# nolmoonen/jpeggpu

Measured on AMD Instinct MI355X. Metric: images/s, 12 MP 4:2:0 baseline JPEG decode, inputs resident in HBM (value_full_path: from pinned host memory, parse + transfer + decode; latency_ms: p50 of the reference's protocol), higher is better.
Workload: dtype int16/int32 fixed point, u8 out; 1 GPU; cfg2: 4032x3024 4:2:0 interleaved baseline JPEG, DRI=252 (one MCU row), 16 seeded images per rank; batch_per_gpu=256, mode=batch, streams=4, subsequence_bytes=256, device_scan=False, stuffed_scan_bytes=3163303, parallelism=image-sharded x1

## Files before the change

include/jpeggpu/jpeggpu_ext.h:

```cpp
#ifndef JPEGGPU_JPEGGPU_EXT_H_
#define JPEGGPU_JPEGGPU_EXT_H_

#include <jpeggpu/jpeggpu.h>

#ifdef __cplusplus
extern "C" {
#endif

enum jpeggpu_status jpeggpu_ext_set_subsequence_bytes(jpeggpu_decoder_t decoder, int subseq_bytes);
enum jpeggpu_status jpeggpu_ext_set_batched(jpeggpu_decoder_t decoder, int batched);
enum jpeggpu_status jpeggpu_ext_set_batch_hint(jpeggpu_decoder_t decoder, int images_per_call);

struct jpeggpu_ext_scan_layout {
    int num_components;
    int component_idx[JPEGGPU_MAX_COMP];
    int num_subsequences;
    int num_segments;
    int num_sequences;
    int num_data_units;
    int data_units_per_mcu;
    int num_chunks;
    size_t off_segments;
    size_t off_chunks;
    size_t off_destuffed;
// ... 15 lines not shown
struct jpeggpu_ext_layout {
    int subsequence_bytes;
    int subsequences_per_sequence;
    int num_scans;
    size_t transferred_bytes;
    size_t blob_bytes;
    size_t off_bytes;
    size_t off_qtables;
    struct jpeggpu_ext_scan_layout scans[JPEGGPU_MAX_COMP];
    int shard_rank, shard_world;
};

enum jpeggpu_status jpeggpu_ext_get_layout(jpeggpu_decoder_t decoder, struct jpeggpu_ext_layout* layout);

enum jpeggpu_status jpeggpu_ext_set_segment_shard(jpeggpu_decoder_t decoder, int rank, int world);
enum jpeggpu_status jpeggpu_ext_get_shard_rows(jpeggpu_decoder_t decoder, int component, int* first_row, int* num_rows);

enum jpeggpu_status jpeggpu_ext_set_device_scan(jpeggpu_decoder_t decoder, int enable);
enum jpeggpu_status jpeggpu_ext_get_device_status(
    jpeggpu_decoder_t decoder, const void* d_tmp, jpeggpu_stream_t stream, enum jpeggpu_status* status);

enum jpeggpu_status jpeggpu_ext_set_scale(jpeggpu_decoder_t decoder, int scale_denom);

enum jpeggpu_ext_scale_mode { JPEGGPU_EXT_SCALE_UNIFORM = 0, JPEGGPU_EXT_SCALE_LIBJPEG = 1 };
enum jpeggpu_status jpeggpu_ext_set_scale_mode(jpeggpu_decoder_t decoder, enum jpeggpu_ext_scale_mode mode);
struct jpeggpu_ext_scale_info {
    int scale_denom;
    int mode;
    int block_size[JPEGGPU_MAX_COMP];
    int fancy_upsampling;
};
enum jpeggpu_status jpeggpu_ext_get_scale_info(jpeggpu_decoder_t decoder, struct jpeggpu_ext_scale_info* info);

enum jpeggpu_ext_idct { JPEGGPU_EXT_IDCT_REFERENCE = 0, JPEGGPU_EXT_IDCT_ISLOW = 1 };
enum jpeggpu_status jpeggpu_ext_set_idct(jpeggpu_decoder_t decoder, enum jpeggpu_ext_idct method);

struct jpeggpu_ext_crop_info {
    int x, y, width, height;
    int origin_x[JPEGGPU_MAX_COMP];
    int origin_y[JPEGGPU_MAX_COMP];
    int full_x[JPEGGPU_MAX_COMP];
    int full_y[JPEGGPU_MAX_COMP];
};
enum jpeggpu_status jpeggpu_ext_set_crop(jpeggpu_decoder_t decoder, int x, int y, int width, int height);
enum jpeggpu_status jpeggpu_ext_get_crop(jpeggpu_decoder_t decoder, struct jpeggpu_ext_crop_info* info);

enum jpeggpu_status jpeggpu_ext_set_luma_only(jpeggpu_decoder_t decoder, int enable);

enum jpeggpu_ext_stage {
    JPEGGPU_EXT_STAGE_FRONT      = 0,
    JPEGGPU_EXT_STAGE_DESTUFF    = 1,
    JPEGGPU_EXT_STAGE_SYNC_INTRA = 2,
    JPEGGPU_EXT_STAGE_SYNC_INTER = 3,
    JPEGGPU_EXT_STAGE_TAILS      = 4,
    JPEGGPU_EXT_STAGE_WRITE      = 5,
    JPEGGPU_EXT_STAGE_IDCT       = 6,
    JPEGGPU_EXT_NUM_STAGES       = 7
};
enum jpeggpu_status jpeggpu_ext_set_profiling(jpeggpu_decoder_t decoder, int enable);
enum jpeggpu_status jpeggpu_ext_get_stage_ms(jpeggpu_decoder_t decoder, float* ms );

struct jpeggpu_batch;
typedef struct jpeggpu_batch* jpeggpu_batch_t;
struct jpeggpu_ext_batch_item {
    jpeggpu_decoder_t decoder;
    struct jpeggpu_img* img;
    void* d_tmp;
    size_t tmp_size;
};
size_t jpeggpu_ext_batch_scratch_size(int max_scans);
enum jpeggpu_status jpeggpu_ext_batch_create(jpeggpu_batch_t* batch, int max_scans);
enum jpeggpu_status jpeggpu_ext_decode_batch(
    jpeggpu_batch_t batch,
    const struct jpeggpu_ext_batch_item* items,
    int num_items,
    void* d_scratch,
    size_t scratch_size,
    jpeggpu_stream_t stream);
enum jpeggpu_status jpeggpu_ext_batch_destroy(jpeggpu_batch_t batch);
enum jpeggpu_status jpeggpu_ext_batch_set_sync_iterations(jpeggpu_batch_t batch, int iterations);
enum jpeggpu_status jpeggpu_ext_batch_set_overlap(jpeggpu_batch_t batch, int parts);
enum jpeggpu_status jpeggpu_ext_batch_set_fused_tail(jpeggpu_batch_t batch, int enable);
enum jpeggpu_status jpeggpu_ext_batch_set_sync_run(jpeggpu_batch_t batch, int r);
enum jpeggpu_status jpeggpu_ext_fused_tail_timeouts(unsigned int* count);
enum jpeggpu_status jpeggpu_ext_batch_set_profiling(jpeggpu_batch_t batch, int enable);
enum jpeggpu_status jpeggpu_ext_batch_get_stage_ms(jpeggpu_batch_t batch, float* ms );

enum jpeggpu_status jpeggpu_ext_upsample_planes(
    const struct jpeggpu_img_info* info,
    const struct jpeggpu_img* src,
    struct jpeggpu_img* dst,
    int width,
    int height,
    jpeggpu_stream_t stream);

enum jpeggpu_status jpeggpu_ext_self_test(jpeggpu_stream_t stream);

struct jpeggpu_ext_parse_item {
    jpeggpu_decoder_t decoder;
    struct jpeggpu_img_info* img_info;
    const uint8_t* data;
    size_t size;
};
enum jpeggpu_status jpeggpu_ext_parse_headers(
    const struct jpeggpu_ext_parse_item* items, int num_items, int num_threads, enum jpeggpu_status* statuses);

enum jpeggpu_status jpeggpu_ext_planes_to_rgbi(
    const struct jpeggpu_img_info* info,
    const struct jpeggpu_img* src,
    uint8_t* dst,
    int dst_pitch,
    int width,
    int height,
    jpeggpu_stream_t stream);

enum jpeggpu_status jpeggpu_ext_planes_to_rgbi_fancy(
    const struct jpeggpu_img_info* info,
    const struct jpeggpu_img* src,
    uint8_t* dst,
    int dst_pitch,
    int width,
    int height,
    jpeggpu_stream_t stream);

enum jpeggpu_status jpeggpu_ext_crop_to_rgbi_fancy(
    const struct jpeggpu_img_info* info,
    const struct jpeggpu_ext_crop_info* crop,
    const struct jpeggpu_img* src,
    uint8_t* dst,
    int dst_pitch,
    jpeggpu_stream_t stream);

enum jpeggpu_status jpeggpu_ext_planes_to_rgbi_replicate(
    const struct jpeggpu_img_info* info,
    const struct jpeggpu_img* src,
    uint8_t* dst,
    int dst_pitch,
    int width,
    int height,
    jpeggpu_stream_t stream);
enum jpeggpu_status jpeggpu_ext_crop_to_rgbi_replicate(
    const struct jpeggpu_img_info* info,
    const struct jpeggpu_ext_crop_info* crop,
    const struct jpeggpu_img* src,
    uint8_t* dst,
    int dst_pitch,
    jpeggpu_stream_t stream);

struct jpeggpu_ext_resize_item {
    const struct jpeggpu_img_info* info;
    const struct jpeggpu_ext_crop_info* crop;
    const struct jpeggpu_img* src;
};
enum jpeggpu_ext_filter { JPEGGPU_EXT_FILTER_BILINEAR = 0, JPEGGPU_EXT_FILTER_BICUBIC = 1 };
enum jpeggpu_ext_output_layout { JPEGGPU_EXT_NHWC = 0, JPEGGPU_EXT_NCHW = 1 };
size_t jpeggpu_ext_resize_scratch_size(
    const struct jpeggpu_ext_resize_item* items, int n, int out_w, int out_h, enum jpeggpu_ext_filter filter);
enum jpeggpu_status jpeggpu_ext_resize_to_rgb(
    const struct jpeggpu_ext_resize_item* items,
    int n,
    int out_w,
    int out_h,
    enum jpeggpu_ext_filter filter,
    enum jpeggpu_ext_output_layout layout,
    uint8_t* dst,
    void* d_scratch,
// ... 443 lines not shown
```

jpeggpu_amd/api.py:

```python
import ctypes as C
import enum
import os

from . import build as _build

MAX_COMP = 4
STAGES = ("front", "destuff", "sync_intra", "sync_inter", "tails", "write", "idct")
IDCT_METHODS = {"reference": 0, "islow": 1}
FILTERS = {"bilinear": 0, "bicubic": 1}
LAYOUTS = {"NHWC": 0, "NCHW": 1}
IMAGE_LAYOUTS = {"HWC": 0, "CHW": 1}
SCALE_MODES = {"uniform": 0, "libjpeg": 1}
SUBSAMPLINGS = {"4:4:4": 0, "4:2:2": 1, "4:2:0": 2}
TENSOR_TYPE_NAMES = {"uint8": 0, "float32": 1, "float16": 2, "bfloat16": 3}


def _tensor_types():
    import torch

    return {getattr(torch, name): v for name, v in TENSOR_TYPE_NAMES.items()}


class _TensorTypes(dict):

# ... 128 lines not shown
                ("progressive", C.c_int), ("optimize", C.c_int), ("restart_interval", C.c_int), ("out", C.c_void_p), ("capacity", C.c_size_t)]


class ExtScanLayout(C.Structure):
    _fields_ = [
        ("num_components", C.c_int), ("component_idx", C.c_int * MAX_COMP),
        ("num_subsequences", C.c_int), ("num_segments", C.c_int), ("num_sequences", C.c_int),
        ("num_data_units", C.c_int), ("data_units_per_mcu", C.c_int), ("num_chunks", C.c_int),
        ("off_segments", C.c_size_t), ("off_chunks", C.c_size_t), ("off_destuffed", C.c_size_t),
        ("off_segment_index", C.c_size_t), ("off_state_p", C.c_size_t), ("off_state_n", C.c_size_t),
        ("off_state_cz", C.c_size_t), ("off_state_dc01", C.c_size_t), ("off_state_dc23", C.c_size_t),
        ("off_symbols", C.c_size_t), ("off_du_table", C.c_size_t), ("symbol_region_entries", C.c_int),
        ("device_scan", C.c_int), ("off_device_status", C.c_size_t),
        ("hypotheses", C.c_int), ("hypothesis_blocks", C.c_int),
    ]


class ExtLayout(C.Structure):
    _fields_ = [
        ("subsequence_bytes", C.c_int), ("subsequences_per_sequence", C.c_int), ("num_scans", C.c_int),
        ("transferred_bytes", C.c_size_t), ("blob_bytes", C.c_size_t),
        ("off_bytes", C.c_size_t), ("off_qtables", C.c_size_t),
        ("scans", ExtScanLayout * MAX_COMP),
        ("shard_rank", C.c_int), ("shard_world", C.c_int),
    ]


class ParseItem(C.Structure):
    _fields_ = [("decoder", C.c_void_p), ("img_info", C.POINTER(ImgInfo)), ("data", C.c_void_p), ("size", C.c_size_t)]


class BatchItem(C.Structure):
    _fields_ = [("decoder", C.c_void_p), ("img", C.POINTER(Img)), ("d_tmp", C.c_void_p), ("tmp_size", C.c_size_t)]


class JpegGpuError(RuntimeError):
    def __init__(self, status, where=""):
        self.status = Status(status)
        super().__init__("%s: %s" % (where, status_string(status)))


_lib = None


def lib():
    global _lib
    if _lib is not None:
        return _lib
    try:
        import torch
    except ImportError:
        pass
    path = os.environ.get("JPEGGPU_LIB", _build.LIB_PATH)
    if not os.path.exists(path):
        raise ImportError(
            "jpeggpu_amd: %s is missing -- run `python -c 'import __graft_entry__ as g; g.build()'`" % path)
    L = C.CDLL(path)
    dec = C.c_void_p
    L.jpeggpu_get_status_string.restype = C.c_char_p
    L.jpeggpu_get_status_string.argtypes = [C.c_int]
    L.jpeggpu_decoder_startup.argtypes = [C.POINTER(dec)]
    L.jpeggpu_set_logging.argtypes = [dec, C.c_int]
    L.is_css_444.argtypes = [Subsampling, C.c_int]
    L.jpeggpu_decoder_parse_header.argtypes = [dec, C.POINTER(ImgInfo), C.c_void_p, C.c_size_t]
    L.jpeggpu_decoder_get_buffer_size.argtypes = [dec, C.POINTER(C.c_size_t)]
    L.jpeggpu_decoder_transfer.argtypes = [dec, C.c_void_p, C.c_size_t, C.c_void_p]
    L.jpeggpu_decoder_decode.argtypes = [dec, C.POINTER(Img), C.c_void_p, C.c_size_t, C.c_void_p]
    L.jpeggpu_decoder_cleanup.argtypes = [dec]
    L.jpeggpu_ext_set_subsequence_bytes.argtypes = [dec, C.c_int]
    L.jpeggpu_ext_set_batched.argtypes = [dec, C.c_int]
    L.jpeggpu_ext_set_batch_hint.argtypes = [dec, C.c_int]
    L.jpeggpu_ext_get_layout.argtypes = [dec, C.POINTER(ExtLayout)]
    L.jpeggpu_ext_set_profiling.argtypes = [dec, C.c_int]
    L.jpeggpu_ext_get_stage_ms.argtypes = [dec, C.POINTER(C.c_float)]
    L.jpeggpu_ext_batch_scratch_size.restype = C.c_size_t
    L.jpeggpu_ext_batch_scratch_size.argtypes = [C.c_int]
    L.jpeggpu_ext_batch_create.argtypes = [C.POINTER(C.c_void_p), C.c_int]
    L.jpeggpu_ext_decode_batch.argtypes = [C.c_void_p, C.POINTER(BatchItem), C.c_int, C.c_void_p, C.c_size_t, C.c_void_p]
    L.jpeggpu_ext_batch_destroy.argtypes = [C.c_void_p]
    L.jpeggpu_ext_batch_set_profiling.argtypes = [C.c_void_p, C.c_int]
    L.jpeggpu_ext_batch_set_sync_iterations.argtypes = [C.c_void_p, C.c_int]
    L.jpeggpu_ext_batch_set_overlap.argtypes = [C.c_void_p, C.c_int]
    for name, args in (("jpeggpu_ext_batch_set_fused_tail", [C.c_void_p, C.c_int]), ("jpeggpu_ext_batch_set_sync_run", [C.c_void_p, C.c_int]),
                       ("jpeggpu_ext_fused_tail_timeouts", [C.POINTER(C.c_uint)])):
        if hasattr(L, name):
            getattr(L, name).argtypes = args
    L.jpeggpu_ext_batch_get_stage_ms.argtypes = [C.c_void_p, C.POINTER(C.c_float)]
    L.jpeggpu_ext_upsample_planes.argtypes = [
        C.POINTER(ImgInfo), C.POINTER(Img), C.POINTER(Img), C.c_int, C.c_int, C.c_void_p]
    L.jpeggpu_ext_set_segment_shard.argtypes = [dec, C.c_int, C.c_int]
    L.jpeggpu_ext_get_shard_rows.argtypes = [dec, C.c_int, C.POINTER(C.c_int), C.POINTER(C.c_int)]
    L.jpeggpu_ext_self_test.argtypes = [C.c_void_p]
    L.jpeggpu_ext_set_device_scan.argtypes = [dec, C.c_int]
    L.jpeggpu_ext_set_scale.argtypes = [dec, C.c_int]
    L.jpeggpu_ext_set_idct.argtypes = [dec, C.c_int]
    L.jpeggpu_ext_set_scale_mode.argtypes = [dec, C.c_int]
    L.jpeggpu_ext_get_scale_info.argtypes = [dec, C.POINTER(ScaleInfo)]
    L.jpeggpu_ext_get_device_status.argtypes = [dec, C.c_void_p, C.c_void_p, C.POINTER(C.c_int)]
    L.jpeggpu_ext_parse_headers.argtypes = [C.POINTER(ParseItem), C.c_int, C.c_int, C.POINTER(C.c_int)]
    L.jpeggpu_ext_planes_to_rgbi.argtypes = [
        C.POINTER(ImgInfo), C.POINTER(Img), C.c_void_p, C.c_int, C.c_int, C.c_int, C.c_void_p]
    L.jpeggpu_ext_planes_to_rgbi_fancy.argtypes = [
        C.POINTER(ImgInfo), C.POINTER(Img), C.c_void_p, C.c_int, C.c_int, C.c_int, C.c_void_p]
    L.jpeggpu_ext_planes_to_rgbi_replicate.argtypes = L.jpeggpu_ext_planes_to_rgbi_fancy.argtypes
    L.jpeggpu_ext_set_crop.argtypes = [dec, C.c_int, C.c_int, C.c_int, C.c_int]
    L.jpeggpu_ext_get_crop.argtypes = [dec, C.POINTER(CropInfo)]
    L.jpeggpu_ext_crop_to_rgbi_fancy.argtypes = [
        C.POINTER(ImgInfo), C.POINTER(CropInfo), C.POINTER(Img), C.c_void_p, C.c_int, C.c_void_p]
    L.jpeggpu_ext_crop_to_rgbi_replicate.argtypes = L.jpeggpu_ext_crop_to_rgbi_fancy.argtypes
    L.jpeggpu_ext_resize_scratch_size.restype = C.c_size_t
    L.jpeggpu_ext_resize_scratch_size.argtypes = [C.POINTER(ResizeItem), C.c_int, C.c_int, C.c_int, C.c_int]
    L.jpeggpu_ext_resize_to_rgb.argtypes = [
        C.POINTER(ResizeItem), C.c_int, C.c_int, C.c_int, C.c_int, C.c_int, C.c_void_p, C.c_void_p, C.c_size_t, C.c_void_p]
    L.jpeggpu_ext_get_color_space.argtypes = [dec, C.POINTER(C.c_int)]
    L.jpeggpu_ext_planes_to_rgbi_fancy_cs.argtypes = [
        C.POINTER(ImgInfo), C.c_int, C.POINTER(Img), C.c_void_p, C.c_int, C.c_int, C.c_int, C.c_void_p]
    L.jpeggpu_ext_planes_to_rgbi_replicate_cs.argtypes = L.jpeggpu_ext_planes_to_rgbi_fancy_cs.argtypes
    L.jpeggpu_ext_crop_to_rgbi_fancy_cs.argtypes = [
        C.POINTER(ImgInfo), C.c_int, C.POINTER(CropInfo), C.POINTER(Img), C.c_void_p, C.c_int, C.c_void_p]
    L.jpeggpu_ext_crop_to_rgbi_replicate_cs.argtypes = L.jpeggpu_ext_crop_to_rgbi_fancy_cs.argtypes
    L.jpeggpu_ext_resize_scratch_size_cs.restype = C.c_size_t
    L.jpeggpu_ext_resize_scratch_size_cs.argtypes = [C.POINTER(ResizeItem), C.POINTER(C.c_int), C.c_int, C.c_int, C.c_int, C.c_int]
    L.jpeggpu_ext_resize_to_rgb_cs.argtypes = [
        C.POINTER(ResizeItem), C.POINTER(C.c_int), C.c_int, C.c_int, C.c_int, C.c_int, C.c_int, C.c_void_p, C.c_void_p, C.c_size_t,
        C.c_void_p]
    L.jpeggpu_ext_set_progressive.argtypes = [dec, C.c_int]
    L.jpeggpu_ext_get_progressive_info.argtypes = [dec, C.POINTER(ProgressiveInfo)]
    L.jpeggpu_ext_get_orientation.argtypes = [dec, C.POINTER(C.c_int)]
    L.jpeggpu_ext_orient_size.argtypes = [C.c_int, C.c_int, C.c_int, C.POINTER(C.c_int), C.POINTER(C.c_int)]
    L.jpeggpu_ext_orient_rect.argtypes = [C.c_int, C.c_int, C.c_int] + [C.POINTER(C.c_int)] * 4
    L.jpeggpu_ext_planes_to_rgbi_oriented.argtypes = [
        C.POINTER(ImgInfo), C.c_int, C.c_int, C.c_int, C.POINTER(Img), C.c_void_p, C.c_int, C.c_int, C.c_int, C.c_void_p]
    L.jpeggpu_ext_crop_to_rgbi_oriented.argtypes = [
        C.POINTER(ImgInfo), C.c_int, C.c_int, C.c_int, C.POINTER(CropInfo), C.POINTER(Img), C.c_void_p, C.c_int, C.c_void_p]
    L.jpeggpu_ext_resize_scratch_size_oriented.restype = C.c_size_t
    L.jpeggpu_ext_resize_scratch_size_oriented.argtypes = [
        C.POINTER(ResizeItem), C.POINTER(C.c_int), C.POINTER(C.c_int), C.c_int, C.c_int, C.c_int, C.c_int]
    L.jpeggpu_ext_resize_to_rgb_oriented.argtypes = [
        C.POINTER(ResizeItem), C.POINTER(C.c_int), C.POINTER(C.c_int), C.c_int, C.c_int, C.c_int, C.c_int, C.c_int, C.c_void_p,
        C.c_void_p, C.c_size_t, C.c_void_p]
    L.jpeggpu_ext_resize_to_tensor.argtypes = [
        C.POINTER(ResizeItem), C.POINTER(C.c_int), C.POINTER(C.c_int), C.c_int, C.c_int, C.c_int, C.c_int, C.c_int, C.POINTER(TensorSpec),
        C.c_void_p, C.c_void_p, C.c_size_t, C.c_void_p]
    L.jpeggpu_ext_resize_view_scratch_size.restype = C.c_size_t
    L.jpeggpu_ext_resize_view_scratch_size.argtypes = [
        C.POINTER(ResizeItem), C.POINTER(C.c_int), C.POINTER(C.c_int), C.POINTER(ResizeView), C.c_int, C.c_int, C.c_int, C.c_int]
    L.jpeggpu_ext_resize_view_to_tensor.argtypes = [
        C.POINTER(ResizeItem), C.POINTER(C.c_int), C.POINTER(C.c_int), C.POINTER(ResizeView), C.c_int, C.c_int, C.c_int, C.c_int, C.c_int,
        C.POINTER(TensorSpec), C.c_void_p, C.c_void_p, C.c_size_t, C.c_void_p]
    L.jpeggpu_ext_resize_view_rect.argtypes = [C.c_int, C.c_int, C.c_int, C.POINTER(ResizeView), C.c_int, C.c_int, C.c_int] + [C.POINTER(C.c_int)] * 4
    L.jpeggpu_ext_resize_view_weights.argtypes = [
        C.c_int, C.c_int, C.c_int, C.c_int, C.c_int, C.c_int, C.POINTER(C.c_int), C.POINTER(C.c_int), C.POINTER(C.c_int), C.c_int]
    L.jpeggpu_ext_batch_rgb_scratch_size.restype = C.c_size_t
    L.jpeggpu_ext_batch_rgb_scratch_size.argtypes = [C.c_int]
    L.jpeggpu_ext_batch_to_rgb.argtypes = [C.POINTER(RgbItem), C.c_int, C.c_int, C.c_void_p, C.c_size_t, C.c_void_p]
    if hasattr(L, "jpeggpu_ext_encode_batch"):
        L.jpeggpu_ext_encode_header.argtypes = [C.POINTER(EncodeItem), C.c_void_p, C.POINTER(C.c_size_t)]
        L.jpeggpu_ext_encode_bound.argtypes = [C.POINTER(EncodeItem)]
        L.jpeggpu_ext_encode_bound.restype = C.c_size_t
        L.jpeggpu_ext_encode_scratch_size.argtypes = [C.POINTER(EncodeItem), C.c_int]
        L.jpeggpu_ext_encode_scratch_size.restype = C.c_size_t
        L.jpeggpu_ext_encode_batch.argtypes = [C.POINTER(EncodeItem), C.c_int, C.c_void_p, C.c_size_t, C.c_void_p, C.c_void_p, C.c_void_p]
    if hasattr(L, "jpeggpu_ext_roundtrip_batch"):
        L.jpeggpu_ext_roundtrip_scratch_size.argtypes = [C.POINTER(RoundtripItem), C.c_int]
        L.jpeggpu_ext_roundtrip_scratch_size.restype = C.c_size_t
        L.jpeggpu_ext_roundtrip_batch.argtypes = [C.POINTER(RoundtripItem), C.c_int, C.c_int, C.c_void_p, C.c_size_t, C.c_void_p]
# ... 183 lines not shown
        _check(lib().jpeggpu_ext_set_segment_shard(self._h, rank, world), "jpeggpu_ext_set_segment_shard")

    def shard_rows(self, component: int):
        a, n = C.c_int(), C.c_int()
        _check(lib().jpeggpu_ext_get_shard_rows(self._h, component, C.byref(a), C.byref(n)), "jpeggpu_ext_get_shard_rows")
        return a.value, n.value

    def device_status(self, d_tmp: int, stream: int = 0) -> Status:
        st = C.c_int()
        _check(lib().jpeggpu_ext_get_device_status(self._h, d_tmp, stream, C.byref(st)), "jpeggpu_ext_get_device_status")
        return Status(st.value)

    def get_buffer_size(self) -> int:
        n = C.c_size_t()
        _check(lib().jpeggpu_decoder_get_buffer_size(self._h, C.byref(n)), "jpeggpu_decoder_get_buffer_size")
        return n.value

    def transfer(self, d_tmp: int, tmp_size: int, stream: int = 0):
        _check(lib().jpeggpu_decoder_transfer(self._h, d_tmp, tmp_size, stream), "jpeggpu_decoder_transfer")

    def decode(self, planes, pitches, d_tmp: int, tmp_size: int, stream: int = 0):
        _check(lib().jpeggpu_decoder_decode(self._h, C.byref(_img(planes, pitches)), d_tmp, tmp_size, stream), "jpeggpu_decoder_decode")

    def set_profiling(self, on: bool):
        _check(lib().jpeggpu_ext_set_profiling(self._h, int(on)), "jpeggpu_ext_set_profiling")

    def stage_ms(self):
        ms = (C.c_float * len(STAGES))()
        _check(lib().jpeggpu_ext_get_stage_ms(self._h, ms), "jpeggpu_ext_get_stage_ms")
        return dict(zip(STAGES, ms))

    def layout(self) -> ExtLayout:
        lay = ExtLayout()
        _check(lib().jpeggpu_ext_get_layout(self._h, C.byref(lay)), "jpeggpu_ext_get_layout")
        return lay

    def cleanup(self):
        if self._h:
            lib().jpeggpu_decoder_cleanup(self._h)
            self._h = C.c_void_p()

    def __del__(self):
        try:
            self.cleanup()
        except Exception:
            pass


class Batch:

    def __init__(self, max_scans: int):
        self._h = C.c_void_p()
        self.max_scans = max_scans
        _check(lib().jpeggpu_ext_batch_create(C.byref(self._h), max_scans), "jpeggpu_ext_batch_create")
        self.scratch_size = lib().jpeggpu_ext_batch_scratch_size(max_scans)
        self._items = None
        self._keep = None

    def set_items(self, entries):
        n = len(entries)
        arr = (BatchItem * n)()
        imgs = []
        for i, (dec, ptrs, pitches, d_tmp, tmp_size) in enumerate(entries):
            imgs.append(_img(ptrs, pitches))
            arr[i].decoder = dec._h
            arr[i].img = C.pointer(imgs[i])
            arr[i].d_tmp = d_tmp
            arr[i].tmp_size = tmp_size
        self._items, self._keep = arr, (imgs, entries)

    def decode(self, d_scratch: int, stream: int = 0):
        _check(lib().jpeggpu_ext_decode_batch(self._h, self._items, len(self._items), d_scratch, self.scratch_size, stream),
               "jpeggpu_ext_decode_batch")

    def set_overlap(self, parts: int):
        _check(lib().jpeggpu_ext_batch_set_overlap(self._h, parts), "jpeggpu_ext_batch_set_overlap")

    def set_fused_tail(self, enable: bool):
        _check(_newer_symbol("jpeggpu_ext_batch_set_fused_tail")(self._h, 1 if enable else 0), "jpeggpu_ext_batch_set_fused_tail")

    def set_sync_run(self, r: int):
        _check(_newer_symbol("jpeggpu_ext_batch_set_sync_run")(self._h, int(r)), "jpeggpu_ext_batch_set_sync_run")

    def set_coefficients_only(self, enable: bool):
        _check(_newer_symbol("jpeggpu_ext_batch_set_coefficients_only")(self._h, 1 if enable else 0), "jpeggpu_ext_batch_set_coefficients_only")

    def set_sync_iterations(self, n: int):
        _check(lib().jpeggpu_ext_batch_set_sync_iterations(self._h, n), "jpeggpu_ext_batch_set_sync_iterations")

    def set_profiling(self, on: bool):
        _check(lib().jpeggpu_ext_batch_set_profiling(self._h, int(on)), "jpeggpu_ext_batch_set_profiling")

    def stage_ms(self):
        ms = (C.c_float * len(STAGES))()
        _check(lib().jpeggpu_ext_batch_get_stage_ms(self._h, ms), "jpeggpu_ext_batch_get_stage_ms")
        return dict(zip(STAGES, ms))

    def destroy(self):
        if self._h:
            lib().jpeggpu_ext_batch_destroy(self._h)
            self._h = C.c_void_p()

    def __del__(self):
        try:
            self.destroy()
        except Exception:
            pass


def fused_tail_timeouts() -> int:
    n = C.c_uint(0)
    _check(_newer_symbol("jpeggpu_ext_fused_tail_timeouts")(C.byref(n)), "jpeggpu_ext_fused_tail_timeouts")
    return n.value


def self_test(stream: int = 0) -> None:
    _check(lib().jpeggpu_ext_self_test(stream), "jpeggpu_ext_self_test")


def draft_scale(width, height, requested):
    rw, rh = requested
    rw, rh = min(int(rw), width), min(int(rh), height)
    if rw < 1 or rh < 1:
        raise ValueError("requested size must be positive")
    s = min(width // rw, height // rh)
    return 8 if s >= 8 else 4 if s >= 4 else 2 if s >= 2 else 1


def orient_size(orientation, w, h):
    ow, oh = C.c_int(), C.c_int()
    _check(lib().jpeggpu_ext_orient_size(int(orientation), int(w), int(h), C.byref(ow), C.byref(oh)), "jpeggpu_ext_orient_size")
    return ow.value, oh.value


def orient_rect(orientation, w, h, rect):
    v = [C.c_int(int(a)) for a in rect]
    _check(lib().jpeggpu_ext_orient_rect(int(orientation), int(w), int(h), *[C.byref(a) for a in v]), "jpeggpu_ext_orient_rect")
    return tuple(a.value for a in v)


def _frame_size(info):
    n = info.num_components
    hmax, vmax = max(info.subsampling.x[:n]), max(info.subsampling.y[:n])
    return (info.sizes_x[[c for c in range(n) if info.subsampling.x[c] == hmax][0]],
            info.sizes_y[[c for c in range(n) if info.subsampling.y[c] == vmax][0]])


def decode_to_planes(data: bytes, device="cuda:0", subseq_bytes=None, return_tmp=False, device_scan=False, scale=1,
                     idct="reference", crop=None, scale_mode="uniform", return_color=False, progressive=False,
                     displayed_crop=False, return_orientation=False, luma_only=False):
    import torch

    dec = Decoder(subseq_bytes)
    try:
        if luma_only:
            dec.set_luma_only(True)
        if scale != 1:
            dec.set_scale(scale)
        if scale_mode != "uniform":
            dec.set_scale_mode(scale_mode)
        if idct != "reference":
            dec.set_idct(idct)
        if device_scan:
            dec.set_device_scan(True)
        if progressive:
            dec.set_progressive(True)
# ... 1417 lines not shown
```

jpeggpu_amd/csrc/jg_batch.cpp:

```cpp
#include "jg_decoder.hpp"
#include "jg_front.hpp"
#include "jg_kernels.hpp"
#include "jg_prog.hpp"
#include "jg_stage_timer.hpp"

#include <hip/hip_runtime.h>

#include <algorithm>
#include <cstdint>
#include <cstdlib>
#include <cstring>
#include <new>
#include <vector>

using jg::Decoder;

struct jpeggpu_batch {
    static constexpr int kRing = 4;
    int max_jobs = 0;
    uint8_t* staging[kRing]     = {};
    hipEvent_t copied[kRing]    = {};
    bool in_use[kRing]          = {};
    int next                    = 0;
    int sync_iters              = 1;
    bool sync_iters_set         = false;
    long long keep_flows_below  = jg::kKeepFlowsBelowSubseq;
    bool fuse_tail_write        = true;
    int sync_run                = 2;
    bool coefficients_only      = false;
    static constexpr int kMaxOverlap = 4;
    int overlap                 = 1;
    hipStream_t aux[kMaxOverlap - 1] = {};
    hipEvent_t joined[kMaxOverlap - 1] = {};
    std::vector<jg::ScanJob> jobs;
    std::vector<jg::FrontParams> fronts;
    std::vector<jg::ProgImage> progs;
    jg::ProgExtent prog_extent;
    hipEvent_t prog_done        = nullptr;
    std::vector<int> order, group_begin;
    struct Part {
        int begin, end, way;
        jg::JobExtent extent;
    };
    std::vector<Part> parts;
    jg::StageTimer timer;
};

namespace {

struct Call {
    const jpeggpu_ext_batch_item* items;
    int num_items;
    uint8_t* d_scratch;
    hipStream_t stream;
    bool keep_flows        = false;
    uint32_t front_windows = 0;
    size_t jbytes = 0, fbytes = 0, pbytes = 0;
    int ring = 0;
    hipStream_t part_stream[jpeggpu_batch::kMaxOverlap];
};

jpeggpu_status gather_jobs(jpeggpu_batch& b, Call& c)
{
    jg::ScanJob* d_jobs_rw = reinterpret_cast<jg::ScanJob*>(c.d_scratch);
    std::vector<int>& order = b.order;
    order.resize(static_cast<size_t>(c.num_items));
    for (int i = 0; i < c.num_items; ++i) order[static_cast<size_t>(i)] = i;
    std::stable_sort(order.begin(), order.end(), [&](int x, int y) { return c.items[x].decoder->d.subseq_bytes > c.items[y].decoder->d.subseq_bytes; });
    std::vector<int>& group_begin = b.group_begin;
    group_begin.clear();
    int subseq_bytes = 0;
    for (int k = 0; k < c.num_items; ++k) {
        const jpeggpu_ext_batch_item& it = c.items[order[static_cast<size_t>(k)]];
        if (it.decoder->d.subseq_bytes != subseq_bytes) {
            subseq_bytes = it.decoder->d.subseq_bytes;
            group_begin.push_back(static_cast<int>(b.jobs.size()));
        }
        const size_t first_job = b.jobs.size();
        const jpeggpu_status st = jg::build_jobs(it.decoder->d, it.img, it.d_tmp, it.tmp_size, b.sync_iters, false, c.keep_flows, b.jobs, !b.coefficients_only);
        if (st != JPEGGPU_SUCCESS) return st;
        if (const int dk = jg::device_scan_index(it.decoder->d); dk >= 0) {
            b.fronts.push_back(jg::front_params(it.decoder->d, it.d_tmp, d_jobs_rw + first_job + static_cast<size_t>(dk), dk));
            c.front_windows = std::max(c.front_windows, b.fronts.back().num_windows);
        }
        if (const Decoder& pd = it.decoder->d; pd.plan.prog.on) {
            b.progs.push_back(jg::ProgImage{static_cast<uint8_t*>(it.d_tmp), pd.plan.off_blob + pd.plan.prog.blob.header});
            jg::extend(b.prog_extent, *reinterpret_cast<const jg::ProgHeader*>(pd.blob + pd.plan.prog.blob.header));
        }
    }
    group_begin.push_back(static_cast<int>(b.jobs.size()));
    return JPEGGPU_SUCCESS;
}

jpeggpu_status stage_jobs(jpeggpu_batch& b, Call& c, size_t scratch_size)
{
    const size_t n = b.jobs.size(), nf = b.fronts.size(), np = b.progs.size();
    c.jbytes = sizeof(jg::ScanJob) * n, c.fbytes = sizeof(jg::FrontParams) * nf, c.pbytes = sizeof(jg::ProgImage) * np;
    if (static_cast<int>(n) > b.max_jobs || scratch_size < c.jbytes + c.fbytes + c.pbytes) return JPEGGPU_INVALID_ARGUMENT;
    const int r = c.ring = b.next;
    b.next      = (r + 1) % jpeggpu_batch::kRing;
    if (b.in_use[r] && hipEventSynchronize(b.copied[r]) != hipSuccess) return JPEGGPU_INTERNAL_ERROR;
    std::memcpy(b.staging[r], b.jobs.data(), c.jbytes);
    if (nf) std::memcpy(b.staging[r] + c.jbytes, b.fronts.data(), c.fbytes);
    if (np) std::memcpy(b.staging[r] + c.jbytes + c.fbytes, b.progs.data(), c.pbytes);
    if (!b.timer.begin(c.stream, static_cast<size_t>(jg::kNumStages) + 1)) return JPEGGPU_INTERNAL_ERROR;
    if (hipMemcpyAsync(c.d_scratch, b.staging[r], c.jbytes + c.fbytes + c.pbytes, hipMemcpyHostToDevice, c.stream) != hipSuccess) return JPEGGPU_INTERNAL_ERROR;
    if (nf && jg::launch_front_batch(reinterpret_cast<const jg::FrontParams*>(c.d_scratch + c.jbytes), static_cast<int>(nf), c.front_windows, c.stream) != hipSuccess) {
        (void)hipGetLastError();
        return JPEGGPU_INTERNAL_ERROR;
    }
    if (hipEventRecord(b.copied[r], c.stream) != hipSuccess) return JPEGGPU_INTERNAL_ERROR;
    b.in_use[r] = true;
    return JPEGGPU_SUCCESS;
}

jpeggpu_status cut_parts(jpeggpu_batch& b, Call& c)
{
    const int ways   = b.overlap;
    c.part_stream[0] = c.stream;
    for (int w = 1; w < ways; ++w) {
        if (!b.aux[w - 1]) {
            if (hipStreamCreateWithFlags(&b.aux[w - 1], hipStreamNonBlocking) != hipSuccess ||
                hipEventCreateWithFlags(&b.joined[w - 1], hipEventDisableTiming) != hipSuccess)
                return JPEGGPU_INTERNAL_ERROR;
        }
        c.part_stream[w] = b.aux[w - 1];
        if (hipStreamWaitEvent(c.part_stream[w], b.copied[c.ring], 0) != hipSuccess) return JPEGGPU_INTERNAL_ERROR;
    }
    typedef jpeggpu_batch::Part Part;
    b.parts.clear();
    for (size_t g = 0; g + 1 < b.group_begin.size(); ++g) {
        const int lo = b.group_begin[g], hi = b.group_begin[g + 1];
        int gw = ways;
        while (gw > 1 && (hi - lo) / gw < 4) --gw;
        for (int w = 0; w < gw; ++w) {
            Part p{lo + static_cast<int>(static_cast<long long>(hi - lo) * w / gw), lo + static_cast<int>(static_cast<long long>(hi - lo) * (w + 1) / gw), w, jg::JobExtent{}};
            for (int j = p.begin; j < p.end; ++j) jg::extend(p.extent, b.jobs[static_cast<size_t>(j)]);
            p.extent.repack_flows = c.keep_flows;
            p.extent.fuse_tail_write = b.fuse_tail_write && !b.sync_iters_set;
            p.extent.sync_run = c.keep_flows || b.sync_iters_set ? 1 : b.sync_run;
            if (p.end > p.begin) b.parts.push_back(p);
        }
    }
    return JPEGGPU_SUCCESS;
}

jpeggpu_status run_progressive(jpeggpu_batch& b, const Call& c)
{
    for (int k = 0; k < c.num_items; ++k) {
        const Decoder& pd = c.items[k].decoder->d;
        if (pd.plan.prog.on && hipMemsetAsync(static_cast<uint8_t*>(c.items[k].d_tmp) + pd.plan.prog.coef_begin, 0, pd.plan.prog.coef_bytes, c.stream) != hipSuccess)
            return JPEGGPU_INTERNAL_ERROR;
    }
    const jg::ProgImage* d_progs = reinterpret_cast<const jg::ProgImage*>(c.d_scratch + c.jbytes + c.fbytes);
    if (jg::launch_prog_batch(d_progs, static_cast<int>(b.progs.size()), b.prog_extent, c.stream) != hipSuccess) {
        (void)hipGetLastError();
        return JPEGGPU_INTERNAL_ERROR;
    }
    if (b.overlap > 1) {
        if (!b.prog_done && hipEventCreateWithFlags(&b.prog_done, hipEventDisableTiming) != hipSuccess) return JPEGGPU_INTERNAL_ERROR;
        if (hipEventRecord(b.prog_done, c.stream) != hipSuccess) return JPEGGPU_INTERNAL_ERROR;
        for (int w = 1; w < b.overlap; ++w)
            if (hipStreamWaitEvent(c.part_stream[w], b.prog_done, 0) != hipSuccess) return JPEGGPU_INTERNAL_ERROR;
    }
    return JPEGGPU_SUCCESS;
}

jpeggpu_status run_stages(jpeggpu_batch& b, const Call& c)
{
    const jg::ScanJob* d_jobs = reinterpret_cast<const jg::ScanJob*>(c.d_scratch);
    for (int stage = 0; stage < jg::kNumStages; ++stage) {
        const bool skip = stage == jg::kStageIdct && b.coefficients_only;
        if (stage == jg::kStageWrite && !b.progs.empty()) {
            const jpeggpu_status st = run_progressive(b, c);
            if (st != JPEGGPU_SUCCESS) return st;
        }
        for (const jpeggpu_batch::Part& p : b.parts) {
            if (skip) break;
            if (jg::launch_stage_batch(static_cast<jg::Stage>(stage), d_jobs + p.begin, p.end - p.begin, p.extent, c.part_stream[p.way]) != hipSuccess) {
                (void)hipGetLastError();
                return JPEGGPU_INTERNAL_ERROR;
            }
        }
        (void)b.timer.mark(stage, c.stream);
    }
    for (int w = 1; w < b.overlap; ++w) {
        if (hipEventRecord(b.joined[w - 1], c.part_stream[w]) != hipSuccess ||
            hipStreamWaitEvent(c.stream, b.joined[w - 1], 0) != hipSuccess)
            return JPEGGPU_INTERNAL_ERROR;
    }
    return JPEGGPU_SUCCESS;
}

jpeggpu_status decode_batch_impl(
    jpeggpu_batch_t batch, const jpeggpu_ext_batch_item* items, int num_items, void* d_scratch, size_t scratch_size, jpeggpu_stream_t stream)
{
    if (!batch || !items || num_items < 0 || !d_scratch) return JPEGGPU_INVALID_ARGUMENT;
    if (num_items == 0) return JPEGGPU_SUCCESS;
    batch->jobs.clear();
    batch->fronts.clear();
    batch->progs.clear();
    batch->prog_extent = jg::ProgExtent{};
    for (int i = 0; i < num_items; ++i)
        if (!items[i].decoder || !items[i].img) return JPEGGPU_INVALID_ARGUMENT;
    {
        bool all_lone = num_items <= jg::kLonePlanImages && !batch->timer.enabled() && !batch->coefficients_only;
        for (int i = 0; i < num_items && all_lone; ++i) all_lone = !items[i].decoder->d.batched;
        if (all_lone) {
            for (int i = 0; i < num_items; ++i) {
                const jpeggpu_status st = jg::do_decode(items[i].decoder->d, items[i].img, items[i].d_tmp, items[i].tmp_size, stream, false);
                if (st != JPEGGPU_SUCCESS) return st;
            }
            return JPEGGPU_SUCCESS;
        }
    }
    Call c{items, num_items, static_cast<uint8_t*>(d_scratch), stream};
    {
        long long total_subseq = 0;
        for (int i = 0; i < num_items; ++i) {
            const jg::Stream& s = items[i].decoder->d.reader.s;
            if (!items[i].decoder->d.parsed) return JPEGGPU_INVALID_ARGUMENT;
            for (int k = 0; k < s.num_scans; ++k) total_subseq += s.scans[k].num_subseq;
        }
        c.keep_flows = batch->sync_iters_set ? false : total_subseq < batch->keep_flows_below;
    }
    jpeggpu_status st = gather_jobs(*batch, c);
    if (st == JPEGGPU_SUCCESS) st = stage_jobs(*batch, c, scratch_size);
    if (st == JPEGGPU_SUCCESS) st = cut_parts(*batch, c);
    if (st == JPEGGPU_SUCCESS) st = run_stages(*batch, c);
    return st;
}

}

extern "C" {

size_t jpeggpu_ext_batch_scratch_size(int max_scans)
{
    static_assert(sizeof(jg::ProgImage) <= sizeof(jg::FrontParams), "a progressive item takes the place of front-end parameters");
    return static_cast<size_t>(max_scans > 0 ? max_scans : 0) * (sizeof(jg::ScanJob) + sizeof(jg::FrontParams));
}

enum jpeggpu_status jpeggpu_ext_batch_create(jpeggpu_batch_t* batch, int max_scans)
{
    if (!batch || max_scans <= 0) return JPEGGPU_INVALID_ARGUMENT;
    jpeggpu_batch* b = new (std::nothrow) jpeggpu_batch();
    if (!b) return JPEGGPU_OUT_OF_HOST_MEMORY;
    b->max_jobs = max_scans;
    if (const char* e = std::getenv("JPEGGPU_EXP_KEEP_FLOWS_BELOW")) b->keep_flows_below = std::atoll(e);
    if (const char* e = std::getenv("JPEGGPU_FUSE_TAIL_WRITE")) b->fuse_tail_write = std::atoi(e) != 0;
    if (const char* e = std::getenv("JPEGGPU_SYNC_RUN")) {
        const int r = std::atoi(e);
        if (r == 1 || r == 2 || r == 4) b->sync_run = r;
    }
    for (int r = 0; r < jpeggpu_batch::kRing; ++r) {
        void* p = nullptr;
        if (hipHostMalloc(&p, jpeggpu_ext_batch_scratch_size(max_scans), hipHostMallocDefault) != hipSuccess ||
            hipEventCreateWithFlags(&b->copied[r], hipEventDisableTiming) != hipSuccess) {
            (void)hipGetLastError();
            jpeggpu_ext_batch_destroy(b);
            return JPEGGPU_INTERNAL_ERROR;
        }
        b->staging[r] = static_cast<uint8_t*>(p);
    }
    *batch = b;
    return JPEGGPU_SUCCESS;
}

enum jpeggpu_status jpeggpu_ext_batch_destroy(jpeggpu_batch_t batch)
{
    if (!batch) return JPEGGPU_INVALID_ARGUMENT;
    for (int w = 0; w < jpeggpu_batch::kMaxOverlap - 1; ++w) {
        if (batch->aux[w]) {
            (void)hipStreamSynchronize(batch->aux[w]);
            (void)hipStreamDestroy(batch->aux[w]);
        }
        if (batch->joined[w]) (void)hipEventDestroy(batch->joined[w]);
    }
    for (int r = 0; r < jpeggpu_batch::kRing; ++r) {
        if (batch->staging[r]) (void)hipHostFree(batch->staging[r]);
        if (batch->copied[r]) (void)hipEventDestroy(batch->copied[r]);
    }
    if (batch->prog_done) (void)hipEventDestroy(batch->prog_done);
    delete batch;
    return JPEGGPU_SUCCESS;
}

enum jpeggpu_status jpeggpu_ext_decode_batch(
    jpeggpu_batch_t batch,
    const struct jpeggpu_ext_batch_item* items,
    int num_items,
    void* d_scratch,
    size_t scratch_size,
    jpeggpu_stream_t stream)
{
    try {
        return decode_batch_impl(batch, items, num_items, d_scratch, scratch_size, stream);
    } catch (const std::bad_alloc&) {
        return JPEGGPU_OUT_OF_HOST_MEMORY;
    }
}

enum jpeggpu_status jpeggpu_ext_batch_set_overlap(jpeggpu_batch_t batch, int parts)
{
    if (!batch || parts < 1 || parts > jpeggpu_batch::kMaxOverlap) return JPEGGPU_INVALID_ARGUMENT;
    batch->overlap = parts;
    return JPEGGPU_SUCCESS;
}

enum jpeggpu_status jpeggpu_ext_batch_set_fused_tail(jpeggpu_batch_t batch, int enable)
{
    if (!batch) return JPEGGPU_INVALID_ARGUMENT;
    batch->fuse_tail_write = enable != 0;
    return JPEGGPU_SUCCESS;
}

enum jpeggpu_status jpeggpu_ext_fused_tail_timeouts(unsigned int* count)
{
    if (!count) return JPEGGPU_INVALID_ARGUMENT;
    return jg::read_fuse_timeouts(count) == hipSuccess ? JPEGGPU_SUCCESS : JPEGGPU_INTERNAL_ERROR;
}

enum jpeggpu_status jpeggpu_ext_batch_set_sync_iterations(jpeggpu_batch_t batch, int iterations)
{
    if (!batch || iterations < 1) return JPEGGPU_INVALID_ARGUMENT;
    batch->sync_iters     = iterations;
    batch->sync_iters_set = true;
    return JPEGGPU_SUCCESS;
}

enum jpeggpu_status jpeggpu_ext_batch_set_coefficients_only(jpeggpu_batch_t batch, int enable)
{
    if (!batch) return JPEGGPU_INVALID_ARGUMENT;
    batch->coefficients_only = enable != 0;
    return JPEGGPU_SUCCESS;
}

enum jpeggpu_status jpeggpu_ext_batch_set_sync_run(jpeggpu_batch_t batch, int r)
{
    if (!batch || (r != 1 && r != 2 && r != 4)) return JPEGGPU_INVALID_ARGUMENT;
    batch->sync_run = r;
    return JPEGGPU_SUCCESS;
}

enum jpeggpu_status jpeggpu_ext_batch_set_profiling(jpeggpu_batch_t batch, int enable)
{
    if (!batch) return JPEGGPU_INVALID_ARGUMENT;
    batch->timer.enable(enable != 0);
    return JPEGGPU_SUCCESS;
}

enum jpeggpu_status jpeggpu_ext_batch_get_stage_ms(jpeggpu_batch_t batch, float* ms)
{
    if (!batch || !ms) return JPEGGPU_INVALID_ARGUMENT;
    return batch->timer.mean_ms(ms);
}

}
```

jpeggpu_amd/csrc/jg_defs.h:

```cpp
#ifndef JG_DEFS_H_
#define JG_DEFS_H_

#include <stddef.h>
#include <stdint.h>

#if defined(__HIPCC__)
#define JG_HD __host__ __device__
#else
#define JG_HD
#endif

namespace jg {

constexpr int kMaxComp      = 4;
constexpr int kMaxScans     = 4;
constexpr int kMaxDuPerMcu  = 10;
constexpr int kSeqLanes    = 256;
constexpr int kSeqOverlap  = 16;
constexpr int kSeqSubseq   = kSeqLanes - kSeqOverlap;
constexpr int kSeqOverlapBatch = 1;
constexpr int kSeqSubseqBatch  = kSeqLanes - kSeqOverlapBatch;
constexpr int kTailPartSubseq = 960;
constexpr long long kKeepFlowsBelowSubseq = 220000;
constexpr int kDestuffWin   = 4096;

#define JG_ORDER_NATURAL                                                                           \
    {0,  1,  8,  16, 9,  2,  3,  10, 17, 24, 32, 25, 18, 11, 4,  5,  12, 19, 26, 33, 40, 48,       \
     41, 34, 27, 20, 13, 6,  7,  14, 21, 28, 35, 42, 49, 56, 57, 50, 43, 36, 29, 22, 15, 23,       \
     30, 37, 44, 51, 58, 59, 52, 45, 38, 31, 39, 46, 53, 60, 61, 54, 47, 55, 62, 63}

constexpr int kLutBitsDc   = 9;
constexpr int kLutBitsAc   = 11;
constexpr int kSubBits     = 5;
constexpr int kSubTableSize = 2 << kSubBits;
constexpr int kMaxSubTables = 16;
constexpr int kHuffAuxSize = 16 + 16 + 256;
constexpr int kDcTableSize = (2 << kLutBitsDc) + kHuffAuxSize;
constexpr int kAcTableSize = (2 << kLutBitsAc) + kHuffAuxSize;

constexpr int kSyncEntryBytes = 4;
constexpr int kMultiMaxPre    = 15;
constexpr int kSyncMultiMaxBits = 31;
static_assert(kLutBitsAc + 15 <= kSyncMultiMaxBits && kSyncMultiMaxBits < (1 << 5),
              "a multi-symbol entry: codes inside the index, the last symbol's magnitude (category <= 15) behind it");
constexpr int kDcTableSizeSync = (kSyncEntryBytes << kLutBitsDc) + kHuffAuxSize;
constexpr int kAcTableSizeSync = (kSyncEntryBytes << kLutBitsAc) + kHuffAuxSize;

constexpr uint32_t kMaxTablePack =
    kMaxComp * (kDcTableSize + kMaxSubTables * kSubTableSize) + kMaxComp * (kAcTableSize + kMaxSubTables * kSubTableSize) + kMaxDuPerMcu * 16;
constexpr uint32_t kMaxTablePackSync =
    kMaxComp * (kDcTableSizeSync + kMaxSubTables * kSubTableSize) + kMaxComp * (kAcTableSizeSync + kMaxSubTables * kSubTableSize) + kMaxDuPerMcu * 16;
static_assert(kMaxTablePack < 65536 && kMaxTablePackSync < 65536, "table offsets are 16-bit");

constexpr uint32_t kEobAdvance = 63u;
constexpr uint32_t kEntrySlow  = 0x8000u;
JG_HD inline uint32_t huff_entry(int codelen, uint32_t sym, bool is_dc)
{
    const uint32_t s   = sym & 15u;
    const uint32_t r   = is_dc ? 0u : (sym >> 4);
    const bool eob = !is_dc && s == 0 && r != 15;
    return (static_cast<uint32_t>(codelen) + s) | (s << 5) | ((eob ? kEobAdvance : r + 1u) << 9);
}

constexpr int kRowLeadWords = 1;
constexpr int kRowTailWords = 2;
constexpr int kRowExtraWords = kRowLeadWords + kRowTailWords;
JG_HD constexpr int tile_rows_log2(int log2_w) { return log2_w >= 6 ? 4 : 5; }
constexpr int kMaxTileRows = 32;
JG_HD inline uint32_t tiled_slot(uint32_t row, uint32_t slot, int log2_w)
{
    const int lr = tile_rows_log2(log2_w);
    return (((row >> lr) * ((1u << log2_w) + kRowExtraWords) + slot) << lr) + (row & ((1u << lr) - 1u));
}
JG_HD inline uint32_t tiled_word(uint32_t linear_word, int log2_w)
{
    return tiled_slot(linear_word >> log2_w, (linear_word & ((1u << log2_w) - 1u)) + kRowLeadWords, log2_w);
}
JG_HD inline uint64_t tiled_buffer_bytes(uint32_t num_subseq, int subseq_bytes, int spare_rows)
{
    const uint64_t rows = (static_cast<uint64_t>(num_subseq) + static_cast<uint64_t>(spare_rows) + kMaxTileRows - 1) / kMaxTileRows * kMaxTileRows;
    return rows * (static_cast<uint64_t>(subseq_bytes) + 4u * kRowExtraWords);
}

constexpr uint32_t kMaxUnitEntries = 64 + 63;

constexpr uint32_t kSymSectorEntries = 16;
JG_HD constexpr uint32_t sym_region_entries(int subseq_bytes)
{
    return ((static_cast<uint32_t>(subseq_bytes) * 8u * 64u + 126u) / 127u + kMaxUnitEntries + kSymSectorEntries - 1u) / kSymSectorEntries * kSymSectorEntries;
}
static_assert(sym_region_entries(32) == 272 && sym_region_entries(64) == 400 && sym_region_entries(128) == 656 && sym_region_entries(256) == 1168,
              "whole sectors, at least ceil(8 B 64 / 127) + kMaxUnitEntries entries");

struct uint2_t {
    uint32_t x, y;
};

constexpr uint32_t kSymTileSubseq = 64;
constexpr uint32_t kSymSectorStride = kSymTileSubseq * kSymSectorEntries;
JG_HD inline uint32_t sym_region_base(uint32_t sub, uint32_t region_entries)
{
    return (sub / kSymTileSubseq) * (region_entries / kSymSectorEntries) * kSymSectorStride + (sub % kSymTileSubseq) * kSymSectorEntries;
}
JG_HD inline uint32_t sym_at(uint32_t base, uint32_t e)
{
    return base + (e / kSymSectorEntries) * kSymSectorStride + (e % kSymSectorEntries);
}
JG_HD inline uint32_t sym_advance(uint32_t first, uint32_t k)
{
    const uint32_t w = (first % kSymSectorEntries) + k;
    return (first & ~(kSymSectorEntries - 1u)) + (w / kSymSectorEntries) * kSymSectorStride + (w % kSymSectorEntries);
}
JG_HD inline uint64_t sym_buffer_entries(uint32_t num_subseq, uint32_t region_entries)
{
    const uint64_t tiles = (static_cast<uint64_t>(num_subseq) + kSymTileSubseq - 1) / kSymTileSubseq;
    return tiles * (region_entries / kSymSectorEntries) * kSymSectorStride + 16u * kSymSectorStride;
}
struct Segment {
    int subseq_offset;
    int subseq_count;
};

struct DestuffChunk {
    uint32_t win_off;
    uint32_t begin;
    uint32_t end;
    uint32_t dst_off;
    uint32_t pad_end;
    int32_t seg;
// ... 189 lines not shown
```

jpeggpu_amd/csrc/jg_huff_core.h:

```cpp
#ifndef JG_HUFF_CORE_H_
#define JG_HUFF_CORE_H_

#include "jg_defs.h"

namespace jg {

struct LaneState {
    int p;
    int n;
    int c;
    int z;
    uint32_t dc01;
    uint32_t dc23;
};

JG_HD inline uint32_t pk_add_u16(uint32_t a, uint32_t b)
{
#if defined(__HIP_DEVICE_COMPILE__)
    typedef unsigned short us2 __attribute__((ext_vector_type(2)));
    const us2 r = __builtin_bit_cast(us2, a) + __builtin_bit_cast(us2, b);
    return __builtin_bit_cast(uint32_t, r);
#else
    return ((a + b) & 0xFFFFu) | (((a >> 16) + (b >> 16)) << 16);
#endif
// ... 5 lines not shown
    int sh;
    typename Fetch::Pos pos;
    uint32_t next_raw;

    JG_HD inline void seek(int p, const Fetch& fetch)
    {
        const int q = p - 1;
        sh          = 31 - (q & 31);
        pos         = fetch.start(q >> 5);
        hi          = fetch.cook(fetch.load(pos), pos);
        fetch.advance(pos);
        lo = fetch.cook(fetch.load(pos), pos);
        fetch.advance(pos);
        next_raw = fetch.load(pos);
#if defined(__HIP_DEVICE_COMPILE__)
        asm volatile("v_mov_b32 %0, %0\n\tv_mov_b32 %1, %1" : "+v"(hi), "+v"(lo));
#endif
    }
    JG_HD inline uint32_t peek(const Fetch& fetch)
    {
        if (sh < 0) {
#if defined(__HIP_DEVICE_COMPILE__)
            asm("v_mov_b32 %0, %1\n\tv_mov_b32 %1, %2" : "+v"(hi), "+v"(lo) : "v"(fetch.cook(next_raw, pos)));
#else
            hi = lo;
            lo = fetch.cook(next_raw, pos);
#endif
            sh += 32;
            fetch.advance(pos);
            next_raw = fetch.load(pos);
        }
#if defined(__HIP_DEVICE_COMPILE__)
        return __builtin_amdgcn_alignbit(hi, lo, static_cast<uint32_t>(sh));
#else
        return static_cast<uint32_t>(((static_cast<uint64_t>(hi) << 32) | lo) >> sh);
#endif
    }
    JG_HD inline void skip(int len) { sh -= len; }
};

#if defined(JG_TABS_IN_LDS)
#define JG_TAB_AS __attribute__((address_space(3)))
#define JG_TAB_AT(tabs, off) (reinterpret_cast<::jg::TabPtr>(static_cast<uintptr_t>(static_cast<uint32_t>(off))))
#else
#define JG_TAB_AS
#define JG_TAB_AT(tabs, off) ((tabs) + (off))
#endif
typedef JG_TAB_AS const uint8_t* TabPtr;

JG_HD inline uint32_t ld_u16(TabPtr p) { return *reinterpret_cast<JG_TAB_AS const uint16_t*>(p); }
JG_HD inline uint32_t ld_u32(TabPtr p) { return *reinterpret_cast<JG_TAB_AS const uint32_t*>(p); }

JG_HD inline uint32_t huff_long_code(TabPtr aux, uint32_t peek, bool is_dc)
{
    const uint32_t v = peek >> 16;
    int l            = 9;
#if defined(__HIP_DEVICE_COMPILE__)
    typedef uint32_t u32x4 __attribute__((ext_vector_type(4)));
    const u32x4 lim = *reinterpret_cast<JG_TAB_AS const u32x4*>(aux);
#pragma unroll
    for (int j = 0; j < 7; ++j) l += v >= ((lim[j >> 1] >> (16 * (j & 1))) & 0xFFFFu) ? 1 : 0;
#else
    for (int j = 0; j < 7; ++j) l += v >= ld_u16(aux + 2 * j) ? 1 : 0;
#endif
    const uint32_t code = v >> (16 - l);
    const uint32_t off  = ld_u16(aux + 16 + 2 * (l - 9));
    const uint32_t sym  = aux[32 + ((off + code) & 0xFFu)];
    return huff_entry(l, sym, is_dc);
}

template <int kEntryBytes = 2>
JG_HD inline uint32_t huff_second_level(TabPtr tab, uint32_t e, uint32_t peek, bool is_dc)
{
    const int lb       = is_dc ? kLutBitsDc : kLutBitsAc;
    const TabPtr aux   = tab + (is_dc ? (kEntryBytes << kLutBitsDc) : (kEntryBytes << kLutBitsAc));
    if (e != 0) {
        const uint32_t i2 = (peek >> (32 - kSubBits - lb)) & ((1u << kSubBits) - 1u);
        e                 = ld_u16(aux + kHuffAuxSize - kSubTableSize + (e >> 5) * kSubTableSize + 2 * i2);
        if (e != 0) return e;
    }
    return huff_long_code(aux, peek, is_dc);
}

JG_HD inline int extend_magnitude(uint32_t bits, int s)
{
    const uint32_t mask = (1u << s) - 1u;
    return bits > (mask >> 1) ? static_cast<int>(bits) : static_cast<int>(bits - mask);
}

JG_HD inline uint32_t bits_field(uint32_t peek, int total_len, int s)
{
#if defined(__HIP_DEVICE_COMPILE__)
    return __builtin_amdgcn_ubfe(peek, 32 - total_len, s);
#else
    return s ? (peek << (total_len - s)) >> (32 - s) : 0u;
#endif
}

struct NoSink {
    static constexpr bool kSums = true;
};

struct SpecSink : NoSink {
    static constexpr bool kSums = false;
};

JG_HD inline uint32_t sym_entry_ac(int zpos, int value) { return (static_cast<uint32_t>(value) << 6) | static_cast<uint32_t>(zpos); }
JG_HD inline uint32_t sym_entry_escape(int value) { return (static_cast<uint32_t>(value) >> 10) << 6; }
JG_HD inline bool sym_needs_escape(int value) { return static_cast<uint32_t>(value + 511) > 1022u; }
constexpr int kEscapeFromCategory = 10;
JG_HD inline uint32_t sym_entry_index(uint32_t e) { return e & 63u; }
JG_HD inline int sym_entry_value(uint32_t e) { return static_cast<int16_t>(e) >> 6; }
JG_HD inline int sym_entry_value(uint32_t e, uint32_t escape) { return static_cast<int16_t>(((escape >> 6) << 10) | ((e & 0xFFFFu) >> 6)); }
constexpr uint32_t kUnitHasEscape = 0x80u;

#if defined(__HIP_DEVICE_COMPILE__)
#define JG_WAVE_ANY(x) (__builtin_amdgcn_ballot_w64(x) != 0ull)
#else
#define JG_WAVE_ANY(x) (x)
#endif

template <class Fetch, class Sink>
JG_HD inline void decode_subsequence(
    LaneState& st,
    BitWindow<Fetch>& bw,
    const Fetch& fetch,
    int end_bit,
    const uint8_t* tabs,
    const ScanParams& sp,
    Sink&)
{
#if defined(__HIP_DEVICE_COMPILE__)
    typedef uint32_t u32x4 __attribute__((ext_vector_type(4)));
#define JG_LOAD_CURSOR(off) (*reinterpret_cast<JG_TAB_AS const u32x4*>(JG_TAB_AT(tabs, off)))
    u32x4 cur = JG_LOAD_CURSOR(sp.cursor_off + 16u * static_cast<uint32_t>(st.c));
#define JG_CUR_TABS cur[0]
#define JG_CUR_META cur[1]
#define JG_CUR_SELF cur[2]
#define JG_CUR_NEXT cur[3]
#else
#define JG_LOAD_CURSOR(off) (*reinterpret_cast<const CursorEntry*>(tabs + (off)))
    CursorEntry cur = JG_LOAD_CURSOR(sp.cursor_off + 16u * static_cast<uint32_t>(st.c));
#define JG_CUR_TABS cur.tabs
#define JG_CUR_META cur.meta
#define JG_CUR_SELF cur.self
#define JG_CUR_NEXT cur.next
#endif
    int p       = st.p;
    int zm      = st.z - 1;
    int units   = 0;
    uint32_t dc01 = st.dc01, dc23 = st.dc23;
    bool is_dc = st.z == 0;
    uint32_t peek, e;
    int total;
#define JG_COMMIT()                                                                                       \
    do {                                                                                                  \
        bw.skip(total);                                                                                   \
        p += total;                                                                                       \
        const int adv     = e >> 9;                                                                       \
        const int zp      = zm + adv;                              \
        const bool du_end = zp >= 63;                                                                     \
        if (Sink::kSums && is_dc) {                                                                       \
            const int s      = (e >> 5) & 15;                                                             \
            const int v      = extend_magnitude(bits_field(peek, total, s), s);                           \
            const uint64_t d = static_cast<uint64_t>(static_cast<uint32_t>(v) & 0xFFFFu) << (JG_CUR_META & 63); \
            dc01             = pk_add_u16(dc01, static_cast<uint32_t>(d));                                \
            dc23             = pk_add_u16(dc23, static_cast<uint32_t>(d >> 32));                          \
        }                                                                                                 \
        zm = du_end ? -1 : zp;                                                                            \
        if (Sink::kSums) units += du_end ? 1 : 0;                                                         \
        cur = JG_LOAD_CURSOR(du_end ? JG_CUR_NEXT : JG_CUR_SELF);                                         \
        is_dc = du_end;                         \
    } while (0)
    {
        while (end_bit - p >= 31) {
            peek               = bw.peek(fetch);
            const TabPtr tab   = JG_TAB_AT(tabs, is_dc ? (JG_CUR_TABS & 0xFFFFu) : (JG_CUR_TABS >> 16));
            const uint32_t idx = peek >> (is_dc ? 32 - kLutBitsDc : 32 - kLutBitsAc);
            const uint32_t e32 = ld_u32(tab + kSyncEntryBytes * idx);
            const uint32_t one = e32 & 0xFFFFu, m = e32 >> 16;
            e                  = zm + static_cast<int>((m >> 5) & 15u) < 63 ? m : one;
            if (JG_WAVE_ANY((one & 31u) == 0)) {
                if ((one & 31u) == 0) e = huff_second_level<kSyncEntryBytes>(tab, one, peek, is_dc);
            }
            total = e & 31;
            JG_COMMIT();
        }
#define JG_LOOKUP_SYNC()                                                                                  \
    do {                                                                                                  \
        peek               = bw.peek(fetch);                                                              \
        const TabPtr tab   = JG_TAB_AT(tabs, is_dc ? (JG_CUR_TABS & 0xFFFFu) : (JG_CUR_TABS >> 16));      \
        const uint32_t idx = peek >> (is_dc ? 32 - kLutBitsDc : 32 - kLutBitsAc);                         \
        e                  = ld_u16(tab + kSyncEntryBytes * idx);                                         \
        if ((e & 31u) == 0) e = huff_second_level<kSyncEntryBytes>(tab, e, peek, is_dc);                  \
        total = e & 31;                                                                                   \
    } while (0)
        JG_LOOKUP_SYNC();
        while (p + total <= end_bit) {
            JG_COMMIT();
            JG_LOOKUP_SYNC();
        }
#undef JG_LOOKUP_SYNC
    }
#undef JG_COMMIT
    if (Sink::kSums) st.n += 64 * units + (zm + 1) - st.z;
    st.p    = p;
    st.z    = zm + 1;
    st.c    = (JG_CUR_META >> 8) & 0xFF;
    st.dc01 = dc01;
    st.dc23 = dc23;
#undef JG_LOAD_CURSOR
#undef JG_CUR_TABS
#undef JG_CUR_META
#undef JG_CUR_SELF
#undef JG_CUR_NEXT
}

constexpr int kWriteDcPeriod = 4;
constexpr int kWriteRarePeriod = 8;

JG_HD inline uint32_t bit_mask(int s)
{
#if defined(__HIP_DEVICE_COMPILE__)
    uint32_t m;
    asm("v_bfm_b32 %0, %1, 0" : "=v"(m) : "v"(s));
    return m;
#else
    return (1u << s) - 1u;
#endif
}

template <int kLutBits>
JG_HD inline uint32_t lut16_entry(TabPtr tab, uint32_t peek)
{
#if defined(__HIP_DEVICE_COMPILE__) && defined(JG_TABS_IN_LDS)
    uint32_t a;
    asm("v_lshrrev_b32 %0, %1, %2\n\tv_lshl_add_u32 %0, %0, 1, %3"
        : "=&v"(a)
        : "n"(32 - kLutBits), "v"(peek), "v"(static_cast<uint32_t>(reinterpret_cast<uintptr_t>(tab))));
    return ld_u16(reinterpret_cast<TabPtr>(static_cast<uintptr_t>(a)));
#else
    return ld_u16(tab + 2 * (peek >> (32 - kLutBits)));
#endif
}

JG_HD inline int lut16_entry_signed(TabPtr tab, uint32_t peek)
{
#if defined(__HIP_DEVICE_COMPILE__) && defined(JG_TABS_IN_LDS)
    uint32_t a;
    asm("v_lshrrev_b32 %0, %1, %2\n\tv_lshl_add_u32 %0, %0, 1, %3"
        : "=&v"(a)
        : "n"(32 - kLutBitsAc), "v"(peek), "v"(static_cast<uint32_t>(reinterpret_cast<uintptr_t>(tab))));
    return *reinterpret_cast<JG_TAB_AS const int16_t*>(static_cast<uintptr_t>(a));
#else
    return *reinterpret_cast<JG_TAB_AS const int16_t*>(tab + 2 * (peek >> (32 - kLutBitsAc)));
#endif
}

JG_HD inline uint32_t zero_if_negative(uint32_t e, int x)
{
#if defined(__HIP_DEVICE_COMPILE__)
    uint32_t r;
    asm("v_ashrrev_i32 %0, 31, %1\n\tv_bfi_b32 %0, %0, 0, %2" : "=&v"(r) : "v"(x), "v"(e));
    return r;
#else
    return x < 0 ? 0u : e;
#endif
}

JG_HD inline int extend_field(uint32_t peek, int total, int s)
{
#if defined(__HIP_DEVICE_COMPILE__)
    const int t = __builtin_amdgcn_sbfe(static_cast<int>(peek), static_cast<uint32_t>(32 - total), static_cast<uint32_t>(s));
    return t - static_cast<int>(bit_mask(s) ^ static_cast<uint32_t>(t >> 31));
#else
    const uint32_t bits = bits_field(peek, total, s);
    const uint32_t mask = bit_mask(s);
    return bits > (mask >> 1) ? static_cast<int>(bits) : static_cast<int>(bits - mask);
#endif
}

JG_HD inline int extend_bits(uint32_t bits, int s)
{
    const uint32_t mask = bit_mask(s);
    return bits > (mask >> 1) ? static_cast<int>(bits) : static_cast<int>(bits - mask);
// ... 143 lines not shown
```

jpeggpu_amd/csrc/jg_kernels.hip:

```cpp
#define JG_TABS_IN_LDS 1
#include "jg_huff_core.h"
#include "jg_kernels.hpp"
#include "jg_sync_runs.h"

#include <hip/hip_runtime.h>

#include <type_traits>

#include "jg_bytes.h"
#include "jg_idct.hpp"
#include "jg_jobs.h"
#include "jg_wave.h"

namespace jg {

namespace {

constexpr int T   = kSeqLanes;
constexpr int kMaxSeq = kSeqLanes - 1;


constexpr int kDestuffChunksPerWg = 2;

template <class J_t>
// ... 435 lines not shown
            st    = LaneState{};
            known = true;
        }
        lim = min(img_end, seg.subseq_offset + seg.subseq_count - img_first);
        flowing = known;
    }
    NoSink sink;
    const auto flow_step = [&](int j) -> bool {
        st.n    = 0;
        st.dc01 = 0;
        st.dc23 = 0;
        ++rel;
        fetch.set_row(img_first + j, rel);
        bw.seek(st.p, fetch);
        decode_subsequence(st, bw, fetch, (rel + 1) * kBits, s_tab, sp, sink);
        const int cz     = st.c | (st.z << 8);
        const bool synced = st.p == s_p[j] && cz == s_cz[j] && (s_pend[j] & 2);
        s_p[j]    = st.p;
        s_n[j]    = st.n;
        s_cz[j]   = cz;
        s_dc01[j] = st.dc01;
        s_dc23[j] = st.dc23;
        s_pend[j] = 2;
        return !synced;
    };
    int j    = t;
    int iter = 0;
    for (; iter < sp.max_intra_iters; ++iter) {
        bool go = flowing && j + 1 < lim;
        if (iter > 0) {
            int rank;
            const int total = block_rank<T>(go, s_wave, rank);
            if (total == 0) break;
            if (go) {
                s_fj[rank]   = j | lim << 16;
                s_frel[rank] = rel;
                s_fp[rank]   = st.p;
                s_fcz[rank]  = st.c | (st.z << 8);
            }
            __syncthreads();
            go = t < total;
            if (go) {
                const int pk = s_fj[t], cz = s_fcz[t];
                j    = pk & 0xFFFF;
                lim  = pk >> 16;
                rel  = s_frel[t];
                st.p = s_fp[t];
                st.c = cz & 0xFF;
                st.z = cz >> 8;
            }
        }
        flowing = go;
        if (go) flowing = flow_step(++j);
    }
    if (iter == sp.max_intra_iters && flowing && j + 1 < lim) {
        if (j >= OV) s_pend[j] |= 1;
        if (j == OV - 1) s_cut = 1;
    }
    __syncthreads();

    if (active && t >= OV) {
        J.pending[sub] = static_cast<uint8_t>(s_pend[t] & 1);
        J.st_p[sub]    = s_p[t];
        J.st_n[sub]    = s_n[t];
        J.st_cz[sub]   = s_cz[t];
        J.st_dc01[sub] = s_dc01[t];
        J.st_dc23[sub] = s_dc23[t];
    }
    if (t == OV - 1) {
        const bool have = active && !s_cut;
        J.bnd_p[blockIdx.x]  = have ? s_p[t] : -1;
        J.bnd_cz[blockIdx.x] = have ? s_cz[t] : -1;
    }
}

constexpr int kBatchSeqPerWg = 2;
struct SeqLdsBatch {
    static constexpr uint32_t kState = 0;
    static constexpr uint32_t kOne   = (6 * (T + 1) * 4 + 64 + 15) / 16 * 16;
    static constexpr uint32_t kTabs  = kState + kBatchSeqPerWg * kOne;
    static_assert(kTabs % 16 == 0, "the table pack is read with 16-byte loads");
};
static_assert(kStaticLdsSlack + SeqLdsBatch::kTabs + kMaxTablePackSync <= 65536, "absolute table addresses are packed into 16 bits (load_tables)");
constexpr int kFuseJobs = 16, kFuseMaxJobs = 256, kFuseOwn = kFuseJobs + 2 * kFuseMaxJobs;
constexpr uint32_t kFuseEmpty = 0xFFFFFFFFu;
static_assert(fuse_ctl_words(0) == static_cast<size_t>(kFuseOwn), "the plan carves what fuse_init lays out (jg_defs.h)");

__device__ __forceinline__ void fuse_init(const ScanJob* jobs, int job, const JobView& J, int lanes)
{
    JG_GLOBAL uint32_t* own  = as_global(jobs[job].fuse_ctl);
    JG_GLOBAL uint32_t* ctl0 = as_global(jobs[0].fuse_ctl);
    const int t = threadIdx.x, SEQ = J.sp.seq_subseq, S = J.sp.num_subseq;
    if (t < kFuseJobs) own[t] = 0u;
    if (t < 2 && job < kFuseMaxJobs) ctl0[kFuseJobs + 2 * job + t] = 0u;
    for (int q = t; q < J.num_seq; q += lanes) {
        const int first = q * SEQ, last = min(first + SEQ, S) - 1;
        uint32_t holders = 0;
        for (int k = 0; k < J.num_tail_parts; ++k) holders += J.tail_parts[k] <= last && J.tail_parts[k + 1] > first ? 1u : 0u;
        own[kFuseOwn + q]             = holders;
        own[kFuseOwn + J.num_seq + q] = kFuseEmpty;
    }
}

struct RunIo {
    const JobView& J;
    int* s_p;
    int* s_cz;
    __device__ __forceinline__ Segment segment_of(int sub) const { return ld_global(J.segments + J.seg_idx[sub]); }
    __device__ __forceinline__ void put_e1(int lane, int p, int cz) const
    {
        s_p[lane]  = p;
        s_cz[lane] = cz;
    }
    __device__ __forceinline__ bool e1_is(int lane, int p, int cz) const { return s_p[lane] == p && s_cz[lane] == cz; }
    __device__ __forceinline__ void store(int sub, const LaneState& st, int cz, bool pending) const
    {
        J.pending[sub] = static_cast<uint8_t>(pending ? 1 : 0);
        J.st_p[sub]    = st.p;
        J.st_n[sub]    = st.n;
        J.st_cz[sub]   = cz;
        J.st_dc01[sub] = st.dc01;
        J.st_dc23[sub] = st.dc23;
    }
};

template <int W, class JS, int R>
__device__ __forceinline__ void sync_intra_batch_runs(const JS& js, uint8_t* smem)
{
    const int which = threadIdx.x / T, l = threadIdx.x % T;
    int* s_p        = reinterpret_cast<int*>(smem + SeqLdsBatch::kState + which * SeqLdsBatch::kOne);
    int* s_cz       = s_p + 2 * T;
    uint8_t* s_tab  = smem + SeqLdsBatch::kTabs;

    const JobView J(js.get());
    if constexpr (std::is_same<JS, JobArray>::value) {
        if (blockIdx.x == 0) fuse_init(js.jobs, static_cast<int>(blockIdx.y), J, T * kBatchSeqPerWg);
    }
    if (static_cast<int>(blockIdx.x) * kBatchSeqPerWg * R >= J.num_seq) return;
    ScanParams sp = J.sp;
    sp.use_sync_pack();
    const int SEQ   = sp.seq_subseq;
    const int group = static_cast<int>(blockIdx.x) * kBatchSeqPerWg + which;
    RunLane ln;
    run_plan<R>(ln, l, group * SEQ * R, SEQ, sp.num_subseq);
    const int lane_seg = J.seg_idx[ln.active ? ln.a : 0];

    load_tables(s_tab, J.tables_sync, sp);
    const Segment lane_segment = ld_global(J.segments + lane_seg);
    __syncthreads();

    GlobalFetch<W> fetch{reinterpret_cast<JG_GLOBAL const uint32_t*>(J.destuffed), 0, 0};
    const RunIo io{J, s_p, s_cz};
    run_speculate<W>(ln, l, lane_segment, fetch, s_tab, sp, io);
    __syncthreads();
    run_flow<W, R>(ln, l, fetch, s_tab, sp, io);

    if (l < R && group * R + l < J.num_seq) {
        J.bnd_p[group * R + l]  = -1;
        J.bnd_cz[group * R + l] = -1;
    }
}

template <int W, class JS, int R = 1>
__global__ __launch_bounds__(T * kBatchSeqPerWg) void huff_sync_intra_batch(JS js)
{
    extern __shared__ __attribute__((aligned(16))) uint8_t smem[];
    if constexpr (R > 1) {
        sync_intra_batch_runs<W, JS, R>(js, smem);
        return;
    }
    const int which = threadIdx.x / T;
    const int seq   = blockIdx.x * kBatchSeqPerWg + which;
    int* s_p         = reinterpret_cast<int*>(smem + SeqLdsBatch::kState + which * SeqLdsBatch::kOne);
    int* s_n         = s_p + T;
    int* s_cz        = s_n + T;
    uint32_t* s_dc01 = reinterpret_cast<uint32_t*>(s_cz + T);
    uint32_t* s_dc23 = s_dc01 + T;
    int* s_pend      = reinterpret_cast<int*>(s_dc23 + T);
    uint8_t* s_tab   = smem + SeqLdsBatch::kTabs;

    const JobView J(js.get());
    if constexpr (std::is_same<JS, JobArray>::value) {
        if (blockIdx.x == 0) fuse_init(js.jobs, static_cast<int>(blockIdx.y), J, T * kBatchSeqPerWg);
    }
    if (static_cast<int>(blockIdx.x) * kBatchSeqPerWg >= J.num_seq) return;
    ScanParams sp = J.sp;
    sp.use_sync_pack();
    const int t         = threadIdx.x % T;
    s_pend[t]           = 0;
    const int SEQ = sp.seq_subseq, OV = T - SEQ;
    const int first_sub = seq * SEQ;
    const int img_first = first_sub - OV;
    const int img_end   = min(T, sp.num_subseq - img_first);

    constexpr int kBits = W * 32;
    const int sub       = img_first + t;
    const bool active   = sub >= 0 && t < img_end;
    const int lane_seg = J.seg_idx[active ? sub : 0];

    load_tables(s_tab, J.tables_sync, sp);
    const Segment lane_segment = ld_global(J.segments + lane_seg);
    __syncthreads();

    constexpr bool mh = false;
    LaneState st{};
    BitWindow<GlobalFetch<W>> bw{};
    GlobalFetch<W> fetch{reinterpret_cast<JG_GLOBAL const uint32_t*>(J.destuffed), 0, 0};
    Segment seg{0, 0};
    int rel = 0;
    bool known = true;
    if (active) {
        seg = lane_segment;
        rel = sub - seg.subseq_offset;
        if (mh) {
            st.p         = J.mh_p[sub];
            const int cz = J.mh_cz[sub];
            st.c         = cz & 0xFF;
            st.z         = cz >> 8;
            known        = J.mh_known[sub] != 0;
            s_pend[t]    = known ? 2 : 0;
        } else {
            st.p = rel * kBits;
            fetch.set_row(sub, rel);
            bw.seek(st.p, fetch);
            if (JS::kSpeculateStateOnly) {
                SpecSink none;
                decode_subsequence(st, bw, fetch, (rel + 1) * kBits, s_tab, sp, none);
            } else {
                NoSink sums;
                decode_subsequence(st, bw, fetch, (rel + 1) * kBits, s_tab, sp, sums);
                s_n[t]    = st.n;
                s_dc01[t] = st.dc01;
                s_dc23[t] = st.dc23;
            }
            s_pend[t] = 2;
        }
        s_p[t]  = st.p;
        s_cz[t] = st.c | (st.z << 8);
    }
    __syncthreads();

    const bool covers_starts = JS::kSpeculateStateOnly || mh;
    bool flowing = covers_starts ? t + 1 < img_end && img_first + t + 1 >= 0 : active;
    int lim      = 0;
    if (flowing) {
        const int sub_j = img_first + t + 1;
        if (covers_starts && (!active || rel + 1 == seg.subseq_count)) {
            seg   = ld_global(J.segments + J.seg_idx[sub_j]);
            rel   = -1;
            st    = LaneState{};
            known = true;
        }
        lim = min(img_end, seg.subseq_offset + seg.subseq_count - img_first);
        flowing = known;
    }
    NoSink sink;
    int iter = 0;
    for (; iter < sp.max_intra_iters; ++iter) {
        const int j = t + 1 + iter;
        if (flowing && j < lim) {
            st.n    = 0;
            st.dc01 = 0;
            st.dc23 = 0;
            ++rel;
            fetch.set_row(img_first + j, rel);
            bw.seek(st.p, fetch);
            decode_subsequence(st, bw, fetch, (rel + 1) * kBits, s_tab, sp, sink);
            const int cz = st.c | (st.z << 8);
            if (st.p == s_p[j] && cz == s_cz[j] && (s_pend[j] & 2)) flowing = false;
            s_p[j]    = st.p;
            s_n[j]    = st.n;
            s_cz[j]   = cz;
            s_dc01[j] = st.dc01;
            s_dc23[j] = st.dc23;
            s_pend[j] = 2;
        } else {
            flowing = false;
        }
        const bool more = __syncthreads_or(flowing && j + 1 < lim);
        if (!more) break;
    }
    if (iter == sp.max_intra_iters && flowing && t + 1 + iter < lim && t + iter >= OV) s_pend[t + iter] |= 1;
    __syncthreads();

    if (active && t >= OV) {
        J.pending[sub] = static_cast<uint8_t>(s_pend[t] & 1);
        J.st_p[sub]    = s_p[t];
        J.st_n[sub]    = s_n[t];
        J.st_cz[sub]   = s_cz[t];
        J.st_dc01[sub] = s_dc01[t];
        J.st_dc23[sub] = s_dc23[t];
    }
    if (t == OV - 1 && seq < J.num_seq) {
        J.bnd_p[seq]  = -1;
        J.bnd_cz[seq] = -1;
    }
}


template <int W, class JS>
__global__ __launch_bounds__(T) void huff_mh_spec(JS js)
{
    extern __shared__ __attribute__((aligned(16))) uint8_t smem[];
    const JobView J(js.get());
    ScanParams sp = J.sp;
    sp.use_sync_pack();
    load_tables(smem, J.tables_sync, sp);
    __syncthreads();
    const int sub = blockIdx.x * T + threadIdx.x, h = blockIdx.y;
    if (sub == 0 && h == 0) st_global(J.mh_pool, uint2_t{0u, 0u});
    if (sub >= sp.num_subseq) return;
    const Segment seg = ld_global(J.segments + J.seg_idx[sub]);
    const int rel     = sub - seg.subseq_offset;
    LaneState st{};
    st.p = rel * (W * 32);
    st.c = h;
    GlobalFetch<W> fetch{reinterpret_cast<JG_GLOBAL const uint32_t*>(J.destuffed), 0, 0};
    fetch.set_row(sub, rel);
    BitWindow<GlobalFetch<W>> bw{};
    bw.seek(st.p, fetch);
    SpecSink none;
    decode_subsequence(st, bw, fetch, (rel + 1) * (W * 32), smem, sp, none);
    const size_t at = static_cast<size_t>(h) * sp.num_subseq + sub;
    J.mh_p[at]      = st.p;
    J.mh_cz[at]     = st.c | (st.z << 8);
}

template <int W, class JS>
__global__ __launch_bounds__(T) void huff_mh_flow(JS js)
{
    extern __shared__ __attribute__((aligned(16))) uint8_t smem[];
    const JobView J(js.get());
    ScanParams sp = J.sp;
    sp.use_sync_pack();
    load_tables(smem, J.tables_sync, sp);
    __syncthreads();
    const int sub = blockIdx.x * T + threadIdx.x, h = blockIdx.y;
    const int S = sp.num_subseq, H = sp.mh;
    if (sub >= S) return;
    const size_t at   = static_cast<size_t>(h) * S + sub;
    const Segment seg = ld_global(J.segments + J.seg_idx[sub]);
    const int seg_end = seg.subseq_offset + seg.subseq_count;
    LaneState st{};
    st.p = J.mh_p[at];
    {
        const int cz = J.mh_cz[at];
        st.c         = cz & 0xFF;
        st.z         = cz >> 8;
    }
    GlobalFetch<W> fetch{reinterpret_cast<JG_GLOBAL const uint32_t*>(J.destuffed), 0, 0};
// ... 751 lines not shown
        JG_GLOBAL uint32_t* own = as_global(job.fuse_ctl);
        const int SEQ = J.sp.seq_subseq, lo = J.tail_parts[part], hi = J.tail_parts[part + 1];
        for (int q = lo / SEQ + static_cast<int>(threadIdx.x); q <= (hi - 1) / SEQ && q < J.num_seq; q += T) {
            if (JG_FUSE_ADD(own + kFuseOwn + q, 0xFFFFFFFFu) == 1u) {
                const uint32_t i = JG_FUSE_ADD(ctl0 + kFuseJobs + 2 * j, 1u);
                if (i < static_cast<uint32_t>(J.num_seq)) JG_FUSE_STORE(own + kFuseOwn + J.num_seq + i, static_cast<uint32_t>(q));
            }
        }
        return;
    }
    const uint32_t r = role - num_tail;
    if (r >= static_cast<uint32_t>(num_jobs) * static_cast<uint32_t>(max_seq)) return;
    const uint32_t home = r / static_cast<uint32_t>(max_seq);
    if (static_cast<int>(r % static_cast<uint32_t>(max_seq)) >= constant_job(jobs, home).num_seq) return;
    if (threadIdx.x < 64) {
        uint32_t polls = 0, got_job = kFuseEmpty, got_i = 0;
        while (got_job == kFuseEmpty) {
            for (int base = 0; base < num_jobs && got_job == kFuseEmpty; base += 64) {
                const int k      = base + static_cast<int>(threadIdx.x);
                const uint32_t j = (home + static_cast<uint32_t>(k)) % static_cast<uint32_t>(num_jobs);
                bool has         = false;
                if (k < num_jobs) {
                    const uint32_t pushed = JG_FUSE_LOAD(ctl0 + kFuseJobs + 2 * j), claimed = JG_FUSE_LOAD(ctl0 + kFuseJobs + 2 * j + 1);
                    has                   = claimed < pushed;
                }
                const unsigned long long any = __builtin_amdgcn_ballot_w64(has);
                if (any) {
                    const int first = __builtin_ctzll(any);
                    const uint32_t jj = static_cast<uint32_t>(__builtin_amdgcn_readlane(static_cast<int>(j), first));
                    uint32_t i = 0;
                    if (threadIdx.x == 0) i = JG_FUSE_ADD(ctl0 + kFuseJobs + 2 * jj + 1, 1u);
                    i = static_cast<uint32_t>(__builtin_amdgcn_readfirstlane(static_cast<int>(i)));
                    if (i < static_cast<uint32_t>(constant_job(jobs, jj).num_seq)) {
                        got_job = jj;
                        got_i   = i;
                    }
                }
            }
            if (got_job == kFuseEmpty) {
                if (++polls > kFuseMaxPolls) break;
                __builtin_amdgcn_s_sleep(32);
            }
        }
        uint32_t q = kFuseEmpty;
        if (got_job != kFuseEmpty) {
            const ScanJob& job = constant_job(jobs, got_job);
            JG_GLOBAL uint32_t* entry = as_global(job.fuse_ctl) + kFuseOwn + job.num_seq + got_i;
            while ((q = JG_FUSE_LOAD(entry)) == kFuseEmpty) {
                if (++polls > kFuseMaxPolls) break;
                __builtin_amdgcn_s_sleep(8);
            }
        }
        if (threadIdx.x == 0) {
            if (q == kFuseEmpty) atomicAdd(&g_fuse_timeouts, 1u);
            s_claim[0] = got_job;
            s_claim[1] = q;
        }
    }
    __syncthreads();
    const uint32_t seq = __builtin_amdgcn_readfirstlane(s_claim[1]);
    if (seq == kFuseEmpty) return;
    const ScanJob& job = constant_job(jobs, __builtin_amdgcn_readfirstlane(s_claim[0]));
    const JobView J(job);
    write_sequence<W, true>(J, static_cast<int>(seq), smem);
}
#undef JG_FUSE_LOAD
#undef JG_FUSE_ADD
#undef JG_FUSE_STORE


template <class K>
hipError_t allow_lds(K kernel, size_t bytes)
{
    if (bytes <= 64 * 1024) return hipSuccess;
    return hipFuncSetAttribute(
        reinterpret_cast<const void*>(kernel), hipFuncAttributeMaxDynamicSharedMemorySize, static_cast<int>(bytes));
}

inline bool fuses_tail_write(const JobExtent& e, int num_jobs)
{
    return e.fuse_tail_write && !e.repack_flows && e.max_tail_parts > 0 && e.max_tail_part < kTailLargeFrom && e.max_seq > 0 && num_jobs <= kFuseMaxJobs;
}

template <int W, class JS>
hipError_t launch_huff(Stage stage, const JS& js, const JobExtent& e, int grid_y, hipStream_t stream)
{
    const size_t seq_lds = SeqLds::kTabs + e.max_tab_bytes_sync;
    hipError_t err       = hipSuccess;
    if (e.max_tab_bytes > kMaxTablePack || e.max_tab_bytes_sync > kMaxTablePackSync) return hipErrorInvalidValue;
    switch (stage) {
    case kStageSyncIntra:
        if constexpr (JS::kRepackFlows) {
            if ((err = allow_lds(huff_sync_intra<W, JS>, seq_lds)) != hipSuccess) return err;
            huff_sync_intra<W, JS><<<dim3(e.max_seq, grid_y), T, seq_lds, stream>>>(js);
        } else if (e.repack_flows) {
            if ((err = allow_lds(huff_sync_intra<W, JobArrayLow>, seq_lds)) != hipSuccess) return err;
            huff_sync_intra<W, JobArrayLow><<<dim3(e.max_seq, grid_y), T, seq_lds, stream>>>(JobArrayLow{js.jobs});
        } else {
            const size_t lds = SeqLdsBatch::kTabs + e.max_tab_bytes_sync;
            if (e.sync_run == 2 || e.sync_run == 4) {
                const int per_wg = kBatchSeqPerWg * e.sync_run;
                const dim3 grid((e.max_seq + per_wg - 1) / per_wg, grid_y);
                if (e.sync_run == 2) {
                    if ((err = allow_lds(huff_sync_intra_batch<W, JS, 2>, lds)) != hipSuccess) return err;
                    huff_sync_intra_batch<W, JS, 2><<<grid, T * kBatchSeqPerWg, lds, stream>>>(js);
                } else {
                    if ((err = allow_lds(huff_sync_intra_batch<W, JS, 4>, lds)) != hipSuccess) return err;
                    huff_sync_intra_batch<W, JS, 4><<<grid, T * kBatchSeqPerWg, lds, stream>>>(js);
                }
                break;
            }
            if ((err = allow_lds(huff_sync_intra_batch<W, JS>, lds)) != hipSuccess) return err;
            huff_sync_intra_batch<W, JS><<<dim3((e.max_seq + kBatchSeqPerWg - 1) / kBatchSeqPerWg, grid_y), T * kBatchSeqPerWg, lds, stream>>>(js);
        }
        break;
    case kStageSyncInter:
        if (e.max_tail_parts > 0 && !(std::is_same<JS, JobArray>::value && fuses_tail_write(e, grid_y)))
        {
            if (e.max_tail_part >= kTailLargeFrom) {
                constexpr int TL = kTailLanesLarge;
                huff_sync_tail<W, TL, JS><<<dim3(e.max_tail_parts, grid_y), TL, 3 * TL * 4 + e.max_tab_bytes_sync, stream>>>(js);
            } else {
                huff_sync_tail<W, T, JS><<<dim3(e.max_tail_parts, grid_y), T, 3 * T * 4 + e.max_tab_bytes_sync, stream>>>(js);
            }
        }
        break;
    case kStageWrite: {
        size_t lds = WriteLds::kTabs + e.max_tab_bytes;
        if constexpr (std::is_same<JS, JobArray>::value) {
            if (fuses_tail_write(e, grid_y)) {
                const size_t tail_lds = 3 * T * 4 + e.max_tab_bytes_sync;
                lds                   = lds > tail_lds ? lds : tail_lds;
                if ((err = allow_lds(huff_tail_write<W>, lds)) != hipSuccess) return err;
                const long long wgs = static_cast<long long>(grid_y) * (static_cast<long long>(e.max_tail_parts) + e.max_seq);
                if (wgs > 0x7FFFFFFFll) return hipErrorInvalidValue;
                huff_tail_write<W><<<dim3(static_cast<unsigned>(wgs)), T, lds, stream>>>(js.jobs, grid_y, e.max_tail_parts, e.max_seq);
                break;
            }
        }
        huff_write<W, JS><<<dim3(e.max_seq, grid_y), T, lds, stream>>>(js);
        break;
    }
    default: return hipErrorInvalidValue;
    }
    return hipGetLastError();
}


inline hipError_t launch_idct(const JobByValue& js, const JobExtent& e, int, hipStream_t stream) { return launch_idct_job(js.job, e, stream); }
inline hipError_t launch_idct(const JobsByValue& js, const JobExtent& e, int num_jobs, hipStream_t stream) { return launch_idct_scans(js.jobs, num_jobs, e, stream); }
inline hipError_t launch_idct(const JobSingle& js, const JobExtent& e, int, hipStream_t stream) { return launch_idct_device_job(js.job, e, stream); }
inline hipError_t launch_idct(const JobArray& js, const JobExtent& e, int num_jobs, hipStream_t stream) { return launch_idct_batch(js.jobs, num_jobs, e, stream); }

template <class JS>
hipError_t launch_any(Stage stage, const JS& js, const JobExtent& e, int grid_y, hipStream_t stream)
{
    switch (stage) {
    case kStageFront:
        return hipSuccess;
    case kStageDestuff:
        if (e.max_chunks == 0) return hipSuccess;
        destuff_kernel<JS><<<dim3((e.max_chunks + kDestuffChunksPerWg - 1) / kDestuffChunksPerWg, grid_y), 256, 0, stream>>>(js);
        return hipGetLastError();
    case kStageTails:
        if (e.max_seq == 0 || (e.max_tail_parts > 0 && e.max_tail_part < kTailLargeFrom)) return hipSuccess;
        huff_seq_tails<JS><<<dim3(e.max_seq, grid_y), T, 0, stream>>>(js);
        return hipGetLastError();
    case kStageIdct: return launch_idct(js, e, grid_y, stream);
    case kStageSyncIntra:
    case kStageSyncInter:
    case kStageWrite:
        if (e.max_seq == 0) return hipSuccess;
        switch (e.subseq_words) {
        case 8: return launch_huff<8, JS>(stage, js, e, grid_y, stream);
        case 16: return launch_huff<16, JS>(stage, js, e, grid_y, stream);
        case 32: return launch_huff<32, JS>(stage, js, e, grid_y, stream);
        case 64: return launch_huff<64, JS>(stage, js, e, grid_y, stream);
        }
        return hipErrorInvalidValue;
    default: return hipErrorInvalidValue;
// ... 112 lines not shown
```

jpeggpu_amd/csrc/jg_kernels.hpp:

```cpp
#ifndef JG_KERNELS_HPP_
#define JG_KERNELS_HPP_

#include "jg_defs.h"

#include <hip/hip_runtime_api.h>

namespace jg {

bool subseq_bytes_supported(int subseq_bytes);

enum Stage {
    kStageFront     = 0,
    kStageDestuff   = 1,
    kStageSyncIntra = 2,
    kStageSyncInter = 3,
    kStageTails     = 4,
    kStageWrite     = 5,
    kStageIdct      = 6,
    kNumStages      = 7
};

struct JobExtent {
    int max_chunks      = 0;
    int max_seq         = 0;
    int max_tail_parts  = 0;
    int max_tail_part   = 0;
    int max_idct_blocks = 0;
    int subseq_words    = 0;
    uint32_t scales     = 0;
    uint32_t draft_sizes = 0;
    bool luma_reference = false;
    uint32_t methods    = 0;
    bool crop           = false;
    uint32_t max_tab_bytes = 0;
    uint32_t max_tab_bytes_sync = 0;
    bool fuse_tail_write = false;
    int sync_run        = 1;
    bool repack_flows   = false;
};
void extend(JobExtent& e, const ScanJob& job);
hipError_t read_fuse_timeouts(unsigned int* count);

hipError_t launch_stage(Stage stage, const ScanJob& job, hipStream_t stream);

hipError_t launch_stage_scans(Stage stage, const ScanJob* jobs, int num_jobs, hipStream_t stream);

hipError_t launch_mh(const ScanJob& job, const ScanJob* d_job, int max_seg_subseq, hipStream_t stream);

hipError_t launch_stage_device_job(Stage stage, const ScanJob* d_job, const JobExtent& extent, hipStream_t stream);

hipError_t launch_stage_batch(
    Stage stage, const ScanJob* d_jobs, int num_jobs, const JobExtent& extent, hipStream_t stream);

}

#endif
```

jpeggpu_amd/csrc/jg_plan.cpp:

```cpp
#include "jg_decoder.hpp"

#include <algorithm>
#include <cstring>
#include <new>

namespace jg {

namespace {

size_t align_up(size_t v, size_t a) { return (v + a - 1) / a * a; }

struct Carve {
    size_t at = 0;
    std::vector<PlanTrace::Region>* trace = nullptr;
    size_t operator()(size_t bytes)
    {
        const size_t o = at;
        at += align_up(bytes, 256);
        if (trace) trace->push_back({o, bytes});
        return o;
    }
};

template <typename T>
T* at(uint8_t* base, size_t off)
{
    return reinterpret_cast<T*>(base + off);
}

}

void Decoder::set_block_sizes()
{
    const Stream& s = reader.s;
    const int mn    = 8 >> scale_log2;
    draft           = false;
    for (int c = 0; c < s.num_comp; ++c) {
        int size = mn;
        if (scale_mode == JPEGGPU_EXT_SCALE_LIBJPEG)
            while (size < 8 && (s.hs_max * mn) % (s.comp[c].hs * size * 2) == 0 && (s.vs_max * mn) % (s.comp[c].vs * size * 2) == 0) size *= 2;
        blk_lg[c] = size == 8 ? 0 : size == 4 ? 1 : size == 2 ? 2 : 3;
        if (size != mn) draft = true;
    }
}

bool Decoder::set_crop_window()
{
    const Stream& s = reader.s;
    Crop c;
    c.on = true;
    c.x = crop_request[0], c.y = crop_request[1], c.w = crop_request[2], c.h = crop_request[3];
    if (c.x + static_cast<long long>(c.w) > scaled(s.size_x) || c.y + static_cast<long long>(c.h) > scaled(s.size_y)) return false;
    int lo_x[kMaxComp], hi_x[kMaxComp], lo_y[kMaxComp], hi_y[kMaxComp];
    c.mx0 = c.my0 = 1 << 30;
    for (int k = 0; k < s.num_comp; ++k) {
        const Component& fc = s.comp[k];
        const int n = blk(k), hs = eff_hs(k), vs = eff_vs(k);
        lo_x[k] = std::max(static_cast<int>(static_cast<long long>(c.x) * hs / s.hs_max) - 1, 0);
        hi_x[k] = std::min(static_cast<int>(static_cast<long long>(c.x + c.w - 1) * hs / s.hs_max) + 1, full_x(k) - 1);
        lo_y[k] = std::max(static_cast<int>(static_cast<long long>(c.y) * vs / s.vs_max) - 1, 0);
        hi_y[k] = std::min(static_cast<int>(static_cast<long long>(c.y + c.h - 1) * vs / s.vs_max) + 1, full_y(k) - 1);
        c.mx0 = std::min(c.mx0, lo_x[k] / (n * fc.hs)), c.mx1 = std::max(c.mx1, hi_x[k] / (n * fc.hs) + 1);
        c.my0 = std::min(c.my0, lo_y[k] / (n * fc.vs)), c.my1 = std::max(c.my1, hi_y[k] / (n * fc.vs) + 1);
    }
    for (int k = 0; k < s.num_comp; ++k) {
        const Component& fc = s.comp[k];
        const int n = blk(k);
        c.ox[k] = c.mx0 * n * fc.hs, c.oy[k] = c.my0 * n * fc.vs;
        c.wx[k] = hi_x[k] + 1 - c.ox[k], c.wy[k] = hi_y[k] + 1 - c.oy[k];
    }
    crop = c;
    return true;
}

IdctWindow Decoder::scan_window(const Scan& sc) const
{
    IdctWindow w{};
    if (!crop.on) return w;
    if (sc.num_comp > 1) {
        w.mx0 = crop.mx0, w.my0 = crop.my0, w.mcus_x = crop.mx1 - crop.mx0, w.mcus_y = crop.my1 - crop.my0;
    } else {
        const int c = sc.comp[0].comp_idx, n = blk(c);
        w.mx0 = crop.ox[c] / n, w.my0 = crop.oy[c] / n;
        w.mcus_x = (crop.ox[c] + crop.wx[c] + n - 1) / n - w.mx0, w.mcus_y = (crop.oy[c] + crop.wy[c] + n - 1) / n - w.my0;
    }
    const MagicDiv m = magic_div(static_cast<uint32_t>(w.mcus_x));
    w.mcus_x_mul = m.mul, w.mcus_x_shift = m.shift;
    return w;
}

void Decoder::make_plan(PlanTrace* trace)
{
    const Stream& s = reader.s;
    Plan p;
    Carve blob{0, trace ? &trace->blob : nullptr};
    p.blob_qtables = blob(sizeof(s.qtable));
    for (int i = 0; i < s.num_scans; ++i) {
        const Scan& sc      = s.scans[i];
        ScanPlan& sp        = p.scan[i];
        sp.blob_tables      = blob(sc.table_pack.size());
        sp.blob_tables_sync = blob(sc.table_pack_sync.size());
        sp.blob_segments    = blob(sc.segments.size() * sizeof(Segment));
        sp.blob_chunks      = blob(sc.chunks.size() * sizeof(DestuffChunk));
        sp.blob_parts       = blob(sc.tail_parts.size() * sizeof(int));
        sp.mh = 0;
        sp.mh_blocks.clear();
        int run = 1;
        {
            int du_tabs[2 * kMaxDuPerMcu], m = 0;
            for (int rep = 0; rep < 2; ++rep)
                for (int a = 0; a < sc.num_comp; ++a)
                    for (int k = 0; k < sc.comp[a].h * sc.comp[a].v && m < 2 * kMaxDuPerMcu; ++k) du_tabs[m++] = sc.comp[a].dc_id * 4 + sc.comp[a].ac_id;
            for (int i = 1, cur = 1; i < m; ++i) {
                cur = du_tabs[i] == du_tabs[i - 1] ? cur + 1 : 1;
                run = std::max(run, std::min(cur, sc.du_per_mcu));
            }
        }
        if (!batched && sc.du_per_mcu >= 2 && sc.du_per_mcu <= kMhMaxHyp && mh_enabled && run >= 2) {
            int longest = sc.device_walk ? kMhMaxSegSubseq : 0;
            for (const Segment& g : sc.segments) longest = std::max(longest, g.subseq_count);
            const bool device_blocks = sc.device_walk && s.restart_interval == 0;
            if (device_blocks) longest = std::max(sc.num_subseq, kMhMaxSegSubseq + 1);
            if (longest <= kMhMaxSegSubseq && run < 3 && sc.du_per_mcu < 4) longest = -1;
            if (longest > kMhMaxSegSubseq && run < 3) longest = -1;
            sp.mh_blocks_device = 0;
            if (longest < 0) {
            } else if (longest <= kMhMaxSegSubseq) {
                sp.mh             = sc.du_per_mcu;
                sp.max_seg_subseq = longest;
            } else if (device_blocks) {
                const int nb = (sc.num_subseq + kMhMaxSegSubseq - 1) / kMhMaxSegSubseq;
                if (nb <= kMhMaxBlocks) {
                    sp.mh               = sc.du_per_mcu;
                    sp.max_seg_subseq   = kMhMaxSegSubseq;
                    sp.mh_blocks_device = nb;
                }
            } else if (!sc.device_walk) {
                for (const Segment& g : sc.segments) {
                    for (int r = 0; r < g.subseq_count; r += kMhMaxSegSubseq)
                        sp.mh_blocks.push_back(MhBlock{g.subseq_offset + r, std::min(kMhMaxSegSubseq, g.subseq_count - r),
                                                       g.subseq_offset + g.subseq_count, r == 0 ? 1 : 0});
                }
                if (sp.mh_blocks.size() <= static_cast<size_t>(kMhMaxBlocks)) {
                    sp.mh             = sc.du_per_mcu;
                    sp.max_seg_subseq = kMhMaxSegSubseq;
                    sp.blob_mh_blocks = blob(sp.mh_blocks.size() * sizeof(MhBlock));
                } else {
                    sp.mh_blocks.clear();
                }
            }
        }
    }
    if (s.progressive) {
        const size_t begin = blob.at;
        p.prog.on = true;
        prog_plan_blob(s, p.prog.blob, blob.at);
        if (trace) trace->blob.push_back({begin, blob.at - begin});
    }
    p.blob_size = blob.at;

    Carve tmp{0, trace ? &trace->tmp : nullptr};
    p.bytes_len = s.xfer_end - s.xfer_begin;
    p.off_bytes = tmp(align_up(p.bytes_len, kDestuffWin) + kDestuffWin);
    p.off_blob  = tmp(p.blob_size);
    for (int i = 0; i < s.num_scans; ++i) {
        const Scan& sc = s.scans[i];
        ScanPlan& sp   = p.scan[i];
        const size_t S = static_cast<size_t>(sc.num_subseq);
        sp.num_seq     = static_cast<int>((S + kSeqSubseq - 1) / kSeqSubseq);
        const size_t Q = static_cast<size_t>(sp.num_seq);
        sp.destuffed   = tmp(tiled_buffer_bytes(static_cast<uint32_t>(S), subseq_bytes, 96) + 256);
        sp.seg_idx     = tmp(S * 4);
        sp.st_p        = tmp(S * 4);
        sp.st_n        = tmp(S * 4);
        sp.st_cz       = tmp(S * 4);
        sp.st_dc01     = tmp(S * 4);
        sp.st_dc23     = tmp(S * 4);
        sp.pending     = tmp(S);
        sp.flow_list   = tmp(S * 4);
        sp.tails_n     = tmp(Q * 4);
        sp.tails_dc01  = tmp(Q * 4);
        sp.tails_dc23  = tmp(Q * 4);
        sp.bnd_p       = tmp(Q * 4);
        sp.bnd_cz      = tmp(Q * 4);
        sp.fuse_ctl    = tmp(fuse_ctl_words(Q) * 4);
        if (sp.mh > 1) {
            const size_t N = S * static_cast<size_t>(sp.mh);
            sp.mh_p        = tmp(N * 4);
            sp.mh_cz       = tmp(N * 4);
            sp.mh_link     = tmp(N * 4);
            sp.mh_pool     = tmp((1 + static_cast<size_t>(mh_pool_entries(static_cast<uint32_t>(S)))) * sizeof(uint2_t));
            sp.mh_known    = tmp(S);
            const size_t nblocks = sp.mh_blocks_device ? static_cast<size_t>(sp.mh_blocks_device) : sp.mh_blocks.size();
            if (nblocks) {
                sp.mh_blk_exit  = tmp(nblocks * 64 * sizeof(uint16_t));
                sp.mh_blk_entry = tmp(nblocks * sizeof(uint16_t));
            }
            if (sp.mh_blocks_device) sp.d_mh_blocks = tmp(nblocks * sizeof(MhBlock));
        }
        if (sc.device_walk) {
            const size_t E  = static_cast<size_t>(sc.expect_segments);
            sp.num_windows  = static_cast<uint32_t>(align_up(p.bytes_len, kDestuffWin) / kDestuffWin) - sc.front_win0;
            const size_t Wn = sp.num_windows;
            sp.d_segments   = tmp(E * sizeof(Segment));
            sp.d_chunks     = tmp(static_cast<size_t>(sc.max_chunks) * sizeof(DestuffChunk));
            sp.d_parts      = tmp(static_cast<size_t>(sc.max_tail_parts) * sizeof(int));
            sp.d_win_data   = tmp(Wn * 4);
            sp.d_win_nmark  = tmp(Wn * 4);
            sp.d_win_bad    = tmp(Wn * 4);
            sp.d_win_prefix = tmp((Wn + 1) * 4);
            sp.d_mark_off   = tmp((Wn + 1) * 4);
            sp.d_mk_pos     = tmp((E + 1) * 4);
            sp.d_mk_g       = tmp((E + 1) * 4);
            sp.d_seg_cnt    = tmp((E + 1) * 4);
            sp.d_seg_nch    = tmp((E + 1) * 4);
            sp.d_job        = tmp(sizeof(ScanJob));
            sp.d_status     = tmp(32);
        }
    }
    for (int i = 0; i < s.num_scans; ++i) {
        p.scan[i].sym    = tmp(sym_buffer_entries(sym_regions(i), sym_region()) * 2 + 256);
        p.scan[i].du_tab = tmp(static_cast<size_t>(s.scans[i].num_du) * sizeof(uint2_t));
    }
    if (s.progressive) {
        p.prog.coef_begin = tmp.at;
        for (int c = 0; c < s.num_comp; ++c)
            p.prog.coef[c] = tmp(static_cast<size_t>(s.prog_blocks_x[c]) * static_cast<size_t>(s.prog_blocks_y[c]) * 64 * sizeof(int16_t));
        p.prog.coef_bytes = tmp.at - p.prog.coef_begin;
    }
    p.total = tmp.at;
    plan    = p;
}

jpeggpu_status Decoder::plan_image(jpeggpu_img_info* img_info, const uint8_t* data, size_t size, PlanTrace* trace)
{
    parsed      = false;
    scale_log2  = scale_log2_request;
    idct_method = idct_method_request;
    scale_mode  = scale_mode_request;
    draft       = false;
    crop.on     = false;
    const bool want_crop = crop_request[2] > 0;
    if (want_crop && shard_world > 1) {
        logger.log("a crop and a segment shard do not go together\n");
        return JPEGGPU_NOT_SUPPORTED;
    }
    jpeggpu_status st;
    try {
        const int ask = subseq_request > 0 ? subseq_request : -batch_hint;
        st = reader.parse(data, size, ask, logger, device_scan != 0, shard_rank, shard_world, progressive);
        subseq_bytes = reader.subseq_bytes();
    } catch (const std::bad_alloc&) {
        return JPEGGPU_OUT_OF_HOST_MEMORY;
    }
    if (st != JPEGGPU_SUCCESS) return st;
    const Stream& s = reader.s;
    luma_only = false;
    if (luma_only_request) {
        if (s.color_space != kColorGray && s.color_space != kColorYCbCr && s.color_space != kColorRGB) {
            logger.log("luma-only decoding: colour model %d has no grey\n", s.color_space);
            return JPEGGPU_NOT_SUPPORTED;
        }
        luma_only = s.color_space == kColorYCbCr;
    }
    set_block_sizes();
    if (want_crop) {
        if (!set_crop_window()) {
            logger.log("crop %d,%d %dx%d does not lie inside the image\n", crop_request[0], crop_request[1], crop_request[2], crop_request[3]);
            return JPEGGPU_INVALID_ARGUMENT;
        }
        const Scan& sc = s.scans[0];
        if (s.num_scans == 1 && s.restart_interval > 0 && !sc.device_walk && !sc.segments.empty()) {
            const IdctWindow w = scan_window(sc);
            const int m0 = w.my0 * sc.mcus_x + w.mx0, m1 = (w.my0 + w.mcus_y - 1) * sc.mcus_x + w.mx0 + w.mcus_x - 1;
            reader.cut_segments(m0 / sc.mcus_per_segment, m1 / sc.mcus_per_segment + 1);
        }
    }
    if (device_scan)
        logger.log("device-side marker scan: %s (jpeggpu_ext_set_device_scan / JPEGGPU_DEVICE_SCAN)\n",
                   device_scan == 2 ? "checked -- jpeggpu_decoder_decode waits for the stream and returns the device's status" : "asynchronous");
    std::memset(img_info, 0, sizeof(*img_info));
    img_info->num_components = s.num_comp;
    for (int c = 0; c < s.num_comp; ++c) {
        img_info->sizes_x[c]       = plane_x(c);
        img_info->sizes_y[c]       = plane_y(c);
        img_info->subsampling.x[c] = eff_hs(c);
        img_info->subsampling.y[c] = eff_vs(c);
    }
    this->data = data;
    data_size  = size;
    for (int i = 0; i < s.num_scans; ++i) {
        const uint64_t entries = sym_buffer_entries(sym_regions(i), sym_region());
        if (entries * 2u >= (1ull << 32)) {
            logger.log("scan %d: %d subsequences of %d bytes need a symbol stream of %llu bytes (32-bit offsets)\n", i,
                       s.scans[i].num_subseq, subseq_bytes, static_cast<unsigned long long>(entries * 2u));
            return JPEGGPU_NOT_SUPPORTED;
        }
    }
    try {
        make_plan(trace);
    } catch (const std::bad_alloc&) {
        return JPEGGPU_OUT_OF_HOST_MEMORY;
    }
    if (plan.prog.on && plan.off_blob + plan.blob_size >= (1ull << 32)) return JPEGGPU_NOT_SUPPORTED;
    return JPEGGPU_SUCCESS;
}

void Decoder::fill_blob(uint8_t* dst) const
{
    const Stream& s = reader.s;
    std::memset(dst, 0, plan.blob_size);
    std::memcpy(dst + plan.blob_qtables, s.qtable, sizeof(s.qtable));
    for (int i = 0; i < s.num_scans; ++i) {
        const Scan& sc     = s.scans[i];
        const ScanPlan& sp = plan.scan[i];
        if (!sc.table_pack.empty()) std::memcpy(dst + sp.blob_tables, sc.table_pack.data(), sc.table_pack.size());
        if (!sc.table_pack_sync.empty()) std::memcpy(dst + sp.blob_tables_sync, sc.table_pack_sync.data(), sc.table_pack_sync.size());
        if (!sc.segments.empty()) std::memcpy(dst + sp.blob_segments, sc.segments.data(), sc.segments.size() * sizeof(Segment));
        if (!sc.chunks.empty()) std::memcpy(dst + sp.blob_chunks, sc.chunks.data(), sc.chunks.size() * sizeof(DestuffChunk));
        if (!sc.tail_parts.empty()) std::memcpy(dst + sp.blob_parts, sc.tail_parts.data(), sc.tail_parts.size() * sizeof(int));
        if (!sp.mh_blocks.empty()) std::memcpy(dst + sp.blob_mh_blocks, sp.mh_blocks.data(), sp.mh_blocks.size() * sizeof(MhBlock));
    }
    if (!plan.prog.on) return;
    const ProgPlan& pp = plan.prog;
    ProgPlacement at{};
    at.blob_in_tmp = plan.off_blob;
    at.bytes_off = plan.off_bytes, at.bytes_len = plan.bytes_len;
    at.coef_begin = pp.coef_begin, at.coef_bytes = pp.coef_bytes;
    for (int c = 0; c < s.num_comp; ++c) at.coef[c] = pp.coef[c], at.sym[c] = plan.scan[c].sym, at.du_tab[c] = plan.scan[c].du_tab;
    prog_fill_blob(s, pp.blob, at, dst);
}

jpeggpu_status build_jobs(
    Decoder& d, const jpeggpu_img* img, void* d_tmp, size_t tmp_size, int max_intra_iters, bool lone, bool keep_flows, std::vector<ScanJob>& jobs, bool planes)
{
    if (!d.parsed) return JPEGGPU_INVALID_ARGUMENT;
    const Stream& s = d.reader.s;
    for (int c = 0; c < s.num_comp && planes; ++c) {
        if (c > 0 && d.luma_only) break;
        if (!img->image[c] || img->pitch[c] < d.plane_x(c)) return JPEGGPU_INVALID_ARGUMENT;
    }
    if (!d_tmp || (reinterpret_cast<uintptr_t>(d_tmp) & 255)) return JPEGGPU_INVALID_ARGUMENT;
    if (tmp_size < d.plan.total) return JPEGGPU_INTERNAL_ERROR;
    uint8_t* base    = static_cast<uint8_t*>(d_tmp);
    const Plan& plan = d.plan;
    uint8_t* blob    = base + plan.off_blob;

    for (int i = 0; i < s.num_scans; ++i) {
        const Scan& sc     = s.scans[i];
        const ScanPlan& pl = plan.scan[i];
        ScanJob job{};
        ScanParams& sp      = job.sp;
        sp.num_subseq       = sc.num_subseq;
        sp.num_segments     = static_cast<int>(sc.segments.size());
        sp.du_per_mcu       = sc.du_per_mcu;
        sp.num_comp         = sc.num_comp;
        sp.mcus_per_segment = sc.mcus_per_segment;
        sp.total_mcus       = sc.shard_mcus ? sc.shard_mcus : sc.mcus_x * sc.mcus_y;
        sp.subseq_words     = d.subseq_bytes / 4;
        sp.tab_bytes        = static_cast<uint32_t>(sc.table_pack.size());
        sp.max_intra_iters  = keep_flows ? kSeqLanes : max_intra_iters;
        sp.tail_marks       = keep_flows ? 0 : 1;
        sp.cursor_off       = sc.cursor_off;
        sp.tab_bytes_sync   = static_cast<uint32_t>(sc.table_pack_sync.size());
        sp.cursor_off_sync  = sc.cursor_off_sync;
        sp.mh               = lone ? pl.mh : 0;
        sp.seq_subseq       = keep_flows ? kSeqSubseq : kSeqSubseqBatch;
        d.seq_subseq_used   = sp.seq_subseq;
        job.mh_p            = at<int>(base, pl.mh_p);
        job.mh_cz           = at<int>(base, pl.mh_cz);
        job.mh_link         = at<uint32_t>(base, pl.mh_link);
        job.mh_pool         = at<uint2_t>(base, pl.mh_pool);
        job.mh_known        = at<uint8_t>(base, pl.mh_known);
        job.num_mh_blocks   = lone ? static_cast<int>(pl.mh_blocks.size()) : 0;
        job.mh_blocks       = job.num_mh_blocks ? at<const MhBlock>(blob, pl.blob_mh_blocks) : nullptr;
        if (lone && pl.mh_blocks_device) {
            job.num_mh_blocks = pl.mh_blocks_device;
            job.mh_blocks     = at<const MhBlock>(base, pl.d_mh_blocks);
        }
        job.mh_blk_exit     = at<uint16_t>(base, pl.mh_blk_exit);
        job.mh_blk_entry    = at<uint16_t>(base, pl.mh_blk_entry);
        IdctParams& ip = job.ip;
        ip.num_du      = sc.num_du;
        ip.du_per_mcu  = sc.du_per_mcu;
        ip.mcus_x      = sc.mcus_x;
        ip.first_mcu   = sc.first_mcu;
        ip.scale_log2  = static_cast<uint8_t>(d.draft || d.luma_only ? kDraftScale | d.scale_log2 : d.scale_log2);
        ip.idct_method = d.scale_log2 == 0 ? d.idct_method : kIdctReference;
        {
            const MagicDiv a = magic_div(static_cast<uint32_t>(sc.du_per_mcu)), b = magic_div(static_cast<uint32_t>(sc.mcus_x));
            ip.du_per_mcu_mul = a.mul, ip.du_per_mcu_shift = a.shift;
            ip.mcus_x_mul = b.mul, ip.mcus_x_shift = b.shift;
        }
        int du         = 0;
        for (int a = 0; a < sc.num_comp; ++a) {
            const ScanComponent& c = sc.comp[a];
            for (int y = 0; y < c.v; ++y) {
                for (int x = 0; x < c.h; ++x) {
                    ip.du_comp[du] = static_cast<uint8_t>(a);
                    ip.du_dx[du]   = static_cast<uint8_t>(x);
// ... 120 lines not shown
```

jpeggpu_amd/csrc/jg_reader.cpp:

```cpp
#include "jg_reader.hpp"
#include "jg_huff_core.h"

#include <algorithm>
#if defined(__SSE2__)
#include <immintrin.h>
#define JG_HAVE_SSE2 1
#else
#define JG_HAVE_SSE2 0
#endif
#include <cstdlib>
#include <cstring>

namespace jg {

namespace {
constexpr uint8_t M_SOF0 = 0xC0, M_SOF1 = 0xC1, M_SOF2 = 0xC2, M_DHT = 0xC4, M_RST0 = 0xD0, M_RST7 = 0xD7,
                  M_SOI = 0xD8, M_EOI = 0xD9, M_SOS = 0xDA, M_DQT = 0xDB, M_DRI = 0xDD, M_APP0 = 0xE0, M_APP1 = 0xE1, M_APP14 = 0xEE;
constexpr int kNatural[64] = JG_ORDER_NATURAL;

inline int ceil_div(int a, int b) { return (a + b - 1) / b; }
}

#if JG_HAVE_SSE2
struct WindowScan {
    const uint8_t* marker;
    uint32_t ff;
};

#define JG_SCAN_WINDOW_BODY(MASKS)                                                                  \
    const size_t fo    = static_cast<size_t>(from - grid);                                          \
    const uint8_t* blk = grid + (fo & ~static_cast<size_t>(63));                                    \
    uint64_t keep      = ~0ull << (fo & 63);                                                        \
    uint32_t count     = 0;                                                                         \
    for (; blk < lim; blk += 64, keep = ~0ull) {                                                    \
        uint64_t ff, zr;                                                                            \
        MASKS;                                                                                      \
        ff &= keep;                                                                                 \
              \
        const uint64_t next_zero = (zr >> 1) | (static_cast<uint64_t>(blk[64] == 0) << 63);         \
        const uint64_t mk        = ff & ~next_zero;                                                 \
        if (__builtin_expect(mk != 0, 0)) {                                                         \
            const int k = __builtin_ctzll(mk);                                                      \
            count += static_cast<uint32_t>(__builtin_popcountll(ff & ((1ull << k) - 1ull)));        \
            return WindowScan{blk + k, count};                                                      \
        }                                                                                           \
        count += static_cast<uint32_t>(__builtin_popcountll(ff));                                   \
    }                                                                                               \
    return WindowScan{nullptr, count};

WindowScan scan_window_sse2(const uint8_t* from, const uint8_t* lim, const uint8_t* grid)
{
    JG_SCAN_WINDOW_BODY(
        ff = 0; zr = 0; for (int k = 0; k < 4; ++k) {
            const __m128i a = _mm_loadu_si128(reinterpret_cast<const __m128i*>(blk + 16 * k));
            ff |= static_cast<uint64_t>(static_cast<uint32_t>(_mm_movemask_epi8(_mm_cmpeq_epi8(a, _mm_set1_epi8(static_cast<char>(0xFF)))))) << (16 * k);
            zr |= static_cast<uint64_t>(static_cast<uint32_t>(_mm_movemask_epi8(_mm_cmpeq_epi8(a, _mm_setzero_si128())))) << (16 * k);
        })
}

__attribute__((target("avx2,popcnt"))) WindowScan scan_window_avx2(const uint8_t* from, const uint8_t* lim, const uint8_t* grid)
{
    JG_SCAN_WINDOW_BODY(
        const __m256i a0 = _mm256_loadu_si256(reinterpret_cast<const __m256i*>(blk));
        const __m256i a1 = _mm256_loadu_si256(reinterpret_cast<const __m256i*>(blk + 32));
        const __m256i vf = _mm256_set1_epi8(static_cast<char>(0xFF));
        const __m256i vz = _mm256_setzero_si256();
        ff = static_cast<uint32_t>(_mm256_movemask_epi8(_mm256_cmpeq_epi8(a0, vf))) |
             static_cast<uint64_t>(static_cast<uint32_t>(_mm256_movemask_epi8(_mm256_cmpeq_epi8(a1, vf)))) << 32;
        zr = static_cast<uint32_t>(_mm256_movemask_epi8(_mm256_cmpeq_epi8(a0, vz))) |
             static_cast<uint64_t>(static_cast<uint32_t>(_mm256_movemask_epi8(_mm256_cmpeq_epi8(a1, vz)))) << 32;)
}
__attribute__((target("avx512f,avx512bw,popcnt"))) WindowScan scan_window_avx512(const uint8_t* from, const uint8_t* lim, const uint8_t* grid)
{
    JG_SCAN_WINDOW_BODY(
        const __m512i a = _mm512_loadu_si512(reinterpret_cast<const void*>(blk));
        ff = _mm512_cmpeq_epi8_mask(a, _mm512_set1_epi8(static_cast<char>(0xFF)));
        zr = _mm512_testn_epi8_mask(a, a);)
}
#undef JG_SCAN_WINDOW_BODY
#endif

void build_huff_table(
    std::vector<uint8_t>& t, const uint8_t (&num_codes)[16], const uint8_t* huffval, int count, bool is_dc)
{
    const int lb        = is_dc ? kLutBitsDc : kLutBitsAc;
    const size_t lut_sz = static_cast<size_t>(2) << lb;
    t.assign(lut_sz + kHuffAuxSize, 0);
    uint16_t* lut  = reinterpret_cast<uint16_t*>(t.data());
    uint16_t* lim  = reinterpret_cast<uint16_t*>(t.data() + lut_sz);
    uint16_t* voff = lim + 8;
    uint8_t* hv    = t.data() + lut_sz + 32;
    for (int i = 0; i < count && i < 256; ++i) hv[i] = huffval[i];
    int idx       = 0;
    uint32_t code = 0;
    for (int l = 1; l <= 16; ++l) {
        const int first_idx = idx;
        const uint32_t first_code = code;
        for (int i = 0; i < num_codes[l - 1] && idx < 256; ++i) {
            if (l <= lb) {
                const int shift  = lb - l;
                const uint32_t e = huff_entry(l, hv[idx], is_dc);
                const uint32_t lo = (code << shift) & ((1u << lb) - 1);
                for (uint32_t j = 0; j < (1u << shift); ++j) lut[(lo + j) & ((1u << lb) - 1)] = static_cast<uint16_t>(e);
            }
            ++idx;
            ++code;
        }
        if (l >= 9) {
            const uint32_t left = code << (16 - l);
            lim[l - 9]  = static_cast<uint16_t>(left > 0xFFFFu ? 0xFFFFu : left);
            voff[l - 9] = num_codes[l - 1] ? static_cast<uint16_t>((first_idx - static_cast<int>(first_code)) & 0xFF) : 0;
        }
        code <<= 1;
    }
    uint32_t prefix_of[256];
    int num_sub = 0;
    idx         = 0;
    code        = 0;
    for (int l = 1; l <= 16; ++l) {
        for (int i = 0; i < num_codes[l - 1] && idx < 256; ++i, ++idx, ++code) {
            if (l <= lb) continue;
            const uint32_t prefix = (code >> (l - lb)) & ((1u << lb) - 1);
            if (lut[prefix] != 0 || num_sub == kMaxSubTables) continue;
            prefix_of[num_sub++] = prefix;
            lut[prefix]          = static_cast<uint16_t>(num_sub << 5);
        }
        code <<= 1;
    }
    if (num_sub == 0) return;
    t.resize(lut_sz + kHuffAuxSize + static_cast<size_t>(num_sub) * kSubTableSize, 0);
    const uint8_t* aux = t.data() + lut_sz;
    uint16_t* sub      = reinterpret_cast<uint16_t*>(t.data() + lut_sz + kHuffAuxSize);
    const int known    = lb + kSubBits;
    for (int k = 0; k < num_sub; ++k) {
        for (uint32_t i2 = 0; i2 < (1u << kSubBits); ++i2) {
            const uint32_t v    = known >= 16 ? ((prefix_of[k] << kSubBits) | i2) >> (known - 16)
                                              : ((prefix_of[k] << kSubBits) | i2) << (16 - known);
            const uint32_t free = known >= 16 ? 0u : (1u << (16 - known)) - 1u;
            const uint32_t e0 = huff_long_code(aux, v << 16, is_dc);
            const uint32_t e1 = huff_long_code(aux, (v | free) << 16, is_dc);
            const int codelen = static_cast<int>(e0 & 31u) - static_cast<int>((e0 >> 5) & 15u);
            sub[k * (1 << kSubBits) + i2] = static_cast<uint16_t>((e0 == e1 && codelen <= known) ? e0 : 0u);
        }
    }
}

void widen_huff_table(const std::vector<uint8_t>& t, bool is_dc, std::vector<uint8_t>& out)
{
    const int lb          = is_dc ? kLutBitsDc : kLutBitsAc;
    const uint32_t n      = 1u << lb;
    const uint16_t* lut   = reinterpret_cast<const uint16_t*>(t.data());
    const size_t rest     = t.size() - 2u * n;
    out.assign(static_cast<size_t>(kSyncEntryBytes) * n + rest, 0);
    uint32_t* wide = reinterpret_cast<uint32_t*>(out.data());
    for (uint32_t idx = 0; idx < n; ++idx) {
        const uint32_t single = lut[idx];
        uint32_t multi        = single;
        if (!is_dc && (single & 31u) != 0) {
            uint32_t bits = 0, pre = 0, total_adv = 0;
            int count = 0;
            while (true) {
                const uint32_t e   = lut[(idx << bits) & (n - 1u)];
                const uint32_t len = e & 31u, adv = e >> 9;
                if (len == 0) break;
                const bool inside = bits + len <= static_cast<uint32_t>(lb);
                const bool as_last = !inside && bits + (len - ((e >> 5) & 15u)) <= static_cast<uint32_t>(lb);
                if (!inside && !as_last) break;
                if (count > 0 && total_adv > static_cast<uint32_t>(kMultiMaxPre)) break;
                if (bits + len > static_cast<uint32_t>(kSyncMultiMaxBits)) break;
                pre = total_adv;
                total_adv += adv;
                bits += len;
                ++count;
                if (adv == kEobAdvance || as_last) break;
            }
            if (count >= 2) multi = bits | pre << 5 | total_adv << 9;
        }
        wide[idx] = single | multi << 16;
    }
    std::memcpy(out.data() + static_cast<size_t>(kSyncEntryBytes) * n, t.data() + 2u * n, rest);
}

jpeggpu_status Reader::read_sof(const Logger& log)
{
    if (remaining() < 2) return JPEGGPU_INVALID_JPEG;
    const uint16_t length = u16();
    if (length < 2) return JPEGGPU_INVALID_JPEG;
    if (remaining() < static_cast<size_t>(length - 2)) return JPEGGPU_INCOMPLETE_BITSTREAM;
    if (length < 8) return JPEGGPU_INVALID_JPEG;
    const uint8_t precision = u8();
    if (precision != 8) {
        log.log("\tunsupported sample precision %d, only 8 is supported\n", precision);
        return JPEGGPU_NOT_SUPPORTED;
    }
    const uint16_t lines   = u16();
    const uint16_t samples = u16();
    if (lines == 0 || samples == 0) {
        log.log("\tinvalid size x=%d, y=%d\n", samples, lines);
        return JPEGGPU_INVALID_JPEG;
    }
    s.size_x         = samples;
    s.size_y         = lines;
    const uint8_t nc = u8();
    if (nc == 0) return JPEGGPU_INVALID_JPEG;
    if (nc > kMaxComp) {
        log.log("\ttoo many components %d\n", nc);
        return JPEGGPU_NOT_SUPPORTED;
    }
    if (length != 8 + 3 * nc) return JPEGGPU_INVALID_JPEG;
    s.num_comp = nc;
    log.log("\tsize_x: %d, size_y: %d, num_components: %d\n", s.size_x, s.size_y, s.num_comp);
    s.hs_max = s.vs_max = 0;
    for (int c = 0; c < nc; ++c) {
        Component& comp  = s.comp[c];
        comp.id          = u8();
        const uint8_t sf = u8();
        comp.sampling    = sf;
        const int hs = sf >> 4, vs = sf & 15;
        if (hs < 1 || hs > 4 || vs < 1 || vs > 4) {
            log.log("\tinvalid sampling factor (%d, %d)\n", hs, vs);
            return JPEGGPU_INVALID_JPEG;
        }
        comp.hs         = nc == 1 ? 1 : hs;
        comp.vs         = nc == 1 ? 1 : vs;
        const uint8_t q = u8();
        if (q > 3) {
            log.log("\tinvalid quantization table index (%d)\n", q);
            return JPEGGPU_INVALID_JPEG;
        }
        comp.qidx = q;
        for (int d = 0; d < c; ++d) {
            if (s.comp[d].id == comp.id) return JPEGGPU_INVALID_JPEG;
        }
        log.log("\tc_id: %d, ssx: %d, ssy: %d, qi: %d\n", comp.id, comp.hs, comp.vs, comp.qidx);
        s.hs_max = std::max(s.hs_max, comp.hs);
        s.vs_max = std::max(s.vs_max, comp.vs);
    }
    for (int c = 0; c < nc; ++c) {
        Component& comp = s.comp[c];
        comp.size_x     = ceil_div(s.size_x * comp.hs, s.hs_max);
        comp.size_y     = ceil_div(s.size_y * comp.vs, s.vs_max);
        s.prog_blocks_x[c] = std::max(ceil_div(s.size_x, 8 * s.hs_max) * comp.hs, ceil_div(comp.size_x, 8));
        s.prog_blocks_y[c] = std::max(ceil_div(s.size_y, 8 * s.vs_max) * comp.vs, ceil_div(comp.size_y, 8));
    }
    return JPEGGPU_SUCCESS;
}

jpeggpu_status Reader::read_dht(const Logger& log)
{
    if (remaining() < 2) return JPEGGPU_INVALID_JPEG;
    const uint16_t length = u16();
    if (length < 2 || remaining() < static_cast<size_t>(length - 2)) {
        log.log("\ttoo few bytes in DHT segment\n");
        return JPEGGPU_INVALID_JPEG;
    }
    int rem = length - 2;
    while (rem > 0) {
        const uint8_t index = u8();
        --rem;
        const int tc = index >> 4, th = index & 15;
        if (tc != 0 && tc != 1) {
            log.log("\tinvalid Huffman table class\n");
            return JPEGGPU_INVALID_JPEG;
        }
        if (th > 3) {
// ... 155 lines not shown
        case 8: value = static_cast<int16_t>(rd16(at)); break;
        case 9: value = static_cast<int32_t>(rd32(at)); break;
        default: value = 1;
        }
    }
    return value >= 1 && value <= 8 ? static_cast<int>(value) : 1;
}

jpeggpu_status Reader::read_sos(const Logger& log)
{
    if (!found_sof_) return JPEGGPU_INVALID_JPEG;
    if (s.progressive) return read_sos_progressive(log);
    if (remaining() < 3) {
        log.log("\ttoo few bytes in SOS segment\n");
        return JPEGGPU_INVALID_JPEG;
    }
    const uint16_t length = u16();
    if (length < 3) return JPEGGPU_INVALID_JPEG;
    const uint8_t ns = u8();
    if (ns < 1 || ns > 4) {
        log.log("\tinvalid number of components in scan %d\n", ns);
        return JPEGGPU_INVALID_JPEG;
    }
    if (s.num_scans >= kMaxScans) return JPEGGPU_INVALID_JPEG;
    if (length != 6 + 2 * ns) return JPEGGPU_INVALID_JPEG;
    if (remaining() < static_cast<size_t>(2 * ns + 3)) return JPEGGPU_INCOMPLETE_BITSTREAM;

    Scan& scan            = s.scans[s.num_scans];
    scan                  = Scan{};
    scan.num_comp         = ns;
    const bool interleave = ns > 1;
    scan.du_per_mcu       = 0;
    for (int a = 0; a < ns; ++a) {
        ScanComponent& sc = scan.comp[a];
        const uint8_t sel = u8();
        const uint8_t tab = u8();
        const int id_dc = tab >> 4, id_ac = tab & 15;
        log.log("\tc_id: %d, dc: %d, ac: %d\n", sel, id_dc, id_ac);
        int ci = -1;
        for (int i = 0; i < s.num_comp; ++i) {
            if (s.comp[i].id == sel) {
                ci = i;
                break;
            }
        }
        if (ci < 0) {
            log.log("\tinvalid component selector\n");
            return JPEGGPU_INVALID_JPEG;
        }
        if (a > 0 && ci <= scan.comp[a - 1].comp_idx) return JPEGGPU_INVALID_JPEG;
        if (comp_in_scan_[ci]) return JPEGGPU_INVALID_JPEG;
        if (id_dc > 3 || id_ac > 3) return JPEGGPU_INVALID_JPEG;
        if (!dc_defined_[id_dc] || !ac_defined_[id_ac]) return JPEGGPU_INVALID_JPEG;
        const Component& comp = s.comp[ci];
        if (!qt_defined_[comp.qidx]) {
            log.log("\tquantization table at index %d not defined\n", comp.qidx);
            return JPEGGPU_INVALID_JPEG;
        }
        sc.comp_idx = ci;
        sc.dc_id    = id_dc;
        sc.ac_id    = id_ac;
        sc.h        = interleave ? comp.hs : 1;
        sc.v        = interleave ? comp.vs : 1;
        sc.data_x   = ceil_div(comp.size_x, 8 * sc.h) * 8 * sc.h;
        sc.data_y   = ceil_div(comp.size_y, 8 * sc.v) * 8 * sc.v;
        const int mx = sc.data_x / (8 * sc.h), my = sc.data_y / (8 * sc.v);
        if (a > 0 && (mx != scan.mcus_x || my != scan.mcus_y)) {
            log.log("\tcomponents disagree on the number of MCUs\n");
            return JPEGGPU_NOT_SUPPORTED;
        }
        scan.mcus_x = mx;
        scan.mcus_y = my;
        scan.du_per_mcu += sc.h * sc.v;
    }
    if (scan.du_per_mcu > kMaxDuPerMcu) {
        log.log("\ttoo many data units in mcu\n");
        return JPEGGPU_INVALID_JPEG;
    }
    for (int a = 0; a < ns; ++a) comp_in_scan_[scan.comp[a].comp_idx] = true;
    u8();
    u8();
    u8();

    const auto build_pack = [&](const std::vector<uint8_t> (&dc_tabs)[4], const std::vector<uint8_t> (&ac_tabs)[4],
                                std::vector<uint8_t>& pack, uint32_t& cursor_off, uint32_t limit, bool write_pack) -> bool {
        uint32_t dc_off[kMaxComp], ac_off[kMaxComp];
        pack.clear();
        for (int a = 0; a < ns; ++a) {
            const ScanComponent& sc = scan.comp[a];
            int same_dc = -1, same_ac = -1;
            for (int b = 0; b < a; ++b) {
                if (scan.comp[b].dc_id == sc.dc_id) same_dc = b;
                if (scan.comp[b].ac_id == sc.ac_id) same_ac = b;
            }
            if (same_dc >= 0) {
                dc_off[a] = dc_off[same_dc];
            } else {
                dc_off[a] = static_cast<uint32_t>(pack.size());
                pack.insert(pack.end(), dc_tabs[sc.dc_id].begin(), dc_tabs[sc.dc_id].end());
            }
            if (same_ac >= 0) {
                ac_off[a] = ac_off[same_ac];
            } else {
                ac_off[a] = static_cast<uint32_t>(pack.size());
                pack.insert(pack.end(), ac_tabs[sc.ac_id].begin(), ac_tabs[sc.ac_id].end());
                if (write_pack) {
                    uint16_t* lut = reinterpret_cast<uint16_t*>(pack.data() + ac_off[a]);
                    for (uint32_t i = 0; i < (1u << kLutBitsAc); ++i)
                        if ((lut[i] & 31u) == 0 || ((lut[i] >> 5) & 15u) >= static_cast<uint32_t>(kEscapeFromCategory)) lut[i] |= static_cast<uint16_t>(kEntrySlow);
                }
            }
        }
        if (pack.size() + static_cast<size_t>(kMaxDuPerMcu) * sizeof(CursorEntry) > limit) return false;
        cursor_off = static_cast<uint32_t>(pack.size());
        std::vector<CursorEntry> ring;
        for (int a = 0; a < ns; ++a) {
            for (int k = 0; k < scan.comp[a].h * scan.comp[a].v; ++k) {
                CursorEntry ce;
                const uint32_t du = static_cast<uint32_t>(ring.size());
                ce.tabs = dc_off[a] | ac_off[a] << 16;
                ce.meta = 16u * a | du << 8;
                ce.self = cursor_off + 16u * du;
                ce.next = cursor_off + 16u * (static_cast<int>(du) + 1 == scan.du_per_mcu ? 0u : du + 1u);
                ring.push_back(ce);
            }
        }
        const uint8_t* rb = reinterpret_cast<const uint8_t*>(ring.data());
        pack.insert(pack.end(), rb, rb + ring.size() * sizeof(CursorEntry));
        return true;
    };
    if (!build_pack(dc_tab_, ac_tab_, scan.table_pack, scan.cursor_off, kMaxTablePack, true) ||
        !build_pack(dc_tab_sync_, ac_tab_sync_, scan.table_pack_sync, scan.cursor_off_sync, kMaxTablePackSync, false))
        return JPEGGPU_INTERNAL_ERROR;
    const int total_mcus  = scan.mcus_x * scan.mcus_y;
    scan.mcus_per_segment = s.restart_interval ? s.restart_interval : total_mcus;
    if (s.num_scans == 0) s.first_restart_interval = s.restart_interval;
    scan.num_du           = total_mcus * scan.du_per_mcu;
    scan.begin            = static_cast<size_t>(cur_ - base_);
    if (s.num_scans == 0 && subseq_request_ <= 0) {
        subseq_bytes_ = choose_subseq_bytes(-subseq_request_, static_cast<size_t>(end_ - cur_),
                                            static_cast<size_t>(ceil_div(total_mcus, scan.mcus_per_segment)));
        log.log("\tsubsequence size chosen for this image: %d bytes\n", subseq_bytes_);
    }
    if (s.num_scans == 0) s.xfer_begin = (scan.begin - 1) & ~static_cast<size_t>(15);
    ++s.num_scans;
    bool last_scan = true;
    for (int c = 0; c < s.num_comp; ++c) last_scan = last_scan && comp_in_scan_[c];
    if (device_scan_ && last_scan) {
        const uint8_t* stop = end_;
        for (const uint8_t* q = end_; q - (base_ + scan.begin) >= 2;) {
            q = static_cast<const uint8_t*>(memrchr(base_ + scan.begin + 1, 0xD9, static_cast<size_t>(q - (base_ + scan.begin + 1))));
            if (!q) break;
            if (q[-1] == 0xFF) {
                stop = q + 1;
                break;
            }
        }
        const size_t file_end = static_cast<size_t>(stop - base_);
        const size_t bytes    = file_end - scan.begin;
        size_t walked = 0;
        for (int k = 0; k + 1 < s.num_scans; ++k) walked += s.scans[k].end - s.scans[k].begin;
        const bool worth = bytes >= walked;
        const size_t segments = static_cast<size_t>(ceil_div(total_mcus, scan.mcus_per_segment));
        const size_t win0     = (scan.begin - s.xfer_begin) / kDestuffWin;
        const size_t windows  = (file_end - s.xfer_begin + kDestuffWin - 1) / kDestuffWin - win0;
        const size_t subseq   = bytes / static_cast<size_t>(subseq_bytes_) + segments + 1;
        if (worth && segments <= (1u << 20) && subseq < (1u << 24) && bytes < (1u << 27)) {
            scan.device_walk     = true;
            scan.front_win0      = static_cast<uint32_t>(win0);
            scan.expect_segments = static_cast<int>(segments);
            scan.num_subseq      = static_cast<int>(subseq);
            scan.max_chunks      = static_cast<int>(windows + segments + 1);
            scan.max_tail_parts  = static_cast<int>(subseq / kTailPartSubseq + 3);
            scan.end             = file_end;
            s.xfer_end           = scan.end;
            stop_                = true;
            return JPEGGPU_SUCCESS;
        }
    }
    return walk_scan(scan, log);
}

jpeggpu_status Reader::read_sos_progressive(const Logger& log)
{
    if (remaining() < 3) return JPEGGPU_INVALID_JPEG;
    const uint16_t length = u16();
    if (length < 3) return JPEGGPU_INVALID_JPEG;
    const uint8_t ns = u8();
    if (ns < 1 || ns > 4) return JPEGGPU_INVALID_JPEG;
    if (length != 6 + 2 * ns) return JPEGGPU_INVALID_JPEG;
    if (remaining() < static_cast<size_t>(2 * ns + 3)) return JPEGGPU_INCOMPLETE_BITSTREAM;
    if (s.prog_scans.size() >= static_cast<size_t>(kMaxProgScans)) {
        log.log("\tmore than %d scans\n", kMaxProgScans);
        return JPEGGPU_NOT_SUPPORTED;
    }
    ProgScan ps;
    ps.num_comp           = ns;
    const bool interleave = ns > 1;
    for (int a = 0; a < ns; ++a) {
        ScanComponent& sc = ps.comp[a];
        const uint8_t sel = u8();
        const uint8_t tab = u8();
        int ci            = -1;
        for (int i = 0; i < s.num_comp; ++i)
            if (s.comp[i].id == sel) ci = i;
        if (ci < 0) return JPEGGPU_INVALID_JPEG;
        if (a > 0 && ci <= ps.comp[a - 1].comp_idx) return JPEGGPU_INVALID_JPEG;
        if ((tab >> 4) > 3 || (tab & 15) > 3) return JPEGGPU_INVALID_JPEG;
        const Component& comp = s.comp[ci];
        if (!qt_defined_[comp.qidx]) return JPEGGPU_INVALID_JPEG;
        sc.comp_idx = ci;
        sc.dc_id    = tab >> 4;
        sc.ac_id    = tab & 15;
        sc.h        = interleave ? comp.hs : 1;
        sc.v        = interleave ? comp.vs : 1;
        sc.data_x   = ceil_div(comp.size_x, 8 * sc.h) * 8 * sc.h;
// ... 8 lines not shown
    if (ps.du_per_mcu > kMaxDuPerMcu) return JPEGGPU_INVALID_JPEG;
    ps.ss             = u8();
    ps.se             = u8();
    const uint8_t aa  = u8();
    ps.ah             = aa >> 4;
    ps.al             = aa & 15;
    log.log("\tprogressive scan %d: %d components, Ss %d Se %d Ah %d Al %d\n", static_cast<int>(s.prog_scans.size()), ns, ps.ss, ps.se, ps.ah, ps.al);
    if (ps.ss == 0 ? ps.se != 0 : (ps.se < ps.ss || ps.se > 63 || ns != 1)) return JPEGGPU_INVALID_JPEG;
    if (ps.al > 13) return JPEGGPU_INVALID_JPEG;
    if (ps.ah != 0 && ps.ah != ps.al + 1) return JPEGGPU_INVALID_JPEG;
    const bool dc = ps.ss == 0, first = ps.ah == 0;
    ps.kind       = dc ? (first ? kProgDcFirst : kProgDcRefine) : (first ? kProgAcFirst : kProgAcRefine);
    int level = 0;
    for (int a = 0; a < ns; ++a) {
        const int ci = ps.comp[a].comp_idx;
        if (!dc && prog_al_[ci][0] < 0) {
            log.log("\tAC scan of component %d before its first DC scan\n", ci);
            return JPEGGPU_NOT_SUPPORTED;
        }
        for (int k = ps.ss; k <= ps.se; ++k) {
            if (first ? prog_al_[ci][k] >= 0 : prog_al_[ci][k] != ps.ah) {
                log.log("\tscan breaks the progression of component %d, coefficient %d\n", ci, k);
                return JPEGGPU_NOT_SUPPORTED;
            }
            level = std::max(level, prog_level_[ci][k] + 1);
        }
    }
    ps.level = level;
    for (int a = 0; a < ns; ++a) {
        const int ci = ps.comp[a].comp_idx;
        for (int k = ps.ss; k <= ps.se; ++k) {
            prog_al_[ci][k]    = static_cast<int8_t>(ps.al);
            prog_level_[ci][k] = static_cast<int8_t>(level);
        }
        comp_in_scan_[ci] = true;
        if (ps.kind == kProgDcRefine) continue;
        const int tc = dc ? 0 : 1, th = dc ? ps.comp[a].dc_id : ps.comp[a].ac_id;
        if (!(dc ? dc_defined_ : ac_defined_)[th]) return JPEGGPU_INVALID_JPEG;
        const std::vector<uint8_t>& key = dht_key_[tc][th];
        build_prog_table(ps.table[a], key.data(), key.data() + 16, static_cast<int>(key.size()) - 16);
    }
    const int total_mcus = ps.mcus_x * ps.mcus_y;
    ps.mcus_per_segment  = s.restart_interval ? s.restart_interval : total_mcus;
    if (s.prog_scans.empty()) s.first_restart_interval = s.restart_interval;
    ps.begin             = static_cast<size_t>(cur_ - base_);
    if (s.prog_scans.empty()) {
        if (subseq_request_ <= 0) subseq_bytes_ = 64;
        s.xfer_begin = (ps.begin - 1) & ~static_cast<size_t>(15);
    }
    Scan& w = prog_walk_;
    w.segments.clear();
    w.chunks.clear();
    w.num_subseq       = 0;
    w.mcus_x           = ps.mcus_x;
    w.mcus_y           = ps.mcus_y;
    w.mcus_per_segment = ps.mcus_per_segment;
    const jpeggpu_status st = walk_scan(w, log);
    if (st != JPEGGPU_SUCCESS) return st;
    ps.end = w.end;
    ps.segments.assign(w.segments.size(), uint2_t{0u, 0u});
    for (const DestuffChunk& c : w.chunks) {
        uint2_t& g = ps.segments[static_cast<size_t>(c.seg)];
        if (c.first) g.x = c.begin;
        g.y = c.end;
    }
    s.prog_scans.push_back(ps);
    return JPEGGPU_SUCCESS;
}

jpeggpu_status Reader::finish_progressive(const Logger& log)
{
    if (s.prog_scans.empty()) return JPEGGPU_INVALID_JPEG;
    s.num_levels = 0;
    for (const ProgScan& ps : s.prog_scans) s.num_levels = std::max(s.num_levels, ps.level + 1);
    for (int c = 0; c < s.num_comp; ++c) {
        if (prog_al_[c][0] < 0) {
            log.log("\tcomponent %d has no DC scan\n", c);
            return JPEGGPU_INVALID_JPEG;
        }
    }
    s.num_scans = s.num_comp;
    for (int c = 0; c < s.num_comp; ++c) {
        Scan& scan = s.scans[c];
        scan.table_pack.clear(), scan.table_pack_sync.clear(), scan.segments.clear(), scan.chunks.clear();
        scan.tail_parts.assign(1, 0);
        const Component& comp = s.comp[c];
        scan.num_comp         = 1;
        ScanComponent& sc     = scan.comp[0];
        sc.comp_idx = c, sc.dc_id = sc.ac_id = 0, sc.h = sc.v = 1;
        sc.data_x = ceil_div(comp.size_x, 8) * 8, sc.data_y = ceil_div(comp.size_y, 8) * 8;
        scan.du_per_mcu = 1;
        scan.mcus_x = sc.data_x / 8, scan.mcus_y = sc.data_y / 8;
        scan.mcus_per_segment = scan.mcus_x * scan.mcus_y;
        scan.num_du           = scan.mcus_x * scan.mcus_y;
        scan.prog_regions     = scan.num_du;
        scan.begin = s.prog_scans.front().begin, scan.end = s.prog_scans.back().end;
    }
    s.xfer_end = s.prog_scans.back().end;
    return JPEGGPU_SUCCESS;
}

jpeggpu_status Reader::walk_scan(Scan& scan, const Logger& log)
{
    const size_t xb = s.xfer_begin;
    const auto boff = [&](const uint8_t* p) { return static_cast<size_t>(p - base_) - xb; };

    const uint8_t* seg_begin = cur_;
    size_t chunk_begin       = boff(cur_);
    size_t next_win          = (chunk_begin / kDestuffWin + 1) * kDestuffWin;
    uint32_t ff_in_chunk     = 0;
    size_t seg_first_chunk   = scan.chunks.size();
    int seg_dst_base         = 0;
    size_t chunk_dst         = 0;
    const uint8_t* pos       = cur_;
    (void)seg_begin;

    const auto emit = [&](size_t b, size_t e) {
        DestuffChunk c;
        c.win_off = static_cast<uint32_t>(b / kDestuffWin * kDestuffWin);
        c.begin   = static_cast<uint32_t>(b);
        c.end     = static_cast<uint32_t>(e);
        c.dst_off = static_cast<uint32_t>(chunk_dst);
        c.pad_end = 0;
        c.seg     = static_cast<int32_t>(scan.segments.size());
        c.first   = scan.chunks.size() == seg_first_chunk ? 1u : 0u;
        c.reserved = 0;
        scan.chunks.push_back(c);
        chunk_dst += (e - b) - ff_in_chunk;
        ff_in_chunk = 0;
    };

    const uint8_t* const grid = base_ + xb;
    const auto skip_data = [&](const uint8_t* from) -> const uint8_t* {
#if JG_HAVE_SSE2
        const char* pin      = std::getenv("JPEGGPU_HOST_SIMD");
        if (pin && std::strcmp(pin, "scalar") == 0) return from;
        const bool have_avx2 = !(pin && std::strcmp(pin, "sse2") == 0) && __builtin_cpu_supports("avx2") &&
                               __builtin_cpu_supports("popcnt");
        const bool have_avx512 = have_avx2 && !(pin && std::strcmp(pin, "avx2") == 0) && __builtin_cpu_supports("avx512bw") &&
                                 __builtin_cpu_supports("avx512f");
        const uint8_t* const last_blk = end_ - grid > 64 ? grid + ((static_cast<size_t>(end_ - grid) - 1) & ~static_cast<size_t>(63)) : grid;
        while (true) {
            const uint8_t* wend = grid + next_win;
            if (from >= wend) {
                emit(chunk_begin, next_win);
                chunk_begin = next_win;
                next_win += kDestuffWin;
                continue;
            }
            const uint8_t* lim = wend < last_blk ? wend : last_blk;
            if (from >= lim) return from;
            const WindowScan r = have_avx512 ? scan_window_avx512(from, lim, grid)
                                 : have_avx2 ? scan_window_avx2(from, lim, grid)
                                             : scan_window_sse2(from, lim, grid);
            ff_in_chunk += r.ff;
            if (r.marker) return r.marker;
            from = lim;
            if (lim != wend) return from;
        }
#else
        return from;
#endif
    };

    while (true) {
        pos = skip_data(pos);
        const uint8_t* q =
// ... 72 lines not shown

jpeggpu_status Reader::apply_segment_shard(int rank, int world, const Logger& log)
{
    if (s.num_scans != 1 || s.restart_interval == 0) {
        log.log("\tsegment shard needs one scan with restart markers\n");
        return JPEGGPU_NOT_SUPPORTED;
    }
    Scan& scan = s.scans[0];
    if (scan.mcus_per_segment % scan.mcus_x != 0) {
        log.log("\tsegment shard needs a restart interval of whole MCU rows\n");
        return JPEGGPU_NOT_SUPPORTED;
    }
    const int n = static_cast<int>(scan.segments.size());
    const int a = static_cast<int>(static_cast<long long>(n) * rank / world);
    const int b = static_cast<int>(static_cast<long long>(n) * (rank + 1) / world);
    scan.first_segment  = a;
    scan.total_segments = n;
    cut_segments(a, b);
    return JPEGGPU_SUCCESS;
}

void Reader::cut_segments(int a, int b)
{
    Scan& scan           = s.scans[0];
    const int total_mcus = scan.mcus_x * scan.mcus_y;
    scan.first_mcu       = a * scan.mcus_per_segment;
    scan.shard_mcus      = std::min(b * scan.mcus_per_segment, total_mcus) - std::min(a * scan.mcus_per_segment, total_mcus);
    scan.num_du          = scan.shard_mcus * scan.du_per_mcu;
    if (a == b) {
        scan.segments.clear();
        scan.chunks.clear();
        scan.tail_parts.assign(1, 0);
        scan.num_subseq = 0;
        s.xfer_end      = s.xfer_begin;
        return;
    }
    const uint32_t first_sub = static_cast<uint32_t>(scan.segments[a].subseq_offset);
    const uint32_t dst_shift = first_sub * static_cast<uint32_t>(subseq_bytes_);
    std::vector<Segment> segs(scan.segments.begin() + a, scan.segments.begin() + b);
    for (Segment& g : segs) g.subseq_offset -= static_cast<int>(first_sub);
    std::vector<DestuffChunk> chunks;
    for (const DestuffChunk& c : scan.chunks)
        if (c.seg >= a && c.seg < b) chunks.push_back(c);
    const uint32_t win_shift = chunks.front().win_off;
    uint32_t last_end        = 0;
    for (DestuffChunk& c : chunks) {
        c.win_off -= win_shift;
        c.begin -= win_shift;
        c.end -= win_shift;
        c.dst_off -= dst_shift;
        if (c.pad_end) c.pad_end -= dst_shift;
        c.seg -= a;
        last_end = std::max(last_end, c.end);
    }
    s.xfer_begin += win_shift;
    s.xfer_end = s.xfer_begin + last_end;
    scan.segments.swap(segs);
    scan.chunks.swap(chunks);
    scan.num_subseq = scan.segments.back().subseq_offset + scan.segments.back().subseq_count;
    scan.tail_parts.clear();
    scan.tail_parts.push_back(0);
    for (const Segment& seg : scan.segments)
        if (seg.subseq_offset - scan.tail_parts.back() >= kTailPartSubseq) scan.tail_parts.push_back(seg.subseq_offset);
    scan.tail_parts.push_back(scan.num_subseq);
}

jpeggpu_status Reader::parse(const uint8_t* data, size_t size, int subseq_bytes, const Logger& log, bool device_scan,
                             int shard_rank, int shard_world, bool progressive)
{
    progressive_ = progressive;
    std::memset(prog_al_, -1, sizeof(prog_al_));
    std::memset(prog_level_, -1, sizeof(prog_level_));
    if (shard_world > 1 && device_scan) {
        log.log("segment shard %d of %d: host walk, the device scan that was asked for is not used\n", shard_rank, shard_world);
        device_scan = false;
    }
    device_scan_ = device_scan;
    stop_        = false;
    {
        Scan keep[kMaxScans];
        for (int i = 0; i < kMaxScans; ++i) {
            keep[i].table_pack.swap(s.scans[i].table_pack);
            keep[i].table_pack_sync.swap(s.scans[i].table_pack_sync);
            keep[i].segments.swap(s.scans[i].segments);
            keep[i].chunks.swap(s.scans[i].chunks);
            keep[i].tail_parts.swap(s.scans[i].tail_parts);
        }
        s = Stream{};
        for (int i = 0; i < kMaxScans; ++i) {
            keep[i].table_pack.clear();
            keep[i].table_pack_sync.clear();
            keep[i].segments.clear();
            keep[i].chunks.clear();
            keep[i].tail_parts.clear();
            s.scans[i].table_pack.swap(keep[i].table_pack);
            s.scans[i].table_pack_sync.swap(keep[i].table_pack_sync);
            s.scans[i].segments.swap(keep[i].segments);
            s.scans[i].chunks.swap(keep[i].chunks);
            s.scans[i].tail_parts.swap(keep[i].tail_parts);
        }
    }
    std::memset(s.qtable, 0, sizeof(s.qtable));
    base_         = data;
    cur_          = data;
    end_          = data + size;
    subseq_request_ = subseq_bytes;
    subseq_bytes_   = subseq_bytes > 0 ? subseq_bytes : 64;
    found_sof_    = false;
    exif_         = nullptr;
    exif_len_     = 0;
    exif_cat_.clear();
    std::memset(qt_defined_, 0, sizeof(qt_defined_));
    std::memset(dc_defined_, 0, sizeof(dc_defined_));
    std::memset(ac_defined_, 0, sizeof(ac_defined_));
    std::memset(comp_in_scan_, 0, sizeof(comp_in_scan_));
    if (size >= (1ull << 31)) return JPEGGPU_NOT_SUPPORTED;

    const auto read_marker = [&](uint8_t& marker) -> jpeggpu_status {
        if (remaining() < 2) {
            log.log("\ttoo few bytes for marker\n");
            return JPEGGPU_INVALID_JPEG;
        }
        const uint8_t ff = u8();
        if (ff != 0xFF) {
            log.log("\tinvalid marker byte 0x%02x\n", ff);
            return JPEGGPU_INVALID_JPEG;
        }
        marker = u8();
        while (marker == 0xFF) {
            if (remaining() < 1) return JPEGGPU_INVALID_JPEG;
            marker = u8();
        }
        return JPEGGPU_SUCCESS;
    };

    uint8_t marker = 0;
    jpeggpu_status st;
    if ((st = read_marker(marker)) != JPEGGPU_SUCCESS) return st;
    if (marker != M_SOI) return JPEGGPU_INVALID_JPEG;
    do {
        if ((st = read_marker(marker)) != JPEGGPU_SUCCESS) return st;
        log.log("marker 0x%02x\n", marker);
        st = JPEGGPU_SUCCESS;
        if (marker == M_SOF0 || marker == M_SOF1 || (marker == M_SOF2 && progressive_)) {
            if (found_sof_) return JPEGGPU_INVALID_JPEG;
            found_sof_ = true;
            st         = read_sof(log);
            if (st == JPEGGPU_SUCCESS && marker == M_SOF2) {
                s.progressive = true;
                if (shard_world > 1) {
                    log.log("\ta segment shard of a progressive frame is not supported\n");
                    return JPEGGPU_NOT_SUPPORTED;
                }
            }
        } else if (
            (marker >= 0xC2 && marker <= 0xCF && marker != M_DHT && marker != 0xC8 &&
             marker != 0xCC)) {
            log.log("\tunsupported JPEG type: SOF%d\n", marker - 0xC0);
            return JPEGGPU_NOT_SUPPORTED;
        } else if (marker == M_DHT) {
            st = read_dht(log);
        } else if (marker == M_SOS) {
            st = read_sos(log);
            if (st == JPEGGPU_SUCCESS && stop_) break;
        } else if (marker == M_DQT) {
            st = read_dqt(log);
        } else if (marker == M_DRI) {
            st = read_dri(log);
        } else if (marker == M_EOI) {
            break;
        } else if (marker == M_SOI || (marker >= M_RST0 && marker <= M_RST7) || marker == 0x01) {
            return JPEGGPU_INVALID_JPEG;
        } else {
            if (marker == M_APP0 || marker == M_APP14) note_app_segment(marker);
            if (marker == M_APP1) note_exif_segment();
            st = skip_segment(log);
        }
        if (st != JPEGGPU_SUCCESS) return st;
    } while (true);
// ... 23 lines not shown
```

jpeggpu_amd/csrc/jg_reader.hpp:

```cpp
#ifndef JG_READER_HPP_
#define JG_READER_HPP_

#include "jg_defs.h"
#include "jg_prog_core.h"

#include <jpeggpu/jpeggpu.h>

#include <cstdarg>
#include <cstdio>
#include <vector>

namespace jg {

struct Logger {
    bool enabled = false;
    void log(const char* fmt, ...) const __attribute__((format(printf, 2, 3)))
    {
        if (!enabled) return;
        va_list ap;
        va_start(ap, fmt);
        vprintf(fmt, ap);
        va_end(ap);
    }
};

struct Component {
    uint8_t id;
    uint8_t qidx;
    int hs, vs;
    uint8_t sampling;
    int size_x, size_y;
};

struct ScanComponent {
    int comp_idx;
    int dc_id, ac_id;
    int h, v;
    int data_x, data_y;
};

struct Scan {
    int num_comp = 0;
    ScanComponent comp[kMaxComp];
    size_t begin = 0;
    size_t end   = 0;
    int du_per_mcu = 0;
    int mcus_x = 0, mcus_y = 0;
    int mcus_per_segment = 0;
    int num_subseq = 0;
    int num_du = 0;
    int first_mcu  = 0;
    int shard_mcus = 0;
    int first_segment = 0, total_segments = 0;
    std::vector<uint8_t> table_pack;
    std::vector<uint8_t> table_pack_sync;
    uint32_t cursor_off = 0, cursor_off_sync = 0;
    std::vector<Segment> segments;
    std::vector<DestuffChunk> chunks;
    std::vector<int> tail_parts;
    bool device_walk    = false;
    uint32_t front_win0 = 0;
    int expect_segments = 0;
    int max_chunks      = 0;
    int max_tail_parts  = 0;
    int prog_regions = 0;
};

struct ProgScan {
    int kind = 0;
    int num_comp = 0;
    ScanComponent comp[kMaxComp];
    int ss = 0, se = 0, ah = 0, al = 0;
    int level = 0;
    int du_per_mcu = 0;
    int mcus_x = 0, mcus_y = 0, mcus_per_segment = 0;
    size_t begin = 0, end = 0;
    ProgTable table[kMaxComp];
    std::vector<uint2_t> segments;
};

enum ColorSpace : int { kColorUnknown = 0, kColorGray = 1, kColorYCbCr = 2, kColorRGB = 3, kColorCMYK = 4, kColorYCCK = 5 };

struct Stream {
    int size_x = 0, size_y = 0;
    int hs_max = 0, vs_max = 0;
    int num_comp = 0;
    Component comp[kMaxComp];
    int restart_interval = 0;
    int num_scans = 0;
    Scan scans[kMaxScans];
    uint16_t qtable[4][64];
    bool qtable16[4]{};
    int first_restart_interval = 0;
    size_t xfer_begin = 0;
    size_t xfer_end   = 0;
    bool saw_jfif = false, saw_adobe = false;
    uint8_t adobe_transform = 0;
    int color_space = kColorUnknown;
    int orientation = 1;
    bool progressive = false;
    int num_levels   = 0;
    std::vector<ProgScan> prog_scans;
    int prog_blocks_x[kMaxComp]{}, prog_blocks_y[kMaxComp]{};
};

constexpr int kBatchHintFull = 64;
constexpr int kSubseqAutoLone = 0, kSubseqAutoBatched = -kBatchHintFull;
constexpr int kLonePlanImages = 1;
inline bool lone_plan(int images_per_call) { return images_per_call <= kLonePlanImages; }

constexpr size_t kSmallCallBytes = 36u << 20;
inline int choose_subseq_bytes(int images_per_call, size_t scan_bytes_bound, size_t segments)
{
    if (segments == 0) segments = 1;
    const size_t per_segment = scan_bytes_bound / segments;
    const bool batched = !lone_plan(images_per_call);
    int b = batched ? 256 : 64;
    if (batched && static_cast<size_t>(images_per_call) * scan_bytes_bound < kSmallCallBytes) b = 128;
    if (!batched && segments > 1 && scan_bytes_bound < (1u << 20)) b = 32;
    while (b > 32 && per_segment < static_cast<size_t>(8 * b)) b >>= 1;
    while (b > 64 && scan_bytes_bound < static_cast<size_t>(2 * kSeqSubseq) * static_cast<size_t>(b)) b >>= 1;
    return b;
}

struct Reader {
    jpeggpu_status parse(const uint8_t* data, size_t size, int subseq_bytes, const Logger& log, bool device_scan = false,
                         int shard_rank = 0, int shard_world = 1, bool progressive = false);
    int subseq_bytes() const { return subseq_bytes_; }
    void cut_segments(int a, int b);

    Stream s;

  private:
    const uint8_t* base_ = nullptr;
    const uint8_t* cur_  = nullptr;
    const uint8_t* end_  = nullptr;
    int subseq_bytes_    = 128;
    int subseq_request_  = 128;
    bool found_sof_      = false;
    bool qt_defined_[4]{};
    bool dc_defined_[4]{}, ac_defined_[4]{};
    std::vector<uint8_t> dc_tab_[4], ac_tab_[4];
    std::vector<uint8_t> dc_tab_sync_[4], ac_tab_sync_[4];
    std::vector<uint8_t> dht_key_[2][4];
    bool comp_in_scan_[kMaxComp]{};
    bool device_scan_ = false;
    bool stop_        = false;
    bool progressive_ = false;
    int8_t prog_al_[kMaxComp][64]{};
    int8_t prog_level_[kMaxComp][64]{};
    Scan prog_walk_;
    const uint8_t* exif_ = nullptr;
    size_t exif_len_     = 0;
    std::vector<uint8_t> exif_cat_;

    size_t remaining() const { return static_cast<size_t>(end_ - cur_); }
    uint8_t u8() { return *cur_++; }
    uint16_t u16()
    {
        const uint16_t hi = u8();
        return static_cast<uint16_t>(hi << 8 | u8());
    }
    jpeggpu_status read_sof(const Logger& log);
    jpeggpu_status read_dht(const Logger& log);
    jpeggpu_status read_dqt(const Logger& log);
    jpeggpu_status read_dri(const Logger& log);
    jpeggpu_status read_sos(const Logger& log);
    jpeggpu_status read_sos_progressive(const Logger& log);
    jpeggpu_status finish_progressive(const Logger& log);
    jpeggpu_status walk_scan(Scan& scan, const Logger& log);
    jpeggpu_status skip_segment(const Logger& log);
    void note_app_segment(uint8_t marker);
    void note_exif_segment();
    jpeggpu_status apply_segment_shard(int rank, int world, const Logger& log);
};

int exif_orientation(const uint8_t* d, size_t n);

void build_huff_table(
    std::vector<uint8_t>& t, const uint8_t (&num_codes)[16], const uint8_t* huffval, int count, bool is_dc);
void widen_huff_table(const std::vector<uint8_t>& t, bool is_dc, std::vector<uint8_t>& out);

}

#endif
```

jpeggpu_amd/csrc/jg_sync_runs.h:

```cpp
#ifndef JG_SYNC_RUNS_H_
#define JG_SYNC_RUNS_H_

#include "jg_huff_core.h"

namespace jg {

struct RunLane {
    int a;
    int next;
    int last;
    int end;
    bool active;
    Segment seg;
    int rel;
    LaneState st;
};

template <int R>
JG_HD inline void run_plan(RunLane& ln, int l, int g0, int seq, int S)
{
    const bool overlap = l == 0;
    ln.a               = overlap ? g0 - 1 : g0 + (l - 1) * R;
    ln.active          = ln.a >= 0 && ln.a < S && l <= seq;
    ln.next            = l < seq ? (overlap ? g0 : ln.a + R) : -1;
    ln.last            = l > seq ? ln.a : l == seq ? ln.a + R - 1 : ln.next;
    if (ln.last > S - 1) ln.last = S - 1;
    ln.end = g0 + seq * R < S ? g0 + seq * R : S;
    ln.seg = Segment{0, 0};
    ln.rel = -1;
    ln.st  = LaneState{};
}

template <int W, class Fetch, class Io>
JG_HD inline void run_speculate(RunLane& ln, int l, const Segment& seg, Fetch& fetch, const uint8_t* tabs, const ScanParams& sp, Io& io)
{
    constexpr int kBits = W * 32;
    if (!ln.active) return;
    ln.seg  = seg;
    ln.rel  = ln.a - seg.subseq_offset;
    ln.st.p = ln.rel * kBits;
    fetch.set_row(ln.a, ln.rel);
    BitWindow<Fetch> bw{};
    bw.seek(ln.st.p, fetch);
    SpecSink none;
    decode_subsequence(ln.st, bw, fetch, (ln.rel + 1) * kBits, tabs, sp, none);
    io.put_e1(l, ln.st.p, ln.st.c | (ln.st.z << 8));
}

template <int W, int R, class Fetch, class Io>
JG_HD inline void run_flow(RunLane& ln, int l, Fetch& fetch, const uint8_t* tabs, const ScanParams& sp, Io& io)
{
    constexpr int kBits = W * 32;
    NoSink sink;
#if defined(__HIP_DEVICE_COMPILE__)
#pragma nounroll
#endif
    for (int k = 1; k <= R; ++k) {
        const int j = ln.a + k;
        if (j > ln.last) break;
        if (ln.rel + 1 == ln.seg.subseq_count) {
            ln.seg = io.segment_of(j);
            ln.rel = -1;
            ln.st  = LaneState{};
        }
        ln.st.n    = 0;
        ln.st.dc01 = 0;
        ln.st.dc23 = 0;
        ++ln.rel;
        fetch.set_row(j, ln.rel);
        BitWindow<Fetch> bw{};
        bw.seek(ln.st.p, fetch);
        decode_subsequence(ln.st, bw, fetch, (ln.rel + 1) * kBits, tabs, sp, sink);
        const int cz = ln.st.c | (ln.st.z << 8);
        bool pending = false;
        if (j == ln.next) pending = !io.e1_is(l + 1, ln.st.p, cz) && j + 1 < ln.end && ln.rel + 1 < ln.seg.subseq_count;
        io.store(j, ln.st, cz, pending);
    }
}

}

#endif
```

Baseline: 32760 images/s.

## Add wide-index AC Huffman tables for the batched sync kernels

```diff
diff --git a/include/jpeggpu/jpeggpu_ext.h b/include/jpeggpu/jpeggpu_ext.h
--- a/include/jpeggpu/jpeggpu_ext.h
+++ b/include/jpeggpu/jpeggpu_ext.h
@@ -121,6 +121,7 @@
 enum jpeggpu_status jpeggpu_ext_batch_set_overlap(jpeggpu_batch_t batch, int parts);
 enum jpeggpu_status jpeggpu_ext_batch_set_fused_tail(jpeggpu_batch_t batch, int enable);
 enum jpeggpu_status jpeggpu_ext_batch_set_sync_run(jpeggpu_batch_t batch, int r);
+enum jpeggpu_status jpeggpu_ext_batch_set_sync_wide(jpeggpu_batch_t batch, int enable);
 enum jpeggpu_status jpeggpu_ext_fused_tail_timeouts(unsigned int* count);
 enum jpeggpu_status jpeggpu_ext_batch_set_profiling(jpeggpu_batch_t batch, int enable);
 enum jpeggpu_status jpeggpu_ext_batch_get_stage_ms(jpeggpu_batch_t batch, float* ms );
diff --git a/jpeggpu_amd/api.py b/jpeggpu_amd/api.py
--- a/jpeggpu_amd/api.py
+++ b/jpeggpu_amd/api.py
@@ -234,6 +234,7 @@
     L.jpeggpu_ext_batch_set_sync_iterations.argtypes = [C.c_void_p, C.c_int]
     L.jpeggpu_ext_batch_set_overlap.argtypes = [C.c_void_p, C.c_int]
     for name, args in (("jpeggpu_ext_batch_set_fused_tail", [C.c_void_p, C.c_int]), ("jpeggpu_ext_batch_set_sync_run", [C.c_void_p, C.c_int]),
+                       ("jpeggpu_ext_batch_set_sync_wide", [C.c_void_p, C.c_int]),
                        ("jpeggpu_ext_fused_tail_timeouts", [C.POINTER(C.c_uint)])):
         if hasattr(L, name):
             getattr(L, name).argtypes = args
@@ -583,6 +584,9 @@
     def set_sync_run(self, r: int):
         _check(_newer_symbol("jpeggpu_ext_batch_set_sync_run")(self._h, int(r)), "jpeggpu_ext_batch_set_sync_run")
 
+    def set_sync_wide(self, enable: bool):
+        _check(_newer_symbol("jpeggpu_ext_batch_set_sync_wide")(self._h, 1 if enable else 0), "jpeggpu_ext_batch_set_sync_wide")
+
     def set_coefficients_only(self, enable: bool):
         _check(_newer_symbol("jpeggpu_ext_batch_set_coefficients_only")(self._h, 1 if enable else 0), "jpeggpu_ext_batch_set_coefficients_only")
 
diff --git a/jpeggpu_amd/csrc/jg_batch.cpp b/jpeggpu_amd/csrc/jg_batch.cpp
--- a/jpeggpu_amd/csrc/jg_batch.cpp
+++ b/jpeggpu_amd/csrc/jg_batch.cpp
@@ -27,6 +27,8 @@
     long long keep_flows_below  = jg::kKeepFlowsBelowSubseq;
     bool fuse_tail_write        = true;
     int sync_run                = 2;
+    bool sync_wide              = true;
+    std::vector<uint32_t> wide_bytes;
     bool coefficients_only      = false;
     static constexpr int kMaxOverlap = 4;
     int overlap                 = 1;
@@ -79,6 +81,8 @@
         const size_t first_job = b.jobs.size();
         const jpeggpu_status st = jg::build_jobs(it.decoder->d, it.img, it.d_tmp, it.tmp_size, b.sync_iters, false, c.keep_flows, b.jobs, !b.coefficients_only);
         if (st != JPEGGPU_SUCCESS) return st;
+        for (size_t j = first_job; j < b.jobs.size(); ++j)
+            b.wide_bytes.push_back(static_cast<uint32_t>(it.decoder->d.reader.s.scans[j - first_job].table_pack_wide.size()));
         if (const int dk = jg::device_scan_index(it.decoder->d); dk >= 0) {
             b.fronts.push_back(jg::front_params(it.decoder->d, it.d_tmp, d_jobs_rw + first_job + static_cast<size_t>(dk), dk));
             c.front_windows = std::max(c.front_windows, b.fronts.back().num_windows);
@@ -139,6 +143,13 @@
             p.extent.repack_flows = c.keep_flows;
             p.extent.fuse_tail_write = b.fuse_tail_write && !b.sync_iters_set;
             p.extent.sync_run = c.keep_flows || b.sync_iters_set ? 1 : b.sync_run;
+            p.extent.sync_wide = b.sync_wide && !c.keep_flows && p.end > p.begin;
+            for (int j = p.begin; j < p.end && p.extent.sync_wide; ++j) {
+                const uint32_t wb = b.wide_bytes[static_cast<size_t>(j)];
+                if (wb == 0 && b.jobs[static_cast<size_t>(j)].sp.tab_bytes_sync != 0) p.extent.sync_wide = false;
+                p.extent.max_tab_bytes_wide = std::max(p.extent.max_tab_bytes_wide, wb);
+            }
+            if (p.extent.max_tab_bytes_wide == 0) p.extent.sync_wide = false;
             if (p.end > p.begin) b.parts.push_back(p);
         }
     }
@@ -198,6 +209,7 @@
     if (!batch || !items || num_items < 0 || !d_scratch) return JPEGGPU_INVALID_ARGUMENT;
     if (num_items == 0) return JPEGGPU_SUCCESS;
     batch->jobs.clear();
+    batch->wide_bytes.clear();
     batch->fronts.clear();
     batch->progs.clear();
     batch->prog_extent = jg::ProgExtent{};
@@ -253,6 +265,7 @@
         const int r = std::atoi(e);
         if (r == 1 || r == 2 || r == 4) b->sync_run = r;
     }
+    if (const char* e = std::getenv("JPEGGPU_SYNC_WIDE")) b->sync_wide = std::atoi(e) != 0;
     for (int r = 0; r < jpeggpu_batch::kRing; ++r) {
         void* p = nullptr;
         if (hipHostMalloc(&p, jpeggpu_ext_batch_scratch_size(max_scans), hipHostMallocDefault) != hipSuccess ||
@@ -343,6 +356,13 @@
     return JPEGGPU_SUCCESS;
 }
 
+enum jpeggpu_status jpeggpu_ext_batch_set_sync_wide(jpeggpu_batch_t batch, int enable)
+{
+    if (!batch) return JPEGGPU_INVALID_ARGUMENT;
+    batch->sync_wide = enable != 0;
+    return JPEGGPU_SUCCESS;
+}
+
 enum jpeggpu_status jpeggpu_ext_batch_set_profiling(jpeggpu_batch_t batch, int enable)
 {
     if (!batch) return JPEGGPU_INVALID_ARGUMENT;
diff --git a/jpeggpu_amd/csrc/jg_defs.h b/jpeggpu_amd/csrc/jg_defs.h
--- a/jpeggpu_amd/csrc/jg_defs.h
+++ b/jpeggpu_amd/csrc/jg_defs.h
@@ -45,6 +45,13 @@
               "a multi-symbol entry: codes inside the index, the last symbol's magnitude (category <= 15) behind it");
 constexpr int kDcTableSizeSync = (kSyncEntryBytes << kLutBitsDc) + kHuffAuxSize;
 constexpr int kAcTableSizeSync = (kSyncEntryBytes << kLutBitsAc) + kHuffAuxSize;
+
+constexpr int kLutBitsAcWideMax = 13;
+static_assert(kLutBitsAcWideMax + 15 <= kSyncMultiMaxBits, "a multi-symbol entry of the widest table fits the length field");
+constexpr uint32_t kSyncWideHeaderBytes = 16;
+constexpr uint32_t kSyncWideStateBytes = 4 * 6240;
+constexpr uint32_t kSyncWidePackBudget = 80 * 1024 - kSyncWideStateBytes;
+static_assert(256 + kSyncWidePackBudget <= 65536, "absolute table addresses are packed into 16 bits (load_tables)");
 
 constexpr uint32_t kMaxTablePack =
     kMaxComp * (kDcTableSize + kMaxSubTables * kSubTableSize) + kMaxComp * (kAcTableSize + kMaxSubTables * kSubTableSize) + kMaxDuPerMcu * 16;
diff --git a/jpeggpu_amd/csrc/jg_huff_core.h b/jpeggpu_amd/csrc/jg_huff_core.h
--- a/jpeggpu_amd/csrc/jg_huff_core.h
+++ b/jpeggpu_amd/csrc/jg_huff_core.h
@@ -111,6 +111,17 @@
     return huff_long_code(aux, peek, is_dc);
 }
 
+JG_HD inline uint32_t huff_second_level_wide(TabPtr tab, uint32_t e, uint32_t peek, bool is_dc, int lb)
+{
+    const TabPtr aux = tab + (static_cast<uint32_t>(kSyncEntryBytes) << lb);
+    if (e != 0) {
+        const uint32_t i2 = (peek >> (32 - kSubBits - lb)) & ((1u << kSubBits) - 1u);
+        e                 = ld_u16(aux + kHuffAuxSize - kSubTableSize + (e >> 5) * kSubTableSize + 2 * i2);
+        if (e != 0) return e;
+    }
+    return huff_long_code(aux, peek, is_dc);
+}
+
 JG_HD inline int extend_magnitude(uint32_t bits, int s)
 {
     const uint32_t mask = (1u << s) - 1u;
@@ -149,7 +160,7 @@
 #define JG_WAVE_ANY(x) (x)
 #endif
 
-template <class Fetch, class Sink>
+template <bool kWide = false, class Fetch, class Sink>
 JG_HD inline void decode_subsequence(
     LaneState& st,
     BitWindow<Fetch>& bw,
@@ -202,15 +213,19 @@
         is_dc = du_end;                         \
     } while (0)
     {
+#define JG_IDX_SHIFT() (is_dc ? 32u - kLutBitsDc : kWide ? (JG_CUR_META >> 16) & 0xFFu : 32u - kLutBitsAc)
+#define JG_SECOND_LEVEL(e16)                                                                              \
+    (kWide ? huff_second_level_wide(tab, (e16), peek, is_dc, 32 - static_cast<int>(JG_IDX_SHIFT()))       \
+           : huff_second_level<kSyncEntryBytes>(tab, (e16), peek, is_dc))
         while (end_bit - p >= 31) {
             peek               = bw.peek(fetch);
             const TabPtr tab   = JG_TAB_AT(tabs, is_dc ? (JG_CUR_TABS & 0xFFFFu) : (JG_CUR_TABS >> 16));
-            const uint32_t idx = peek >> (is_dc ? 32 - kLutBitsDc : 32 - kLutBitsAc);
+            const uint32_t idx = peek >> JG_IDX_SHIFT();
             const uint32_t e32 = ld_u32(tab + kSyncEntryBytes * idx);
             const uint32_t one = e32 & 0xFFFFu, m = e32 >> 16;
             e                  = zm + static_cast<int>((m >> 5) & 15u) < 63 ? m : one;
             if (JG_WAVE_ANY((one & 31u) == 0)) {
-                if ((one & 31u) == 0) e = huff_second_level<kSyncEntryBytes>(tab, one, peek, is_dc);
+                if ((one & 31u) == 0) e = JG_SECOND_LEVEL(one);
             }
             total = e & 31;
             JG_COMMIT();
@@ -219,9 +234,9 @@
     do {                                                                                                  \
         peek               = bw.peek(fetch);                                                              \
         const TabPtr tab   = JG_TAB_AT(tabs, is_dc ? (JG_CUR_TABS & 0xFFFFu) : (JG_CUR_TABS >> 16));      \
-        const uint32_t idx = peek >> (is_dc ? 32 - kLutBitsDc : 32 - kLutBitsAc);                         \
+        const uint32_t idx = peek >> JG_IDX_SHIFT();                                                      \
         e                  = ld_u16(tab + kSyncEntryBytes * idx);                                         \
-        if ((e & 31u) == 0) e = huff_second_level<kSyncEntryBytes>(tab, e, peek, is_dc);                  \
+        if ((e & 31u) == 0) e = JG_SECOND_LEVEL(e);                                                       \
         total = e & 31;                                                                                   \
     } while (0)
         JG_LOOKUP_SYNC();
@@ -230,6 +245,8 @@
             JG_LOOKUP_SYNC();
         }
 #undef JG_LOOKUP_SYNC
+#undef JG_SECOND_LEVEL
+#undef JG_IDX_SHIFT
     }
 #undef JG_COMMIT
     if (Sink::kSums) st.n += 64 * units + (zm + 1) - st.z;
diff --git a/jpeggpu_amd/csrc/jg_kernels.hip b/jpeggpu_amd/csrc/jg_kernels.hip
--- a/jpeggpu_amd/csrc/jg_kernels.hip
+++ b/jpeggpu_amd/csrc/jg_kernels.hip
@@ -541,6 +541,35 @@
     static_assert(kTabs % 16 == 0, "the table pack is read with 16-byte loads");
 };
 static_assert(kStaticLdsSlack + SeqLdsBatch::kTabs + kMaxTablePackSync <= 65536, "absolute table addresses are packed into 16 bits (load_tables)");
+template <bool kWide>
+struct BatchShape {
+    static constexpr int kSeqPerWg = kWide ? 4 : kBatchSeqPerWg;
+    static constexpr int kLanes    = T * kSeqPerWg;
+};
+static_assert(BatchShape<true>::kSeqPerWg * SeqLdsBatch::kOne == kSyncWideStateBytes, "the pack's budget is what four sequences' state leaves of half a CU's LDS");
+template <bool kWide>
+constexpr size_t batch_lds_bytes(uint32_t tab_bytes)
+{
+    return static_cast<size_t>(BatchShape<kWide>::kSeqPerWg) * SeqLdsBatch::kOne + (tab_bytes + 15u) / 16u * 16u;
+}
+template <bool kWide>
+__device__ __forceinline__ JG_GLOBAL const uint8_t* batch_pack(const JobView& J, ScanParams& sp, uint8_t* smem, int which, uint8_t*& s_tab, uint8_t*& s_state)
+{
+    if constexpr (kWide) {
+        JG_GLOBAL const uint8_t* hdr = J.tables_sync + sp.tab_bytes_sync;
+        const uint2 h  = ld_global(reinterpret_cast<JG_GLOBAL const uint2*>(hdr));
+        sp.tab_bytes   = h.x;
+        sp.cursor_off  = h.y;
+        s_tab          = smem;
+        s_state        = smem + (h.x + 15u) / 16u * 16u + which * SeqLdsBatch::kOne;
+        return hdr + kSyncWideHeaderBytes;
+    } else {
+        sp.use_sync_pack();
+        s_tab   = smem + SeqLdsBatch::kTabs;
+        s_state = smem + SeqLdsBatch::kState + which * SeqLdsBatch::kOne;
+        return J.tables_sync;
+    }
+}
 constexpr int kFuseJobs = 16, kFuseMaxJobs = 256, kFuseOwn = kFuseJobs + 2 * kFuseMaxJobs;
 constexpr uint32_t kFuseEmpty = 0xFFFFFFFFu;
 static_assert(fuse_ctl_words(0) == static_cast<size_t>(kFuseOwn), "the plan carves what fuse_init lays out (jg_defs.h)");
@@ -583,36 +612,37 @@
     }
 };
 
-template <int W, class JS, int R>
+template <int W, class JS, int R, bool kWide>
 __device__ __forceinline__ void sync_intra_batch_runs(const JS& js, uint8_t* smem)
 {
+    constexpr int kSeqPerWg = BatchShape<kWide>::kSeqPerWg;
     const int which = threadIdx.x / T, l = threadIdx.x % T;
-    int* s_p        = reinterpret_cast<int*>(smem + SeqLdsBatch::kState + which * SeqLdsBatch::kOne);
-    int* s_cz       = s_p + 2 * T;
-    uint8_t* s_tab  = smem + SeqLdsBatch::kTabs;
 
     const JobView J(js.get());
     if constexpr (std::is_same<JS, JobArray>::value) {
-        if (blockIdx.x == 0) fuse_init(js.jobs, static_cast<int>(blockIdx.y), J, T * kBatchSeqPerWg);
-    }
-    if (static_cast<int>(blockIdx.x) * kBatchSeqPerWg * R >= J.num_seq) return;
+        if (blockIdx.x == 0) fuse_init(js.jobs, static_cast<int>(blockIdx.y), J, T * kSeqPerWg);
+    }
+    if (static_cast<int>(blockIdx.x) * kSeqPerWg * R >= J.num_seq) return;
     ScanParams sp = J.sp;
-    sp.use_sync_pack();
+    uint8_t *s_tab, *s_state;
+    JG_GLOBAL const uint8_t* g_tab = batch_pack<kWide>(J, sp, smem, which, s_tab, s_state);
+    int* s_p        = reinterpret_cast<int*>(s_state);
+    int* s_cz       = s_p + 2 * T;
     const int SEQ   = sp.seq_subseq;
-    const int group = static_cast<int>(blockIdx.x) * kBatchSeqPerWg + which;
+    const int group = static_cast<int>(blockIdx.x) * kSeqPerWg + which;
     RunLane ln;
     run_plan<R>(ln, l, group * SEQ * R, SEQ, sp.num_subseq);
     const int lane_seg = J.seg_idx[ln.active ? ln.a : 0];
 
-    load_tables(s_tab, J.tables_sync, sp);
+    load_tables(s_tab, g_tab, sp);
     const Segment lane_segment = ld_global(J.segments + lane_seg);
     __syncthreads();
 
     GlobalFetch<W> fetch{reinterpret_cast<JG_GLOBAL const uint32_t*>(J.destuffed), 0, 0};
     const RunIo io{J, s_p, s_cz};
-    run_speculate<W>(ln, l, lane_segment, fetch, s_tab, sp, io);
-    __syncthreads();
-    run_flow<W, R>(ln, l, fetch, s_tab, sp, io);
+    run_speculate<W, kWide>(ln, l, lane_segment, fetch, s_tab, sp, io);
+    __syncthreads();
+    run_flow<W, R, kWide>(ln, l, fetch, s_tab, sp, io);
 
     if (l < R && group * R + l < J.num_seq) {
         J.bnd_p[group * R + l]  = -1;
@@ -620,31 +650,32 @@
     }
 }
 
-template <int W, class JS, int R = 1>
-__global__ __launch_bounds__(T * kBatchSeqPerWg) void huff_sync_intra_batch(JS js)
+template <int W, class JS, int R = 1, bool kWide = false>
+__global__ __launch_bounds__(BatchShape<kWide>::kLanes) void huff_sync_intra_batch(JS js)
 {
     extern __shared__ __attribute__((aligned(16))) uint8_t smem[];
     if constexpr (R > 1) {
-        sync_intra_batch_runs<W, JS, R>(js, smem);
+        sync_intra_batch_runs<W, JS, R, kWide>(js, smem);
         return;
     }
+    constexpr int kSeqPerWg = BatchShape<kWide>::kSeqPerWg;
     const int which = threadIdx.x / T;
-    const int seq   = blockIdx.x * kBatchSeqPerWg + which;
-    int* s_p         = reinterpret_cast<int*>(smem + SeqLdsBatch::kState + which * SeqLdsBatch::kOne);
+    const int seq   = blockIdx.x * kSeqPerWg + which;
+
+    const JobView J(js.get());
+    if constexpr (std::is_same<JS, JobArray>::value) {
+        if (blockIdx.x == 0) fuse_init(js.jobs, static_cast<int>(blockIdx.y), J, T * kSeqPerWg);
+    }
+    if (static_cast<int>(blockIdx.x) * kSeqPerWg >= J.num_seq) return;
+    ScanParams sp = J.sp;
+    uint8_t *s_tab, *s_state;
+    JG_GLOBAL const uint8_t* g_tab = batch_pack<kWide>(J, sp, smem, which, s_tab, s_state);
+    int* s_p         = reinterpret_cast<int*>(s_state);
     int* s_n         = s_p + T;
     int* s_cz        = s_n + T;
     uint32_t* s_dc01 = reinterpret_cast<uint32_t*>(s_cz + T);
     uint32_t* s_dc23 = s_dc01 + T;
     int* s_pend      = reinterpret_cast<int*>(s_dc23 + T);
-    uint8_t* s_tab   = smem + SeqLdsBatch::kTabs;
-
-    const JobView J(js.get());
-    if constexpr (std::is_same<JS, JobArray>::value) {
-        if (blockIdx.x == 0) fuse_init(js.jobs, static_cast<int>(blockIdx.y), J, T * kBatchSeqPerWg);
-    }
-    if (static_cast<int>(blockIdx.x) * kBatchSeqPerWg >= J.num_seq) return;
-    ScanParams sp = J.sp;
-    sp.use_sync_pack();
     const int t         = threadIdx.x % T;
     s_pend[t]           = 0;
     const int SEQ = sp.seq_subseq, OV = T - SEQ;
@@ -657,7 +688,7 @@
     const bool active   = sub >= 0 && t < img_end;
     const int lane_seg = J.seg_idx[active ? sub : 0];
 
-    load_tables(s_tab, J.tables_sync, sp);
+    load_tables(s_tab, g_tab, sp);
     const Segment lane_segment = ld_global(J.segments + lane_seg);
     __syncthreads();
 
@@ -684,10 +715,10 @@
             bw.seek(st.p, fetch);
             if (JS::kSpeculateStateOnly) {
                 SpecSink none;
-                decode_subsequence(st, bw, fetch, (rel + 1) * kBits, s_tab, sp, none);
+                decode_subsequence<kWide>(st, bw, fetch, (rel + 1) * kBits, s_tab, sp, none);
             } else {
                 NoSink sums;
-                decode_subsequence(st, bw, fetch, (rel + 1) * kBits, s_tab, sp, sums);
+                decode_subsequence<kWide>(st, bw, fetch, (rel + 1) * kBits, s_tab, sp, sums);
                 s_n[t]    = st.n;
                 s_dc01[t] = st.dc01;
                 s_dc23[t] = st.dc23;
@@ -724,7 +755,7 @@
             ++rel;
             fetch.set_row(img_first + j, rel);
             bw.seek(st.p, fetch);
-            decode_subsequence(st, bw, fetch, (rel + 1) * kBits, s_tab, sp, sink);
+            decode_subsequence<kWide>(st, bw, fetch, (rel + 1) * kBits, s_tab, sp, sink);
             const int cz = st.c | (st.z << 8);
             if (st.p == s_p[j] && cz == s_cz[j] && (s_pend[j] & 2)) flowing = false;
             s_p[j]    = st.p;
@@ -1642,6 +1673,20 @@
     return e.fuse_tail_write && !e.repack_flows && e.max_tail_parts > 0 && e.max_tail_part < kTailLargeFrom && e.max_seq > 0 && num_jobs <= kFuseMaxJobs;
 }
 
+template <int W, class JS, int R, bool kWide>
+hipError_t launch_sync_batch(const JS& js, int max_seq, int grid_y, uint32_t tab_bytes, hipStream_t stream)
+{
+    if constexpr (std::is_same<JS, JobArray>::value) {
+        constexpr int per_wg = BatchShape<kWide>::kSeqPerWg * R;
+        const size_t lds     = batch_lds_bytes<kWide>(tab_bytes);
+        if (const hipError_t err = allow_lds(huff_sync_intra_batch<W, JS, R, kWide>, lds); err != hipSuccess) return err;
+        huff_sync_intra_batch<W, JS, R, kWide><<<dim3((max_seq + per_wg - 1) / per_wg, grid_y), BatchShape<kWide>::kLanes, lds, stream>>>(js);
+        return hipSuccess;
+    } else {
+        return hipErrorInvalidValue;
+    }
+}
+
 template <int W, class JS>
 hipError_t launch_huff(Stage stage, const JS& js, const JobExtent& e, int grid_y, hipStream_t stream)
 {
@@ -1656,6 +1701,13 @@
         } else if (e.repack_flows) {
             if ((err = allow_lds(huff_sync_intra<W, JobArrayLow>, seq_lds)) != hipSuccess) return err;
             huff_sync_intra<W, JobArrayLow><<<dim3(e.max_seq, grid_y), T, seq_lds, stream>>>(JobArrayLow{js.jobs});
+        } else if (e.sync_wide) {
+            if (e.max_tab_bytes_wide == 0 || e.max_tab_bytes_wide > kSyncWidePackBudget) return hipErrorInvalidValue;
+            const int R = e.sync_run == 2 || e.sync_run == 4 ? e.sync_run : 1;
+            if (R == 2) err = launch_sync_batch<W, JS, 2, true>(js, e.max_seq, grid_y, e.max_tab_bytes_wide, stream);
+            else if (R == 4) err = launch_sync_batch<W, JS, 4, true>(js, e.max_seq, grid_y, e.max_tab_bytes_wide, stream);
+            else err = launch_sync_batch<W, JS, 1, true>(js, e.max_seq, grid_y, e.max_tab_bytes_wide, stream);
+            if (err != hipSuccess) return err;
         } else {
             const size_t lds = SeqLdsBatch::kTabs + e.max_tab_bytes_sync;
             if (e.sync_run == 2 || e.sync_run == 4) {
diff --git a/jpeggpu_amd/csrc/jg_kernels.hpp b/jpeggpu_amd/csrc/jg_kernels.hpp
--- a/jpeggpu_amd/csrc/jg_kernels.hpp
+++ b/jpeggpu_amd/csrc/jg_kernels.hpp
@@ -36,6 +36,8 @@
     uint32_t max_tab_bytes_sync = 0;
     bool fuse_tail_write = false;
     int sync_run        = 1;
+    bool sync_wide      = false;
+    uint32_t max_tab_bytes_wide = 0;
     bool repack_flows   = false;
 };
 void extend(JobExtent& e, const ScanJob& job);
diff --git a/jpeggpu_amd/csrc/jg_plan.cpp b/jpeggpu_amd/csrc/jg_plan.cpp
--- a/jpeggpu_amd/csrc/jg_plan.cpp
+++ b/jpeggpu_amd/csrc/jg_plan.cpp
@@ -99,7 +99,7 @@
         const Scan& sc      = s.scans[i];
         ScanPlan& sp        = p.scan[i];
         sp.blob_tables      = blob(sc.table_pack.size());
-        sp.blob_tables_sync = blob(sc.table_pack_sync.size());
+        sp.blob_tables_sync = blob(sc.table_pack_sync.size() + (sc.table_pack_wide.empty() ? 0 : kSyncWideHeaderBytes + sc.table_pack_wide.size()));
         sp.blob_segments    = blob(sc.segments.size() * sizeof(Segment));
         sp.blob_chunks      = blob(sc.chunks.size() * sizeof(DestuffChunk));
         sp.blob_parts       = blob(sc.tail_parts.size() * sizeof(int));
@@ -248,6 +248,7 @@
     jpeggpu_status st;
     try {
         const int ask = subseq_request > 0 ? subseq_request : -batch_hint;
+        reader.set_sync_wide(batched);
         st = reader.parse(data, size, ask, logger, device_scan != 0, shard_rank, shard_world, progressive);
         subseq_bytes = reader.subseq_bytes();
     } catch (const std::bad_alloc&) {
@@ -316,6 +317,13 @@
         const ScanPlan& sp = plan.scan[i];
         if (!sc.table_pack.empty()) std::memcpy(dst + sp.blob_tables, sc.table_pack.data(), sc.table_pack.size());
         if (!sc.table_pack_sync.empty()) std::memcpy(dst + sp.blob_tables_sync, sc.table_pack_sync.data(), sc.table_pack_sync.size());
+        if (!sc.table_pack_wide.empty()) {
+            uint8_t* hdr            = dst + sp.blob_tables_sync + sc.table_pack_sync.size();
+            const uint32_t words[4] = {static_cast<uint32_t>(sc.table_pack_wide.size()), sc.cursor_off_wide, 0u, 0u};
+            static_assert(sizeof(words) == kSyncWideHeaderBytes, "the header of the wide pack");
+            std::memcpy(hdr, words, sizeof(words));
+            std::memcpy(hdr + kSyncWideHeaderBytes, sc.table_pack_wide.data(), sc.table_pack_wide.size());
+        }
         if (!sc.segments.empty()) std::memcpy(dst + sp.blob_segments, sc.segments.data(), sc.segments.size() * sizeof(Segment));
         if (!sc.chunks.empty()) std::memcpy(dst + sp.blob_chunks, sc.chunks.data(), sc.chunks.size() * sizeof(DestuffChunk));
         if (!sc.tail_parts.empty()) std::memcpy(dst + sp.blob_parts, sc.tail_parts.data(), sc.tail_parts.size() * sizeof(int));
diff --git a/jpeggpu_amd/csrc/jg_reader.cpp b/jpeggpu_amd/csrc/jg_reader.cpp
--- a/jpeggpu_amd/csrc/jg_reader.cpp
+++ b/jpeggpu_amd/csrc/jg_reader.cpp
@@ -2,6 +2,7 @@
 #include "jg_huff_core.h"
 
 #include <algorithm>
+#include <atomic>
 #if defined(__SSE2__)
 #include <immintrin.h>
 #define JG_HAVE_SSE2 1
@@ -81,9 +82,9 @@
 #endif
 
 void build_huff_table(
-    std::vector<uint8_t>& t, const uint8_t (&num_codes)[16], const uint8_t* huffval, int count, bool is_dc)
-{
-    const int lb        = is_dc ? kLutBitsDc : kLutBitsAc;
+    std::vector<uint8_t>& t, const uint8_t (&num_codes)[16], const uint8_t* huffval, int count, bool is_dc, int index_bits)
+{
+    const int lb        = index_bits > 0 ? index_bits : is_dc ? kLutBitsDc : kLutBitsAc;
     const size_t lut_sz = static_cast<size_t>(2) << lb;
     t.assign(lut_sz + kHuffAuxSize, 0);
     uint16_t* lut  = reinterpret_cast<uint16_t*>(t.data());
@@ -145,9 +146,9 @@
     }
 }
 
-void widen_huff_table(const std::vector<uint8_t>& t, bool is_dc, std::vector<uint8_t>& out)
-{
-    const int lb          = is_dc ? kLutBitsDc : kLutBitsAc;
+void widen_huff_table(const std::vector<uint8_t>& t, bool is_dc, std::vector<uint8_t>& out, int index_bits)
+{
+    const int lb          = index_bits > 0 ? index_bits : is_dc ? kLutBitsDc : kLutBitsAc;
     const uint32_t n      = 1u << lb;
     const uint16_t* lut   = reinterpret_cast<const uint16_t*>(t.data());
     const size_t rest     = t.size() - 2u * n;
@@ -181,6 +182,45 @@
     std::memcpy(out.data() + static_cast<size_t>(kSyncEntryBytes) * n, t.data() + 2u * n, rest);
 }
 
+namespace {
+std::atomic<uint64_t> g_wide_table_builds{0};
+}
+uint64_t wide_table_builds() { return g_wide_table_builds.load(std::memory_order_relaxed); }
+
+void build_wide_table(const uint8_t* payload, size_t payload_len, int index_bits, std::vector<uint8_t>& out)
+{
+    uint8_t num_codes[16];
+    std::memcpy(num_codes, payload, 16);
+    std::vector<uint8_t> narrow;
+    build_huff_table(narrow, num_codes, payload + 16, static_cast<int>(payload_len) - 16, false, index_bits);
+    widen_huff_table(narrow, false, out, index_bits);
+    g_wide_table_builds.fetch_add(1, std::memory_order_relaxed);
+}
+
+const std::vector<uint8_t>& WideTableCache::get(const std::vector<uint8_t>& payload, int index_bits)
+{
+    for (Form& f : forms_) {
+        if (f.bits == index_bits && f.key == payload) {
+            f.used = ++clock_;
+            return f.table;
+        }
+    }
+    Form* slot = nullptr;
+    if (forms_.size() < kForms) {
+        forms_.emplace_back();
+        slot = &forms_.back();
+    } else {
+        slot = &forms_[0];
+        for (Form& f : forms_)
+            if (f.used < slot->used) slot = &f;
+    }
+    slot->key  = payload;
+    slot->bits = index_bits;
+    slot->used = ++clock_;
+    build_wide_table(payload.data(), payload.size(), index_bits, slot->table);
+    return slot->table;
+}
+
 jpeggpu_status Reader::read_sof(const Logger& log)
 {
     if (remaining() < 2) return JPEGGPU_INVALID_JPEG;
@@ -502,8 +542,8 @@
     u8();
     u8();
 
-    const auto build_pack = [&](const std::vector<uint8_t> (&dc_tabs)[4], const std::vector<uint8_t> (&ac_tabs)[4],
-                                std::vector<uint8_t>& pack, uint32_t& cursor_off, uint32_t limit, bool write_pack) -> bool {
+    const auto build_pack = [&](const std::vector<uint8_t>* const (&dc_tabs)[4], const std::vector<uint8_t>* const (&ac_tabs)[4],
+                                std::vector<uint8_t>& pack, uint32_t& cursor_off, uint32_t limit, bool write_pack, const int* ac_bits) -> bool {
         uint32_t dc_off[kMaxComp], ac_off[kMaxComp];
         pack.clear();
         for (int a = 0; a < ns; ++a) {
@@ -517,13 +557,13 @@
                 dc_off[a] = dc_off[same_dc];
             } else {
                 dc_off[a] = static_cast<uint32_t>(pack.size());
-                pack.insert(pack.end(), dc_tabs[sc.dc_id].begin(), dc_tabs[sc.dc_id].end());
+                pack.insert(pack.end(), dc_tabs[sc.dc_id]->begin(), dc_tabs[sc.dc_id]->end());
             }
             if (same_ac >= 0) {
                 ac_off[a] = ac_off[same_ac];
             } else {
                 ac_off[a] = static_cast<uint32_t>(pack.size());
-                pack.insert(pack.end(), ac_tabs[sc.ac_id].begin(), ac_tabs[sc.ac_id].end());
+                pack.insert(pack.end(), ac_tabs[sc.ac_id]->begin(), ac_tabs[sc.ac_id]->end());
                 if (write_pack) {
                     uint16_t* lut = reinterpret_cast<uint16_t*>(pack.data() + ac_off[a]);
                     for (uint32_t i = 0; i < (1u << kLutBitsAc); ++i)
@@ -540,6 +580,7 @@
                 const uint32_t du = static_cast<uint32_t>(ring.size());
                 ce.tabs = dc_off[a] | ac_off[a] << 16;
                 ce.meta = 16u * a | du << 8;
+                if (ac_bits) ce.meta |= static_cast<uint32_t>(32 - ac_bits[scan.comp[a].ac_id]) << 16;
                 ce.self = cursor_off + 16u * du;
                 ce.next = cursor_off + 16u * (static_cast<int>(du) + 1 == scan.du_per_mcu ? 0u : du + 1u);
                 ring.push_back(ce);
@@ -549,9 +590,43 @@
         pack.insert(pack.end(), rb, rb + ring.size() * sizeof(CursorEntry));
         return true;
     };
-    if (!build_pack(dc_tab_, ac_tab_, scan.table_pack, scan.cursor_off, kMaxTablePack, true) ||
-        !build_pack(dc_tab_sync_, ac_tab_sync_, scan.table_pack_sync, scan.cursor_off_sync, kMaxTablePackSync, false))
-        return JPEGGPU_INTERNAL_ERROR;
+    {
+        const std::vector<uint8_t>* dc[4] = {&dc_tab_[0], &dc_tab_[1], &dc_tab_[2], &dc_tab_[3]};
+        const std::vector<uint8_t>* ac[4] = {&ac_tab_[0], &ac_tab_[1], &ac_tab_[2], &ac_tab_[3]};
+        const std::vector<uint8_t>* dcs[4] = {&dc_tab_sync_[0], &dc_tab_sync_[1], &dc_tab_sync_[2], &dc_tab_sync_[3]};
+        const std::vector<uint8_t>* acs[4] = {&ac_tab_sync_[0], &ac_tab_sync_[1], &ac_tab_sync_[2], &ac_tab_sync_[3]};
+        if (!build_pack(dc, ac, scan.table_pack, scan.cursor_off, kMaxTablePack, true, nullptr) ||
+            !build_pack(dcs, acs, scan.table_pack_sync, scan.cursor_off_sync, kMaxTablePackSync, false, nullptr))
+            return JPEGGPU_INTERNAL_ERROR;
+        scan.table_pack_wide.clear();
+        scan.cursor_off_wide = 0;
+        for (int id = 0; id < 4; ++id) scan.wide_bits[id] = 0;
+        if (sync_wide_) {
+            int units[4] = {0, 0, 0, 0}, first[4] = {ns, ns, ns, ns};
+            for (int a = 0; a < ns; ++a) {
+                units[scan.comp[a].ac_id] += scan.comp[a].h * scan.comp[a].v;
+                first[scan.comp[a].ac_id] = std::min(first[scan.comp[a].ac_id], a);
+            }
+            int top = scan.comp[0].ac_id;
+            for (int id = 0; id < 4; ++id)
+                if (units[id] > units[top] || (units[id] == units[top] && first[id] < first[top])) top = id;
+            const bool forced = wide_top_ > 0;
+            for (int k = 0; k < (forced ? 1 : kWideAssignments); ++k) {
+                int bits[4];
+                const std::vector<uint8_t>* acw[4] = {nullptr, nullptr, nullptr, nullptr};
+                for (int id = 0; id < 4; ++id) {
+                    bits[id] = forced ? (id == top ? wide_top_ : wide_rest_) : id == top ? kWideAssignment[k][0] : kWideAssignment[k][1];
+                    if (units[id] > 0) acw[id] = &wide_cache_.get(dht_key_[1][id], bits[id]);
+                }
+                if (build_pack(dcs, acw, scan.table_pack_wide, scan.cursor_off_wide, forced ? 65535u : kSyncWidePackBudget, false, bits)) {
+                    for (int id = 0; id < 4; ++id) scan.wide_bits[id] = units[id] > 0 ? bits[id] : 0;
+                    break;
+                }
+                scan.table_pack_wide.clear();
+            }
+            if (scan.table_pack_wide.empty()) return JPEGGPU_INTERNAL_ERROR;
+        }
+    }
     const int total_mcus  = scan.mcus_x * scan.mcus_y;
     scan.mcus_per_segment = s.restart_interval ? s.restart_interval : total_mcus;
     if (s.num_scans == 0) s.first_restart_interval = s.restart_interval;
@@ -726,7 +801,7 @@
     s.num_scans = s.num_comp;
     for (int c = 0; c < s.num_comp; ++c) {
         Scan& scan = s.scans[c];
-        scan.table_pack.clear(), scan.table_pack_sync.clear(), scan.segments.clear(), scan.chunks.clear();
+        scan.table_pack.clear(), scan.table_pack_sync.clear(), scan.table_pack_wide.clear(), scan.segments.clear(), scan.chunks.clear();
         scan.tail_parts.assign(1, 0);
         const Component& comp = s.comp[c];
         scan.num_comp         = 1;
@@ -965,6 +1040,7 @@
         for (int i = 0; i < kMaxScans; ++i) {
             keep[i].table_pack.swap(s.scans[i].table_pack);
             keep[i].table_pack_sync.swap(s.scans[i].table_pack_sync);
+            keep[i].table_pack_wide.swap(s.scans[i].table_pack_wide);
             keep[i].segments.swap(s.scans[i].segments);
             keep[i].chunks.swap(s.scans[i].chunks);
             keep[i].tail_parts.swap(s.scans[i].tail_parts);
@@ -973,11 +1049,13 @@
         for (int i = 0; i < kMaxScans; ++i) {
             keep[i].table_pack.clear();
             keep[i].table_pack_sync.clear();
+            keep[i].table_pack_wide.clear();
             keep[i].segments.clear();
             keep[i].chunks.clear();
             keep[i].tail_parts.clear();
             s.scans[i].table_pack.swap(keep[i].table_pack);
             s.scans[i].table_pack_sync.swap(keep[i].table_pack_sync);
+            s.scans[i].table_pack_wide.swap(keep[i].table_pack_wide);
             s.scans[i].segments.swap(keep[i].segments);
             s.scans[i].chunks.swap(keep[i].chunks);
             s.scans[i].tail_parts.swap(keep[i].tail_parts);
diff --git a/jpeggpu_amd/csrc/jg_reader.hpp b/jpeggpu_amd/csrc/jg_reader.hpp
--- a/jpeggpu_amd/csrc/jg_reader.hpp
+++ b/jpeggpu_amd/csrc/jg_reader.hpp
@@ -55,6 +55,9 @@
     std::vector<uint8_t> table_pack;
     std::vector<uint8_t> table_pack_sync;
     uint32_t cursor_off = 0, cursor_off_sync = 0;
+    std::vector<uint8_t> table_pack_wide;
+    uint32_t cursor_off_wide = 0;
+    int wide_bits[4] = {0, 0, 0, 0};
     std::vector<Segment> segments;
     std::vector<DestuffChunk> chunks;
     std::vector<int> tail_parts;
@@ -123,10 +126,35 @@
     return b;
 }
 
+constexpr int kWideAssignments = 5;
+constexpr int kWideAssignment[kWideAssignments][2] = {{13, 12}, {13, 11}, {12, 12}, {12, 11}, {11, 11}};
+static_assert(kWideAssignment[0][0] == kLutBitsAcWideMax && kWideAssignment[kWideAssignments - 1][0] == kLutBitsAc &&
+                  kWideAssignment[kWideAssignments - 1][1] == kLutBitsAc,
+              "from the widest index down to the sync pack's");
+
+void build_wide_table(const uint8_t* payload, size_t payload_len, int index_bits, std::vector<uint8_t>& out);
+uint64_t wide_table_builds();
+class WideTableCache {
+  public:
+    WideTableCache() { forms_.reserve(kForms); }
+    const std::vector<uint8_t>& get(const std::vector<uint8_t>& payload, int index_bits);
+
+  private:
+    static constexpr size_t kForms = 16;
+    struct Form {
+        std::vector<uint8_t> key, table;
+        int bits      = 0;
+        uint64_t used = 0;
+    };
+    std::vector<Form> forms_;
+    uint64_t clock_ = 0;
+};
+
 struct Reader {
     jpeggpu_status parse(const uint8_t* data, size_t size, int subseq_bytes, const Logger& log, bool device_scan = false,
                          int shard_rank = 0, int shard_world = 1, bool progressive = false);
     int subseq_bytes() const { return subseq_bytes_; }
+    void set_sync_wide(bool on, int top_bits = 0, int rest_bits = 0) { sync_wide_ = on, wide_top_ = top_bits, wide_rest_ = rest_bits; }
     void cut_segments(int a, int b);
 
     Stream s;
@@ -143,6 +171,9 @@
     std::vector<uint8_t> dc_tab_[4], ac_tab_[4];
     std::vector<uint8_t> dc_tab_sync_[4], ac_tab_sync_[4];
     std::vector<uint8_t> dht_key_[2][4];
+    bool sync_wide_ = false;
+    int wide_top_ = 0, wide_rest_ = 0;
+    WideTableCache wide_cache_;
     bool comp_in_scan_[kMaxComp]{};
     bool device_scan_ = false;
     bool stop_        = false;
@@ -178,8 +209,8 @@
 int exif_orientation(const uint8_t* d, size_t n);
 
 void build_huff_table(
-    std::vector<uint8_t>& t, const uint8_t (&num_codes)[16], const uint8_t* huffval, int count, bool is_dc);
-void widen_huff_table(const std::vector<uint8_t>& t, bool is_dc, std::vector<uint8_t>& out);
+    std::vector<uint8_t>& t, const uint8_t (&num_codes)[16], const uint8_t* huffval, int count, bool is_dc, int index_bits = 0);
+void widen_huff_table(const std::vector<uint8_t>& t, bool is_dc, std::vector<uint8_t>& out, int index_bits = 0);
 
 }
 
diff --git a/jpeggpu_amd/csrc/jg_sync_runs.h b/jpeggpu_amd/csrc/jg_sync_runs.h
--- a/jpeggpu_amd/csrc/jg_sync_runs.h
+++ b/jpeggpu_amd/csrc/jg_sync_runs.h
@@ -31,7 +31,7 @@
     ln.st  = LaneState{};
 }
 
-template <int W, class Fetch, class Io>
+template <int W, bool kWide = false, class Fetch, class Io>
 JG_HD inline void run_speculate(RunLane& ln, int l, const Segment& seg, Fetch& fetch, const uint8_t* tabs, const ScanParams& sp, Io& io)
 {
     constexpr int kBits = W * 32;
@@ -43,11 +43,11 @@
     BitWindow<Fetch> bw{};
     bw.seek(ln.st.p, fetch);
     SpecSink none;
-    decode_subsequence(ln.st, bw, fetch, (ln.rel + 1) * kBits, tabs, sp, none);
+    decode_subsequence<kWide>(ln.st, bw, fetch, (ln.rel + 1) * kBits, tabs, sp, none);
     io.put_e1(l, ln.st.p, ln.st.c | (ln.st.z << 8));
 }
 
-template <int W, int R, class Fetch, class Io>
+template <int W, int R, bool kWide = false, class Fetch, class Io>
 JG_HD inline void run_flow(RunLane& ln, int l, Fetch& fetch, const uint8_t* tabs, const ScanParams& sp, Io& io)
 {
     constexpr int kBits = W * 32;
@@ -70,7 +70,7 @@
         fetch.set_row(j, ln.rel);
         BitWindow<Fetch> bw{};
         bw.seek(ln.st.p, fetch);
-        decode_subsequence(ln.st, bw, fetch, (ln.rel + 1) * kBits, tabs, sp, sink);
+        decode_subsequence<kWide>(ln.st, bw, fetch, (ln.rel + 1) * kBits, tabs, sp, sink);
         const int cz = ln.st.c | (ln.st.z << 8);
         bool pending = false;
         if (j == ln.next) pending = !io.e1_is(l + 1, ln.st.p, cz) && j + 1 < ln.end && ln.rel + 1 < ln.seg.subseq_count;
```

Result: slower. 32360 images/s (-1.2%).
